# cvg/pixel-perfect-sfm

Hardware: NVIDIA B200
Metric: featuremetric BA observations/sec (higher is better)
Workload: dtype f64 (fp16 taps, fp32 horizontal, fp64 vertical/solve)

## Files before the change

pixel-perfect-sfm_b200/build.py:

```python
import os
import subprocess
import sys
from concurrent.futures import ThreadPoolExecutor

HERE = os.path.dirname(os.path.abspath(__file__))
CSRC = os.path.join(HERE, "csrc")
SOURCES = ["pxr_api.cu", "pxr_upload.cu", "pxr_ba.cu", "pxr_ba_block.cu", "pxr_inner.cu", "pxr_refs.cu", "pxr_ka.cu", "pxr_synth.cu", "pxr_extract.cu", "pxr_problem.cu"]
NVCC = os.environ.get("NVCC", "/usr/local/cuda/bin/nvcc")
FLAGS = ["-gencode", "arch=compute_100a,code=sm_100a", "-lineinfo", "-O3", "-std=c++17",
         "-Xcompiler", "-fPIC", "-ccbin", "/usr/bin/g++", "--expt-relaxed-constexpr",
         "-Xptxas", "-v"]
if os.environ.get("PXR_FM_WARPS"):
    FLAGS.append("-DPXR_FM_WARPS=" + os.environ["PXR_FM_WARPS"])


def _newer(src, obj):
    if not os.path.exists(obj):
        return True
    t = os.path.getmtime(obj)
    deps = [src] + [os.path.join(CSRC, f) for f in os.listdir(CSRC) if f.endswith((".cuh", ".h"))]
    deps.append(os.path.join(HERE, "..", "include", "pxr.h"))
    return any(os.path.getmtime(d) > t for d in deps)


def compile_one(name, verbose):
    src = os.path.join(CSRC, name)
    obj = os.path.join(CSRC, name.replace(".cu", ".o"))
    if not _newer(src, obj):
        return name, "up to date"
    cmd = [NVCC] + FLAGS + ["-c", src, "-o", obj]
    r = subprocess.run(cmd, capture_output=True, text=True)
    log = os.path.join(CSRC, name.replace(".cu", ".ptxas.log"))
    with open(log, "w") as f:
        f.write(r.stderr)
    if r.returncode != 0:
        sys.stderr.write(r.stderr[-6000:])
        raise RuntimeError("nvcc failed for " + name)
    return name, "compiled"


def build(verbose=False):
    srcs = [s for s in SOURCES if os.path.exists(os.path.join(CSRC, s))]
    with ThreadPoolExecutor(max_workers=min(8, len(srcs))) as ex:
        for name, status in ex.map(lambda n: compile_one(n, verbose), srcs):
            if verbose:
                print("  %-16s %s" % (name, status))
    objs = [os.path.join(CSRC, s.replace(".cu", ".o")) for s in srcs]
    out = os.path.join(CSRC, "libpxr.so")
    if (not os.path.exists(out)) or any(os.path.getmtime(o) > os.path.getmtime(out) for o in objs):
        cmd = [NVCC, "-shared", "-o", out] + objs + ["-gencode", "arch=compute_100a,code=sm_100a",
                                                     "-Xcompiler", "-fPIC", "-ccbin", "/usr/bin/g++", "-lcudart", "-ldl"]
        r = subprocess.run(cmd, capture_output=True, text=True)
        if r.returncode != 0:
            sys.stderr.write(r.stderr[-4000:])
            raise RuntimeError("link failed")
    return out


def build_bindings(verbose=False):
    import sysconfig
    src = os.path.join(HERE, "bindings", "pxr_pybind.cc")
    try:
        import pybind11
    except ImportError:
        sys.stderr.write("pybind11 not importable: bindings/_pxr_pybind is not built\n")
        return None
    out = os.path.join(HERE, "bindings", "_pxr_pybind" + sysconfig.get_config_var("EXT_SUFFIX"))
    deps = [src, os.path.join(HERE, "..", "include", "pxr.h"), os.path.join(CSRC, "libpxr.so")]
    if os.path.exists(out) and all(os.path.getmtime(d) <= os.path.getmtime(out) for d in deps):
        return out
    cmd = ["/usr/bin/g++", "-O2", "-std=c++17", "-shared", "-fPIC", "-I" + pybind11.get_include(),
           "-I" + sysconfig.get_paths()["include"], src, "-o", out, "-L" + CSRC, "-lpxr", "-Wl,-rpath,$ORIGIN/../csrc"]
    r = subprocess.run(cmd, capture_output=True, text=True)
    if r.returncode != 0:
        sys.stderr.write("bindings/_pxr_pybind did not build:\n" + r.stderr[-3000:])
        return None
    if verbose:
        print("  %-16s compiled" % "pxr_pybind.cc")
    return out


if __name__ == "__main__":
    print(build(verbose=True))
    print(build_bindings(verbose=True))
```

pixel-perfect-sfm_b200/csrc/pxr_ba.cu:

```cuda
#include <chrono>
#include <cmath>
#include <cstdlib>
#include <algorithm>
#include <cstring>
#include <limits>
#include <memory>

#include "pxr_ba_host.h"

#include "pxr_resident.cuh"
#include "pxr_chol2.cuh"

namespace pxr {

template <typename T, int C, int MODE, bool FS>
static int launch_fm(pxr_ctx* ctx, const FmEvalArgs& a, int* n_partials) {
  typedef FmCfg<T, C> Cfg;
  auto kern = fm_eval_kernel<T, C, MODE, FS>;
  static bool attr_set = false;
  if (!attr_set) {
    PXR_CUDA(cudaFuncSetAttribute(kern, cudaFuncAttributeMaxDynamicSharedMemorySize, Cfg::kSmem));
    attr_set = true;
  }
  const int64_t n_batches = cdiv(a.end - a.begin, 32);
  int64_t grid = cdiv(n_batches, Cfg::kWarps);
  const int64_t resident = (int64_t)ctx->sm_count * std::max(1, (int)(200 * 1024 / Cfg::kSmem));
  if (grid > resident) grid = resident;
  if (grid < 1) grid = 1;
  *n_partials = (int)(grid * Cfg::kWarps);
  PXR_LAUNCH(ctx, kern, (unsigned)grid, Cfg::kWarps * 32, Cfg::kSmem, a);
  PXR_CUDA(cudaGetLastError());
  return PXR_OK;
}

template <typename T, int C>
static int launch_fm_tc(pxr_ctx* ctx, const FmEvalArgs& a, int mode, bool fs, int* np) {
  if (mode == 1) return fs ? launch_fm<T, C, 1, true>(ctx, a, np) : launch_fm<T, C, 1, false>(ctx, a, np);
  return fs ? launch_fm<T, C, 0, true>(ctx, a, np) : launch_fm<T, C, 0, false>(ctx, a, np);
}

template <typename T, int C>
static int launch_fm_small(pxr_ctx* ctx, const FmEvalArgs& a, int mode, int* np) {
  const int64_t n = a.end - a.begin;
  *np = 0;
  if (n <= 0) return PXR_OK;
  if (mode == 1) PXR_LAUNCH(ctx, (fm_eval_small_kernel<T, C, 1>), (unsigned)cdiv(n, 128), 128, 0, a);
  else PXR_LAUNCH(ctx, (fm_eval_small_kernel<T, C, 0>), (unsigned)cdiv(n, 128), 128, 0, a);
  PXR_CUDA(cudaGetLastError());
  return PXR_OK;
}

int fm_supported(int dtype, int C) {
  if ((C == 1 || C == 3 || C == 4) && (dtype == PXR_F16 || dtype == PXR_F32 || dtype == PXR_F64)) return 1;
  if (dtype == PXR_F16) return C == 8 || C == 16 || C == 32 || C == 64 || C == 128 || C == 256;
  if (dtype == PXR_F32) return C == 16 || C == 64 || C == 128;
  if (dtype == PXR_F64) return C == 16 || C == 128;
  return 0;
}

int fm_max_partials(pxr_ctx* ctx) { return ctx->sm_count * 16 * 64; }

int launch_fm_eval(pxr_ctx* ctx, int dtype, int C, int mode, bool float_simd, const FmEvalArgs& a, int* np) {
#define PXR_SMALL(T) \
  { if (C == 3) return launch_fm_small<T, 3>(ctx, a, mode, np); if (C == 4) return launch_fm_small<T, 4>(ctx, a, mode, np); \
    if (C == 1) return launch_fm_small<T, 1>(ctx, a, mode, np); }
  if (C < 8) {
    if (dtype == PXR_F16) PXR_SMALL(__half) else if (dtype == PXR_F32) PXR_SMALL(float) else if (dtype == PXR_F64) PXR_SMALL(double)
    return fail(PXR_ERR_UNSUPPORTED, "Unsupported dimensions (CHANNELS=%d, dtype=%d, N_NODES=1).", C, dtype);
  }
#undef PXR_SMALL
#define PXR_CASE(T, CC) \
  if (C == CC) return launch_fm_tc<T, CC>(ctx, a, mode, float_simd, np);
  if (dtype == PXR_F16) {
    PXR_CASE(__half, 128) PXR_CASE(__half, 64) PXR_CASE(__half, 32) PXR_CASE(__half, 16) PXR_CASE(__half, 8)
    PXR_CASE(__half, 256)
  } else if (dtype == PXR_F32) {
    PXR_CASE(float, 128) PXR_CASE(float, 64) PXR_CASE(float, 16)
  } else if (dtype == PXR_F64) {
    PXR_CASE(double, 128) PXR_CASE(double, 16)
  }
#undef PXR_CASE
  return fail(PXR_ERR_UNSUPPORTED, "Unsupported dimensions (CHANNELS=%d, dtype=%d, N_NODES=1).", C, dtype);
}

static int check_desc(const pxr_ba_desc* d) {
  if (!d) return fail(PXR_ERR_INVALID_ARGUMENT, "desc is NULL");
  if (d->n_cameras <= 0 || d->n_images <= 0 || d->n_points < 0 || d->n_obs < 0)
    return fail(PXR_ERR_INVALID_ARGUMENT, "empty problem");
  if (!d->cam_model || !d->cam_params || !d->cam_const_mask || !d->qvec || !d->tvec || !d->img_cam ||
      !d->pose_const || !d->tvec_const_mask || (d->n_points && (!d->xyz || !d->point_const)) ||
      (d->n_obs && (!d->obs_img || !d->obs_pt)) || (!d->patches && d->n_patch_blocks <= 0) || !d->corner || !d->scale)
    return fail(PXR_ERR_INVALID_ARGUMENT, "a required array is NULL");
  if (!fm_supported(d->patch_dtype, d->channels))
    return fail(PXR_ERR_UNSUPPORTED, "Unsupported dimensions (CHANNELS=%d, dtype=%d, N_NODES=1).", d->channels, d->patch_dtype);
  if (d->ph < 1 || d->pw < 1) return fail(PXR_ERR_INVALID_ARGUMENT, "bad patch size");
  for (int c = 0; c < d->n_cameras; ++c)
    if (cam_num_params(d->cam_model[c]) == 0) return fail(PXR_ERR_UNSUPPORTED, "unsupported camera model id %d", d->cam_model[c]);
  for (int i = 0; i < d->n_images; ++i)
    if (d->img_cam[i] < 0 || d->img_cam[i] >= d->n_cameras) return fail(PXR_ERR_INVALID_ARGUMENT, "img_cam out of range");
  const int64_t np = d->obs_patch ? d->n_patches : d->n_obs;
  for (int64_t o = 0; o < d->n_obs; ++o) {
    if (d->obs_img[o] < 0 || d->obs_img[o] >= d->n_images) return fail(PXR_ERR_INVALID_ARGUMENT, "obs_img out of range");
    if (d->obs_pt[o] < 0 || d->obs_pt[o] >= d->n_points) return fail(PXR_ERR_INVALID_ARGUMENT, "obs_pt out of range");
    if (o && d->obs_pt[o] < d->obs_pt[o - 1]) return fail(PXR_ERR_INVALID_ARGUMENT, "observations must be sorted by point index");
    if (d->obs_patch && (d->obs_patch[o] < 0 || d->obs_patch[o] >= np)) return fail(PXR_ERR_INVALID_ARGUMENT, "obs_patch out of range");
  }
  if (!d->obs_patch && d->n_patches < d->n_obs) return fail(PXR_ERR_INVALID_ARGUMENT, "n_patches < n_obs with identity patch map");
  return PXR_OK;
}

int BA::create(pxr_ctx* c, const pxr_ba_desc* d, const pxr_interp_config* ic, const pxr_solver_options* so, bool for_solve) {
  ctx = c;
  PXR_TRY(check_desc(d));
  if (ic) interp = *ic; else pxr_default_interp_config(&interp);
  if (so) opt = *so; else pxr_default_ba_options(&opt);
  if (interp.check_bounds) return fail(PXR_ERR_UNSUPPORTED, "check_bounds=true is not supported on this path");
  env.pcg_sparse = getenv("PXR_PCG_SPARSE") != nullptr; env.build_atomic = getenv("PXR_BUILD_ATOMIC") != nullptr;
  env.chol_multikernel = getenv("PXR_CHOL_MULTIKERNEL") != nullptr; env.chol_test_abort = getenv("PXR_CHOL_TEST_ABORT") != nullptr;
  env.build_staged = getenv("PXR_BUILD_UNSTAGED") == nullptr;
  env.project_staged = getenv("PXR_PROJECT_UNSTAGED") == nullptr;
  env.cg_multi = getenv("PXR_CG_MULTI") != nullptr; env.no_speculation = getenv("PXR_NO_SPECULATION") != nullptr;
  if (const char* t = getenv("PXR_CHOL_TRACE")) env.chol_trace = t;
  PXR_CUDA(cudaSetDevice(ctx->device));
  cudaStream_t s = ctx->stream;
  n_cameras = d->n_cameras; n_images = d->n_images; n_points = d->n_points; n_obs = d->n_obs;
  C = d->channels; ph = d->ph; pw = d->pw; dtype = d->patch_dtype; ups = d->upsampling_factor;
  n_patches = d->obs_patch ? d->n_patches : std::max(d->n_patches, d->n_obs);
  has_refs = d->refs != nullptr;
  cudaStream_t us = nullptr;
  PXR_TRY(upload_stream(ctx, &us));
  struct JoinUpload { BA* ba; cudaStream_t us; ~JoinUpload() { if (ba->res_thread.joinable()) ba->res_thread.join(); cudaStreamSynchronize(us); } } join_upload{this, us};
  double h2d_patch = 0;
  const size_t esz = dtype == PXR_F16 ? 2 : (dtype == PXR_F32 ? 4 : 8);
  const size_t pbytes = (size_t)n_patches * ph * pw * C * esz;
  if (d->n_patch_blocks > 0) {
    if (!d->patch_block_ptrs || !d->patch_block_counts) return fail(PXR_ERR_INVALID_ARGUMENT, "patch block arrays are NULL");
    int64_t tot = 0;
    for (int b = 0; b < d->n_patch_blocks; ++b) tot += d->patch_block_counts[b];
    if (tot < n_patches) return fail(PXR_ERR_INVALID_ARGUMENT, "patch blocks hold %lld patches, %lld needed", (long long)tot, (long long)n_patches);
    PXR_TRY(patches_owned.alloc(ctx, (size_t)tot * ph * pw * C * esz));
    PXR_TRY(resident_setup(d, esz));
    if (!resident) {
      std::vector<size_t> seg_bytes((size_t)d->n_patch_blocks);
      for (int b = 0; b < d->n_patch_blocks; ++b) seg_bytes[b] = (size_t)d->patch_block_counts[b] * ph * pw * C * esz;
      PXR_TRY(upload_segments(ctx, patches_owned.p, d->patch_block_ptrs, seg_bytes.data(), d->n_patch_blocks, &h2d_patch, us));
    }
    d_patches = patches_owned.p;
  } else if (d->patches_on_device) {
    d_patches = (const uint8_t*)d->patches;
  } else {
    PXR_TRY(patches_owned.alloc(ctx, pbytes));
    PXR_TRY(resident_setup(d, esz));
    if (!resident) {
      PXR_TRY(upload_bytes(ctx, patches_owned.p, d->patches, pbytes, nullptr, us));
      h2d_patch = (double)pbytes;
// ... 27 lines not shown
  h_pt_begin.assign(n_points + 1, 0);
  for (int64_t o = 0; o < n_obs; ++o) h_pt_begin[d->obs_pt[o] + 1]++;
  for (int64_t p = 0; p < n_points; ++p) h_pt_begin[p + 1] += h_pt_begin[p];

  double h2d = h2d_patch;
  auto up = [&](auto& buf, const auto* host, size_t n) -> int { h2d += n * sizeof(*host); return buf.upload(host, n, s); };
  PXR_TRY(up(obs_img, d->obs_img, n_obs));
  PXR_TRY(up(obs_pt, d->obs_pt, n_obs));
  if (d->obs_patch) PXR_TRY(up(obs_patch, d->obs_patch, n_obs));
  PXR_TRY(up(img_cam, d->img_cam, n_images));
  PXR_TRY(up(cam_model, d->cam_model, n_cameras));
  PXR_TRY(up(cam_mask, cmask.data(), n_cameras));
  PXR_TRY(up(tmask, d->tvec_const_mask, n_images));
  PXR_TRY(up(pose_off, h_pose_off.data(), n_images));
  PXR_TRY(up(intr_off, h_intr_off.data(), n_cameras));
  PXR_TRY(up(point_off, h_point_off.data(), n_points));
  PXR_TRY(up(pt_begin, h_pt_begin.data(), n_points + 1));
  PXR_TRY(up(corner, d->corner, (size_t)n_patches * 2));
  PXR_TRY(up(scale, d->scale, (size_t)n_patches * 2));
  if (has_refs) PXR_TRY(up(refs, d->refs, (size_t)n_points * C));
  for (int k = 0; k < 2; ++k) {
    PXR_TRY(cam[k].upload(d->cam_params, (size_t)n_cameras * kMaxK, s));
    PXR_TRY(q[k].upload(d->qvec, (size_t)n_images * 4, s));
    PXR_TRY(t[k].upload(d->tvec, (size_t)n_images * 3, s));
    PXR_TRY(X[k].upload(d->xyz, (size_t)n_points * 3, s));
  }
  h2d += ((size_t)n_cameras * kMaxK + n_images * 7 + n_points * 3) * 8.0;
  cur = 0;
  PXR_TRY(uv.alloc((size_t)n_obs * 2));
  if (resident) { double wbytes = 0; PXR_TRY(resident_begin(us, &wbytes)); h2d += wbytes; }
  PXR_TRY(obs_out.alloc((size_t)n_obs * 8));
  PXR_TRY(juv.alloc((size_t)n_obs * juv_stride));
  if (for_solve) {
    PXR_TRY(uv_alt.alloc((size_t)n_obs * 2)); PXR_TRY(obs_out_alt.alloc((size_t)n_obs * 8)); PXR_TRY(juv_alt.alloc((size_t)n_obs * juv_stride));
    PXR_TRY(obs_out_alt.zero(s));
  }
  use_pcg = opt.linear_solver == PXR_SOLVER_ITERATIVE_SCHUR || (opt.linear_solver == PXR_SOLVER_AUTO && n_images > 1000);
  {
    int dc_needed = 0;
    h_img_cols.assign((size_t)n_images * 8, -1); h_img_pd.assign(n_images, 0);
    std::vector<int8_t> h_src((size_t)n_images * 8, -1);
    std::vector<int32_t> h_dc(n_images, 0);
    for (int i = 0; i < n_images; ++i) {
      std::vector<int> cols, src;
      if (h_pose_off[i] >= 0) {
        for (int k = 0; k < 3; ++k) { cols.push_back(h_pose_off[i] + k); src.push_back(k); }
        int la = 3;
        for (int k = 0; k < 3; ++k) if (!(d->tvec_const_mask[i] & (1u << k))) { cols.push_back(h_pose_off[i] + la++); src.push_back(3 + k); }
      }
      const int pd = (int)cols.size();
      const int cam_i = d->img_cam[i];
      if (h_intr_off[cam_i] >= 0) {
        const int kc = cam_num_params(d->cam_model[cam_i]);
        int la = 0;
        for (int k = 0; k < kc; ++k) if (!(cmask[cam_i] & (1u << k))) { cols.push_back(h_intr_off[cam_i] + la++); src.push_back(9 + k); }
      }
      dc_needed = std::max(dc_needed, (int)cols.size());
      h_img_pd[i] = pd;
      h_dc[i] = (int32_t)cols.size();
      for (size_t k = 0; k < cols.size() && k < 8; ++k) { h_img_cols[(size_t)i * 8 + k] = cols[k]; h_src[(size_t)i * 8 + k] = (int8_t)src[k]; }
    }
    img_dc_max = dc_needed;
    if (dc_needed <= 8) {
      PXR_TRY(img_cols8.upload(h_img_cols.data(), h_img_cols.size(), s));
      PXR_TRY(img_src8.upload(h_src.data(), h_src.size(), s));
      PXR_TRY(img_dc8.upload(h_dc.data(), h_dc.size(), s));
      PXR_CUDA(cudaStreamSynchronize(s));
    }
    h_img_cam.assign(d->img_cam, d->img_cam + n_images);
    sparse_schur = for_solve && use_pcg && dc_needed <= 8 && (n_obs > 0 || ctx->world > 1) &&
                   (env.pcg_sparse || (int64_t)nc * nc * 8 > (int64_t)4e9);
    deterministic = for_solve && opt.deterministic != 0;
    if (deterministic && dc_needed > 8)
      return fail(PXR_ERR_UNSUPPORTED, "deterministic assembly needs <= 8 camera columns per image (pose 6 + intrinsics), got %d", dc_needed);
    block_mode = for_solve && dc_needed <= 8 && (ctx->world > 1 || deterministic || getenv("PXR_BLOCK_ASSEMBLY") != nullptr);
    if (ctx->world > 1 && sparse_schur && !block_mode) sparse_schur = false;
    if (!sparse_schur && (int64_t)nc * nc * 8 > (int64_t)40e9)
      return fail(PXR_ERR_UNSUPPORTED, "reduced camera system too large for the dense path (nc=%d) and the block-sparse path needs ITERATIVE_SCHUR with <= 8 camera columns per image", nc);
  }
  if (!sparse_schur && !block_mode) PXR_TRY(Hcc.alloc((size_t)nc * nc));
  PXR_TRY(gc.alloc(nc));
  PXR_TRY(Hpp.alloc((size_t)n_points * 9)); PXR_TRY(gp.alloc((size_t)n_points * 3));
  h_obs_img.assign(d->obs_img, d->obs_img + n_obs);
  use_monolithic_inner = std::getenv("PXR_INNER_MONOLITHIC") != nullptr;
  if (for_solve) PXR_TRY(build_schur_pairs());
  if (block_mode) PXR_TRY(block_setup());
  if (for_solve && n_obs > 0 && n_obs < ((int64_t)1 << 31)) {
    int dc_needed = 0;
    std::vector<int> img_dc(n_images, 0);
    for (int i = 0; i < n_images; ++i) {
      int dc = 0;
      if (h_pose_off[i] >= 0) dc += 3 + (3 - __builtin_popcount(d->tvec_const_mask[i] & 7u));
      const int cam_i = d->img_cam[i];
      if (h_intr_off[cam_i] >= 0) dc += cam_num_params(d->cam_model[cam_i]) - __builtin_popcount(cmask[cam_i]);
      img_dc[i] = dc;
      dc_needed = std::max(dc_needed, dc);
    }
    if (dc_needed <= 8) {
      std::vector<int64_t> cnt(n_images + 1, 0);
      for (int64_t o = 0; o < n_obs; ++o) if (img_dc[d->obs_img[o]] > 0) cnt[d->obs_img[o] + 1]++;
      for (int i = 0; i < n_images; ++i) cnt[i + 1] += cnt[i];
      std::vector<int32_t> list(cnt[n_images]);
      {
        std::vector<int64_t> cur_pos(cnt.begin(), cnt.end() - 1);
        for (int64_t o = 0; o < n_obs; ++o) if (img_dc[d->obs_img[o]] > 0) list[cur_pos[d->obs_img[o]]++] = (int32_t)o;
      }
      std::vector<int64_t> cb;
      h_img_chunk_begin.assign((size_t)n_images + 1, 0);
      for (int i = 0; i < n_images; ++i) {
        h_img_chunk_begin[i] = (int64_t)cb.size();
        for (int64_t b = cnt[i]; b < cnt[i + 1]; b += 128) cb.push_back(b);
      }
      h_img_chunk_begin[n_images] = (int64_t)cb.size();
      cb.push_back(cnt[n_images]);
      io_n_chunks = (int64_t)cb.size() - 1;
      if (io_n_chunks > 0) {
        PXR_TRY(io_obs.upload(list.data(), list.size(), s));
        PXR_TRY(io_chunk_begin.upload(cb.data(), cb.size(), s));
        PXR_CUDA(cudaStreamSynchronize(s));
      }
      if (deterministic) {
        PXR_TRY(det_cam_part.alloc((size_t)std::max<int64_t>(io_n_chunks, 1) * 48));
        PXR_TRY(det_img_chunk_begin.upload(h_img_chunk_begin.data(), h_img_chunk_begin.size(), s));
        PXR_CUDA(cudaStreamSynchronize(s));
      }
    }
  }
  PXR_TRY(W.alloc((size_t)n_obs * dcmax * 3)); PXR_TRY(Wcols.alloc((size_t)n_obs * dcmax)); PXR_TRY(Wdc.alloc(n_obs));
  if (!sparse_schur) PXR_TRY(S.alloc((size_t)(nc + 1) * nc));
  PXR_TRY(rhs.alloc(nc));
  PXR_TRY(diag.alloc(nl)); PXR_TRY(jscale.alloc(nl)); PXR_TRY(D2.alloc(nl)); PXR_TRY(delta.alloc(nl));
  PXR_TRY(partials.alloc(fm_max_partials(ctx)));
  if (deterministic) {
    const int64_t big = std::max<int64_t>({n_obs, n_points * 3, (int64_t)n_images * 4, (int64_t)n_cameras * kMaxK});
    PXR_TRY(det_scal_part.alloc((size_t)(cdiv(big, 128) * 4 + 16)));
    if (io_n_chunks == 0 && n_obs > 0) return fail(PXR_ERR_UNSUPPORTED, "deterministic assembly needs the per-image chunk lists (problem too large for 32-bit observation ids)");
  }
  PXR_TRY(scalars.alloc(16));
  PXR_TRY(flags.alloc(4));
  PXR_TRY(rdiag.alloc(kNB));
  PXR_TRY(Hpp.zero(s)); PXR_TRY(gp.zero(s)); PXR_TRY(obs_out.zero(s));
  PXR_CUDA(cudaStreamSynchronize(s));
  if (res_thread.joinable()) {
    res_thread.join();
    if (res_thread_rc != PXR_OK) return fail(res_thread_rc, "%s", res_thread_err.c_str());
  }
  h2d_bytes = h2d;
  return PXR_OK;
}

int BA::build_schur_pairs() {
  if (sp_built) return PXR_OK;
  PXR_TRY(Tbuf.alloc((size_t)n_obs * dcmax * 3));
  PXR_TRY(Hinv.alloc((size_t)std::max<int64_t>(n_points, 1) * 6));
  const int64_t kChunk = 128;
  const int64_t ni = n_images;
  auto key_of = [&](int ia, int ib, bool self) -> int64_t {
    return ((int64_t)ia * (ia + 1) / 2 + ib) * 2 + (self ? 1 : 0);
  };
  const int64_t n_keys = (ni * (ni + 1) / 2) * 2;
  std::vector<int64_t> count(n_keys + 1, 0);
  int64_t total = 0;
  for (int64_t p = 0; p < n_points; ++p) {
    if (h_point_off[p] < 0) continue;
    for (int64_t i = h_pt_begin[p]; i < h_pt_begin[p + 1]; ++i)
      for (int64_t j = h_pt_begin[p]; j <= i; ++j) {
        const int a = h_obs_img[i], b = h_obs_img[j];
// ... 17 lines not shown
          pp[k] = (int32_t)p;
        }
    }
  }
  std::vector<int64_t> cb;
  std::vector<uint8_t> cself;
  std::vector<int32_t> ckey, ka, kbv;
  std::vector<uint8_t> kself;
  {
    int64_t k = 0;
    for (int64_t ia = 0; ia < ni; ++ia)
      for (int64_t ib = 0; ib <= ia; ++ib)
        for (int self = 0; self < 2; ++self, ++k) {
          if (count[k + 1] == count[k]) continue;
          if (sparse_schur || block_mode) { ka.push_back((int32_t)ia); kbv.push_back((int32_t)ib); kself.push_back((uint8_t)self); h_key_code_local.push_back(k); }
          for (int64_t s = count[k]; s < count[k + 1]; s += kChunk) {
            cb.push_back(s); cself.push_back((uint8_t)self);
            if (sparse_schur || block_mode) ckey.push_back((int32_t)ka.size() - 1);
          }
        }
  }
  cb.push_back(total);
  if (block_mode) {
    h_key_a = ka; h_key_b = kbv; h_key_self = kself;
    PXR_TRY(ss_chunk_key.upload(ckey.data(), ckey.size(), ctx->stream));
    PXR_CUDA(cudaStreamSynchronize(ctx->stream));
    h_chunk_key_local = ckey;
  } else if (sparse_schur) {
    ss_n_keys = (int)ka.size();
    PXR_TRY(ss_key_a.upload(ka.data(), ka.size(), ctx->stream)); PXR_TRY(ss_key_b.upload(kbv.data(), kbv.size(), ctx->stream));
    PXR_TRY(ss_key_self.upload(kself.data(), kself.size(), ctx->stream));
    PXR_TRY(ss_chunk_key.upload(ckey.data(), ckey.size(), ctx->stream));
    PXR_TRY(ss_Bk.alloc((size_t)std::max(ss_n_keys, 1) * 64));
    PXR_TRY(ss_Himg.alloc((size_t)n_images * 64));
    PXR_TRY(ss_img_cols.upload(h_img_cols.data(), h_img_cols.size(), ctx->stream));
    PXR_TRY(ss_img_pd.upload(h_img_pd.data(), h_img_pd.size(), ctx->stream));
    PXR_CUDA(cudaStreamSynchronize(ctx->stream));
  }
  sp_n_chunks = (int64_t)cself.size();
  cudaStream_t s = ctx->stream;
  PXR_TRY(sp_px.upload(px.data(), px.size(), s));
  PXR_TRY(sp_py.upload(py.data(), py.size(), s));
  PXR_TRY(sp_pp.upload(pp.data(), pp.size(), s));
  PXR_TRY(sp_chunk_begin.upload(cb.data(), cb.size(), s));
  PXR_TRY(sp_chunk_self.upload(cself.data(), cself.size(), s));
  PXR_CUDA(cudaStreamSynchronize(s));
  sp_built = true;
  return PXR_OK;
}

SchurPairs BA::schur_pairs() {
  SchurPairs sp;
  sp.px = sp_px.p; sp.py = sp_py.p; sp.pp = sp_pp.p; sp.chunk_begin = sp_chunk_begin.p; sp.chunk_self = sp_chunk_self.p;
  sp.n_chunks = sp_n_chunks;
  return sp;
}

int BA::project(int set, bool jac, double* xy_out) {
  ProjectArgs a;
  a.obs_img = obs_img.p; a.obs_pt = obs_pt.p; a.obs_patch = obs_patch.p;
  a.img_cam = img_cam.p; a.cam_model = cam_model.p;
  a.cam_params = cam[set].p; a.qvec = q[set].p; a.tvec = t[set].p; a.xyz = X[set].p;
  a.corner = corner.p; a.scale = scale.p; a.ups = ups;
  a.obs_begin = 0; a.obs_end = n_obs; a.item_index = nullptr;
  a.uv = uv.p; a.xy = xy_out; a.juv = jac ? juv.p : nullptr; a.juv_stride = juv_stride; a.juv_k = K;
  if (n_obs == 0) return PXR_OK;
  StageScope st(this, 2);
  const size_t staged_smem = (size_t)128 * (juv_stride | 1) * sizeof(double);
  if (jac && env.project_staged && staged_smem <= 48 * 1024)
    PXR_LAUNCH(ctx, ba_project_staged_kernel, (unsigned)cdiv(n_obs, 128), 128, staged_smem, a);
  else if (jac) PXR_LAUNCH(ctx, ba_project_kernel<true>, (unsigned)cdiv(n_obs, 128), 128, 0, a);
  else PXR_LAUNCH(ctx, ba_project_kernel<false>, (unsigned)cdiv(n_obs, 128), 128, 0, a);
  PXR_CUDA(cudaGetLastError());
  return PXR_OK;
}

int BA::resident_setup(const pxr_ba_desc* d, size_t esz) {
  resident = false;
  if (!allow_resident || n_obs == 0) return PXR_OK;
  if (const char* v = getenv("PXR_RESIDENT_WINDOW")) { const int e = std::atoi(v); if (e == 0 || !res_window_fixed) res_window = e; }
  const int W = res_window;
  if (W < 4 || C < 8 || ph > 255 || pw > 255 || ph < W + 2 || pw < W + 2) return PXR_OK;
  if ((size_t)ph * pw * C * esz > staged_chunk_bytes()) return PXR_OK;
  if (getenv("PXR_INNER_MONOLITHIC")) return PXR_OK;
  auto is_device = [](const void* ptr) -> bool {
    cudaPointerAttributes pa;
    if (cudaPointerGetAttributes(&pa, ptr) != cudaSuccess) { cudaGetLastError(); return false; }
    return pa.type == cudaMemoryTypeDevice || pa.type == cudaMemoryTypeManaged;
  };
  res_srcs.clear(); res_block_first.assign(1, 0);
  if (d->n_patch_blocks > 0) {
    for (int b = 0; b < d->n_patch_blocks; ++b) {
      if (is_device(d->patch_block_ptrs[b])) return PXR_OK;
      res_srcs.push_back(d->patch_block_ptrs[b]);
      res_block_first.push_back(res_block_first.back() + d->patch_block_counts[b]);
    }
  } else {
    if (is_device(d->patches)) return PXR_OK;
    res_srcs.push_back(d->patches);
    res_block_first.push_back(n_patches);
  }
  res_esz = esz;
  cudaStream_t s = ctx->stream;
  std::vector<uint8_t> shared((size_t)n_patches, 0);
  if (d->obs_patch) {
    h_obs_patch.assign(d->obs_patch, d->obs_patch + n_obs);
    std::vector<uint8_t> seen((size_t)n_patches, 0);
    for (int64_t o = 0; o < n_obs; ++o) { const int64_t p = d->obs_patch[o]; if (seen[p]) shared[p] = 1; seen[p] = 1; }
  }
  PXR_TRY(res_shared.upload(shared.data(), shared.size(), s));
  PXR_CUDA(cudaStreamSynchronize(s));
  PXR_TRY(res_rect.alloc((size_t)n_patches)); PXR_TRY(res_rect.zero(s));
  PXR_TRY(res_viol_count.alloc(1)); PXR_TRY(res_viol_count.zero(s));
  PXR_TRY(res_viol_list.alloc((size_t)n_obs)); PXR_TRY(res_fix_list.alloc((size_t)n_obs));
  resident = true;
  return PXR_OK;
}

int BA::resident_begin(cudaStream_t us, double* h2d_patch) {
  cudaStream_t s = ctx->stream;
  ProjectArgs pa;
  pa.obs_img = obs_img.p; pa.obs_pt = obs_pt.p; pa.obs_patch = obs_patch.p; pa.img_cam = img_cam.p; pa.cam_model = cam_model.p;
  pa.cam_params = cam[0].p; pa.qvec = q[0].p; pa.tvec = t[0].p; pa.xyz = X[0].p;
  pa.corner = corner.p; pa.scale = scale.p; pa.ups = ups; pa.obs_begin = 0; pa.obs_end = n_obs; pa.item_index = nullptr;
  pa.uv = uv.p; pa.xy = nullptr; pa.juv = nullptr; pa.juv_stride = juv_stride; pa.juv_k = K;
  PXR_LAUNCH(ctx, ba_project_kernel<false>, (unsigned)cdiv(n_obs, 128), 128, 0, pa);
  PXR_LAUNCH(ctx, resident_rect_kernel, (unsigned)cdiv(n_obs, 256), 256, 0, uv.p, obs_patch.p, res_shared.p, n_obs, ph, pw, res_window, res_rect.p);
  PXR_CUDA(cudaGetLastError());
  auto h_rect = std::make_shared<std::vector<uint32_t>>((size_t)n_patches);
  PXR_CUDA(cudaMemcpyAsync(h_rect->data(), res_rect.p, (size_t)n_patches * 4, cudaMemcpyDeviceToHost, s));
  PXR_CUDA(cudaStreamSynchronize(s));
  double bytes = 0;
  for (uint32_t rc : *h_rect) bytes += (double)((rc >> 16) & 255u) * (double)(rc >> 24) * C * (double)res_esz;
  *h2d_patch = bytes;
  res_thread_rc = PXR_OK;
  pxr_ctx* c = ctx;
  uint8_t* slab = patches_owned.p;
  const uint32_t* d_rect = res_rect.p;
  const int64_t np = n_patches; const int ph_ = ph, pw_ = pw, tap = C * (int)res_esz;
  res_thread = std::thread([this, c, slab, d_rect, np, ph_, pw_, tap, us, h_rect]() {
    cudaSetDevice(c->device);
    res_thread_rc = upload_windows(c, slab, res_srcs.data(), res_block_first.data(), (int)res_srcs.size(), h_rect->data(), d_rect,
                                   np, ph_, pw_, tap, nullptr, us);
    if (res_thread_rc != PXR_OK) res_thread_err = pxr_last_error();
  });
  return PXR_OK;
}

void BA::resident_args(FmEvalArgs& a) {
  if (!resident) return;
  a.res_rect = res_rect.p; a.viol_count = res_viol_count.p; a.viol_list = res_viol_list.p; a.viol_capacity = (long long)n_obs;
}

int BA::resident_fix(int64_t* n_fixed) {
  *n_fixed = 0;
  if (!resident) return PXR_OK;
  cudaStream_t s = ctx->stream;
  unsigned long long n = 0;
  PXR_CUDA(cudaMemcpyAsync(&n, res_viol_count.p, sizeof(n), cudaMemcpyDeviceToHost, s));
  PXR_CUDA(cudaStreamSynchronize(s));
  if (n == 0) return PXR_OK;
  n = std::min<unsigned long long>(n, (unsigned long long)n_obs);
  std::vector<int64_t> list((size_t)n);
  PXR_CUDA(cudaMemcpyAsync(list.data(), res_viol_list.p, (size_t)n * 8, cudaMemcpyDeviceToHost, s));
  PXR_CUDA(cudaMemcpyAsync(res_fix_list.p, res_viol_list.p, (size_t)n * 8, cudaMemcpyDeviceToDevice, s));
  PXR_CUDA(cudaMemsetAsync(res_viol_count.p, 0, sizeof(unsigned long long), s));
  PXR_CUDA(cudaStreamSynchronize(s));
  const size_t patch_bytes = (size_t)ph * pw * C * res_esz;
  if (res_whole.size() != (size_t)n_patches) res_whole.assign((size_t)n_patches, 0);
  int64_t fetched = 0;
  for (int64_t o : list) {
    const int64_t p = h_obs_patch.empty() ? o : h_obs_patch[(size_t)o];
    if (res_whole[(size_t)p]) continue;
    res_whole[(size_t)p] = 1; ++fetched;
    const size_t blk = (size_t)(std::upper_bound(res_block_first.begin(), res_block_first.end(), p) - res_block_first.begin()) - 1;
    const uint8_t* src = (const uint8_t*)res_srcs[blk] + (size_t)(p - res_block_first[blk]) * patch_bytes;
    PXR_CUDA(cudaMemcpyAsync(patches_owned.p + (size_t)p * patch_bytes, src, patch_bytes, cudaMemcpyHostToDevice, s));
  }
  PXR_LAUNCH(ctx, resident_mark_full_kernel, (unsigned)cdiv((int64_t)n, 256), 256, 0, res_fix_list.p, (int64_t)n, obs_patch.p, ph, pw, res_rect.p);
  PXR_CUDA(cudaGetLastError());
  res_refetched += fetched; res_passes_repeated++;
  h2d_bytes += (double)fetched * (double)patch_bytes;
  *n_fixed = (int64_t)n;
  return PXR_OK;
}

int BA::fm(int mode, double* residuals_out, double* cost_dev, double* grad_out) {
  PXR_TRY(fm_k1(mode, residuals_out, grad_out, nullptr, n_obs));
  for (;;) {
    int64_t n_fixed = 0;
    PXR_TRY(resident_fix(&n_fixed));
    if (n_fixed == 0) break;
    PXR_TRY(fm_k1(mode, residuals_out, grad_out, res_fix_list.p, n_fixed));
  }
  return fm_cost(cost_dev);
}

int BA::fm_k1(int mode, double* residuals_out, double* grad_out, const int64_t* list, int64_t n) {
  if (n <= 0 || n_obs == 0) return PXR_OK;
  FmEvalArgs a;
  a.uv = uv.p; a.item_patch = obs_patch.p; a.item_ref = obs_pt.p;
  a.patches = d_patches; a.ph = ph; a.pw = pw;
  a.refs = has_refs ? refs.p : nullptr;
  a.begin = 0; a.end = n; a.item_index = list;
  a.out = obs_out.p; a.residuals = residuals_out; a.desc = nullptr; a.grad = grad_out;
  a.loss.type = opt.loss_type; a.loss.a = opt.loss_scale;
  a.l2_normalize = interp.l2_normalize;
  resident_args(a);
  int np = 0;
  StageScope st(this, mode ? 1 : 0);
  return launch_fm_eval(ctx, dtype, C, mode, interp.use_float_simd != 0, a, &np);
}

int BA::fm_cost(double* cost_dev ) {
  if (n_obs > 0) {
    StageScope st2(this, 10);
    LossParams loss; loss.type = opt.loss_type; loss.a = opt.loss_scale;
    const int cb = std::min<int>(fm_max_partials(ctx), ctx->sm_count * 8);
    PXR_LAUNCH(ctx, cost_from_sq_norm_kernel, cb, 256, 0, obs_out.p, (int64_t)0, n_obs, loss, partials.p);
    PXR_LAUNCH(ctx, reduce_partials_kernel, 1, 1024, 0, partials.p, (int64_t)cb, cost_dev);
  } else {
    PXR_CUDA(cudaMemsetAsync(cost_dev, 0, 8, ctx->stream));
  }
  return PXR_OK;
}

int BA::evaluate(int set, bool jac, double* cost_out) {
  PXR_TRY(project(set, jac, nullptr));
  PXR_TRY(fm(jac ? 1 : 0, nullptr, scalars.p + 0));
  if (jac) PXR_TRY(build());
  if (block_mode) return global_cost_block(cost_out);
  PXR_TRY(allreduce_f64(ctx, scalars.p + 0, 1));
  double c = 0;
  PXR_CUDA(cudaMemcpyAsync(&c, scalars.p + 0, 8, cudaMemcpyDeviceToHost, ctx->stream));
  PXR_CUDA(cudaStreamSynchronize(ctx->stream));
  *cost_out = c;
  return PXR_OK;
}

BADev BA::dev() {
  BADev d;
  d.n_cameras = n_cameras; d.n_images = n_images; d.K = K; d.n_points = n_points; d.n_obs = n_obs;
  d.nc = nc; d.nl = (int)nl; d.dcmax = dcmax; d.juv_stride = juv_stride;
  d.obs_img = obs_img.p; d.obs_pt = obs_pt.p; d.img_cam = img_cam.p; d.cam_model = cam_model.p;
  d.cam_mask = cam_mask.p; d.tmask = tmask.p; d.pose_off = pose_off.p; d.intr_off = intr_off.p;
  d.point_off = point_off.p; d.pt_begin = pt_begin.p; d.obs_out = obs_out.p; d.juv = juv.p;
  d.img_cols8 = img_cols8.p; d.img_src8 = img_src8.p; d.img_dc8 = img_dc8.p;
  d.Hcc = Hcc.p; d.Hpp = Hpp.p; d.gp = gp.p; d.W = W.p; d.Wcols = Wcols.p; d.Wdc = Wdc.p;
  d.gc = block_mode ? pack_local.p + pk_off_gc : gc.p;
  d.loss.type = opt.loss_type; d.loss.a = opt.loss_scale;
  return d;
}

int BA::build() {
  if (block_mode) return build_block();
  StageScope st(this, 3);
  if (!sparse_schur) PXR_TRY(Hcc.zero(ctx->stream));
  PXR_TRY(gc.zero(ctx->stream));
  PXR_TRY(Hpp.zero(ctx->stream));
  PXR_TRY(gp.zero(ctx->stream));
  const bool chunked = io_n_chunks > 0 && (sparse_schur || !env.build_atomic);
  if (sparse_schur && !chunked && n_obs > 0) return fail(PXR_ERR_INTERNAL, "block-sparse path without per-image chunks");
  if (sparse_schur) PXR_TRY(ss_Himg.zero(ctx->stream));
  if (n_obs > 0) {
    const BADev dv = dev();
    const size_t staged_smem = (size_t)128 * ((std::max(dv.juv_stride, dv.dcmax * 3) | 1) + 9) * sizeof(double);
    if (img_src8.p && chunked && env.build_staged && staged_smem <= 48 * 1024)
      PXR_LAUNCH(ctx, ba_build_staged_kernel, (unsigned)cdiv(n_obs, 128), 128, staged_smem, dv);
    else if (img_src8.p) PXR_LAUNCH(ctx, ba_build_kernel<true>, (unsigned)cdiv(n_obs, 128), 128, 0, dv, chunked ? 0 : 1);
    else PXR_LAUNCH(ctx, ba_build_kernel<false>, (unsigned)cdiv(n_obs, 128), 128, 0, dv, chunked ? 0 : 1);
  }
  if (n_obs > 0 && chunked)
    PXR_LAUNCH(ctx, ba_build_cam_kernel, (unsigned)cdiv(io_n_chunks * 32, 256), 256, 0, dev(), io_obs.p, io_chunk_begin.p, io_n_chunks,
               sparse_schur ? ss_Himg.p : nullptr);
  const int64_t n = std::max<int64_t>(nc, n_points);
  if (sparse_schur && nc > 0) PXR_CUDA(cudaMemsetAsync(diag.p, 0, (size_t)nc * 8, ctx->stream));
  if (n > 0) PXR_LAUNCH(ctx, ba_diag_kernel, (unsigned)cdiv(n, 256), 256, 0, dev(), diag.p);
  if (sparse_schur && nc > 0) PXR_LAUNCH(ctx, sp_diag_kernel, (unsigned)cdiv((int64_t)n_images * 8, 256), 256, 0, sparse(), diag.p);
  if (ctx->world > 1 && nc > 0) {
    if (!gc_local.p) { PXR_TRY(gc_local.alloc(nc)); PXR_TRY(ar_buf.alloc((size_t)2 * nc)); }
    PXR_CUDA(cudaMemcpyAsync(gc_local.p, gc.p, (size_t)nc * 8, cudaMemcpyDeviceToDevice, ctx->stream));
    PXR_CUDA(cudaMemcpyAsync(ar_buf.p, diag.p, (size_t)nc * 8, cudaMemcpyDeviceToDevice, ctx->stream));
    PXR_CUDA(cudaMemcpyAsync(ar_buf.p + nc, gc.p, (size_t)nc * 8, cudaMemcpyDeviceToDevice, ctx->stream));
    PXR_TRY(allreduce_f64(ctx, ar_buf.p, (size_t)2 * nc));
    PXR_CUDA(cudaMemcpyAsync(diag.p, ar_buf.p, (size_t)nc * 8, cudaMemcpyDeviceToDevice, ctx->stream));
    PXR_CUDA(cudaMemcpyAsync(gc.p, ar_buf.p + nc, (size_t)nc * 8, cudaMemcpyDeviceToDevice, ctx->stream));
  }
  PXR_CUDA(cudaGetLastError());
  return PXR_OK;
}

SparseSchur BA::sparse() {
  SparseSchur q;
  q.n_images = n_images; q.n_keys = ss_n_keys; q.nc = nc;
  q.img_cols = ss_img_cols.p; q.img_pd = ss_img_pd.p; q.img_pose_blk = ss_img_pose_blk.p; q.img_cam_blk = ss_img_cam_blk.p;
  q.key_a = ss_key_a.p; q.key_b = ss_key_b.p; q.key_self = ss_key_self.p;
  q.Himg = ss_Himg.p; q.Bk = ss_Bk.p;
  return q;
}

int BA::chol_launch() {
  cudaStream_t s = ctx->stream;
    if (!chol_graph_exec) {
      chol_multikernel = chol_force_multikernel || env.chol_multikernel;
      if (!chol_multikernel) {
        int per_sm = 0, sms = 0, dev = 0;
        PXR_CUDA(cudaGetDevice(&dev));
        PXR_CUDA(cudaDeviceGetAttribute(&sms, cudaDevAttrMultiProcessorCount, dev));
        chol_band = getenv("PXR_CHOL_BAND") != nullptr;
        if (chol_band) {
          PXR_CUDA(cudaFuncSetAttribute(pxr_chol2::chol_band_kernel, cudaFuncAttributeMaxDynamicSharedMemorySize, (int)pxr_chol2::smem_bytes()));
          PXR_CUDA(cudaOccupancyMaxActiveBlocksPerMultiprocessor(&per_sm, pxr_chol2::chol_band_kernel, pxr_chol::kThreads, pxr_chol2::smem_bytes()));
        } else {
// ... 126 lines not shown
    PXR_TRY(launch_schur_pairs(d));
  }
  if (nc > 0) PXR_CUDA(cudaMemcpyAsync(S.p + (size_t)nc * nc, rhs.p, (size_t)nc * 8, cudaMemcpyDeviceToDevice, s));
  if (ctx->world > 1 && nc > 0) {
    PXR_TRY(allreduce_f64(ctx, S.p, (size_t)(nc + 1) * nc));
    PXR_CUDA(cudaMemcpyAsync(rhs.p, S.p + (size_t)nc * nc, (size_t)nc * 8, cudaMemcpyDeviceToDevice, s));
  }
  }
  st.reset(); st.reset(new StageScope(this, 5));
  last_linear_iterations = 1;
  if (nc > 0 && sparse_schur) {
    PXR_TRY(pcg_solve_sparse());
  } else if (nc > 0 && use_pcg) {
    PXR_TRY(pcg_solve());
  } else if (nc > 0) {
    PXR_TRY(chol_launch());
  }
  st.reset(); st.reset(new StageScope(this, 7));
  PXR_CUDA(cudaMemsetAsync(scalars.p + 4, 0, 4 * 8, s));
  if (n_points > 0) PXR_LAUNCH(ctx, ba_backsub_kernel, (unsigned)cdiv(n_points * 32, 256), 256, 0, d, D2.p, delta.p);
  if (n_obs > 0) {
    if (img_src8.p) PXR_LAUNCH(ctx, ba_model_cost_kernel<true>, (unsigned)cdiv(n_obs, 256), 256, 0, d, delta.p, scalars.p + 4);
    else PXR_LAUNCH(ctx, ba_model_cost_kernel<false>, (unsigned)cdiv(n_obs, 256), 256, 0, d, delta.p, scalars.p + 4);
  }
  PXR_CUDA(cudaGetLastError());
  st.reset();
  double acc = 0, fld = 0;
  if (chol_graph_exec && !chol_multikernel && !use_pcg && env.chol_test_abort) {
    const int one = 1;
    PXR_CUDA(cudaMemcpyAsync(chol_sync.p + (pxr_chol::sync_ints((int)cdiv(nc, kNB)) - 1), &one, sizeof(int), cudaMemcpyHostToDevice, s));
    PXR_CUDA(cudaMemcpyAsync(flags.p + 1, &one, sizeof(int), cudaMemcpyHostToDevice, s));
    PXR_CUDA(cudaStreamSynchronize(s));
  }
  PXR_LAUNCH(ctx, flags_to_double_kernel, 1, 1, 0, flags.p, scalars.p + 5);
  PXR_TRY(allreduce_f64(ctx, scalars.p + 4, 2));
  double two[2] = {0, 0};
  PXR_CUDA(cudaMemcpyAsync(two, scalars.p + 4, 16, cudaMemcpyDeviceToHost, s));
  PXR_CUDA(cudaStreamSynchronize(s));
  acc = two[0]; fld = two[1];
  if (fld != 0.0 && chol_graph_exec && !chol_multikernel && !use_pcg && ctx->world <= 1) {
    int aborted = 0;
    const int nbt = (int)cdiv(nc, kNB);
    PXR_CUDA(cudaMemcpyAsync(&aborted, chol_sync.p + (pxr_chol::sync_ints(nbt) - 1), sizeof(int), cudaMemcpyDeviceToHost, s));
    PXR_CUDA(cudaStreamSynchronize(s));
    if (aborted) {
      cudaGraphExecDestroy(chol_graph_exec); chol_graph_exec = nullptr;
      chol_force_multikernel = true;
      return compute_step(radius, valid, model_cost_change);
    }
  }
  const bool solved = fld == 0.0 && std::isfinite(acc);
  *model_cost_change = -acc;
  *valid = solved && (*model_cost_change > 0.0);
  return PXR_OK;
}

int BA::apply_step(double* step_norm, double* x_norm) {
  PlusArgs a;
  a.n_cameras = n_cameras; a.n_images = n_images; a.n_points = n_points;
  a.cam_model = cam_model.p; a.cam_mask = cam_mask.p; a.tmask = tmask.p;
  a.pose_off = pose_off.p; a.intr_off = intr_off.p; a.point_off = point_off.p;
  a.cam = cam[cur].p; a.q = q[cur].p; a.t = t[cur].p; a.X = X[cur].p;
  a.cam_o = cam[1 - cur].p; a.q_o = q[1 - cur].p; a.t_o = t[1 - cur].p; a.X_o = X[1 - cur].p;
  a.delta = delta.p; a.acc = scalars.p + 4;
  StageScope st(this, 8);
  PXR_CUDA(cudaMemsetAsync(scalars.p + 5, 0, 4 * 8, ctx->stream));
  const int64_t n = std::max<int64_t>(std::max<int64_t>(n_points, n_images), n_cameras);
  if (deterministic) a.part = det_scal_part.p;
  PXR_LAUNCH(ctx, ba_plus_kernel, (unsigned)cdiv(n, 128), 128, 0, a);
  if (deterministic)
    for (int k = 0; k < 4; ++k) PXR_LAUNCH(ctx, det_reduce_add_kernel, 1, 1024, 0, det_scal_part.p, cdiv(n, 128), 4, k, a.acc + 1 + k);
  PXR_CUDA(cudaGetLastError());
  if (!block_mode) PXR_TRY(allreduce_f64(ctx, scalars.p + 5, 2));
  if (step_norm || x_norm) {
    double v[4];
    PXR_CUDA(cudaMemcpyAsync(v, scalars.p + 5, 32, cudaMemcpyDeviceToHost, ctx->stream));
    PXR_CUDA(cudaStreamSynchronize(ctx->stream));
    if (step_norm) *step_norm = std::sqrt(v[0] + v[2]);
    if (x_norm) *x_norm = std::sqrt(v[1] + v[3]);
  }
  return PXR_OK;
}

int BA::eval_list(int set, const int64_t* list, int64_t n, const unsigned long long* n_dev, bool settle) {
  if (n <= 0) return PXR_OK;
  ProjectArgs pa;
  pa.obs_img = obs_img.p; pa.obs_pt = obs_pt.p; pa.obs_patch = obs_patch.p;
  pa.img_cam = img_cam.p; pa.cam_model = cam_model.p;
  pa.cam_params = cam[set].p; pa.qvec = q[set].p; pa.tvec = t[set].p; pa.xyz = X[set].p;
  pa.corner = corner.p; pa.scale = scale.p; pa.ups = ups;
  pa.obs_begin = 0; pa.obs_end = n; pa.item_index = list; pa.n_dev = n_dev;
  pa.uv = uv.p; pa.xy = nullptr; pa.juv = juv.p; pa.juv_stride = juv_stride; pa.juv_k = K;
  PXR_LAUNCH(ctx, ba_project_kernel<true>, (unsigned)cdiv(n, 128), 128, 0, pa);
  FmEvalArgs a;
  a.uv = uv.p; a.item_patch = obs_patch.p; a.item_ref = obs_pt.p;
  a.patches = d_patches; a.ph = ph; a.pw = pw;
  a.refs = has_refs ? refs.p : nullptr;
  a.begin = 0; a.end = n; a.item_index = list; a.end_dev = n_dev;
  a.out = obs_out.p; a.residuals = nullptr; a.desc = nullptr;
  a.loss.type = opt.loss_type; a.loss.a = opt.loss_scale;
  a.l2_normalize = interp.l2_normalize;
  resident_args(a);
  int np = 0;
  PXR_TRY(launch_fm_eval(ctx, dtype, C, 1, interp.use_float_simd != 0, a, &np));
  if (!settle) return PXR_OK;
  for (;;) {
    int64_t n_fixed = 0;
    PXR_TRY(resident_fix(&n_fixed));
    if (n_fixed == 0) break;
    a.item_index = res_fix_list.p; a.begin = 0; a.end = n_fixed; a.end_dev = nullptr;
    PXR_TRY(launch_fm_eval(ctx, dtype, C, 1, interp.use_float_simd != 0, a, &np));
  }
  return PXR_OK;
}

constexpr int kInnerRounds = 53;
int BA::inner_rounds(int set) {
  cudaStream_t s = ctx->stream;
  InnerStepArgs a;
  a.n_points = n_points; a.point_off = point_off.p; a.pt_begin = pt_begin.p;
  a.obs_out = obs_out.p; a.juv = juv.p; a.juv_stride = juv_stride; a.juv_w = 9 + K;
  a.xyz = X[set].p; a.st = inner_state.p;
  a.loss.type = opt.loss_type; a.loss.a = opt.loss_scale;
  a.list = inner_list.p; a.counters = inner_counters.p;
  const unsigned pgrid = (unsigned)cdiv(n_points, 128);
  for (int round = 0; round < kInnerRounds; ++round) {
    if (round >= 2) {
      const cudaError_t q = cudaEventQuery(inner_events[round - 2]);
      if (q == cudaSuccess) { if (inner_cnt_host[2 * (round - 2)] == 0) break; }
      else if (q != cudaErrorNotReady) PXR_CUDA(q);
      else if ((void)cudaGetLastError(), round >= 8 && (round & 3) == 0) {
        PXR_CUDA(cudaEventSynchronize(inner_events[round - 2]));
        if (inner_cnt_host[2 * (round - 2)] == 0) break;
      }
    }
    PXR_CUDA(cudaMemsetAsync(inner_counters.p, 0, 2 * sizeof(unsigned long long), s));
    PXR_LAUNCH(ctx, inner_list_kernel, pgrid, 128, 0, a, round == 0 ? 1 : 0);
    PXR_CUDA(cudaMemcpyAsync(inner_cnt_host + 2 * round, inner_counters.p, 2 * sizeof(unsigned long long), cudaMemcpyDeviceToHost, s));
    PXR_CUDA(cudaEventRecord(inner_events[round], s));
    PXR_TRY(eval_list(set, inner_list.p, n_obs, inner_counters.p, false));
    PXR_LAUNCH(ctx, inner_step_kernel, pgrid, 128, 0, a, round == 0 ? 0 : 1);
  }
  PXR_CUDA(cudaGetLastError());
  return PXR_OK;
}

int BA::inner_iterations_batched(int set) {
  if (n_points == 0 || n_obs == 0) return PXR_OK;
  StageScope stg(this, 9);
  cudaStream_t s = ctx->stream;
  if (!inner_state.p) {
    PXR_TRY(inner_state.alloc(n_points));
    PXR_TRY(inner_list.alloc(n_obs));
    PXR_TRY(inner_counters.alloc(2));
    PXR_CUDA(cudaHostAlloc((void**)&inner_cnt_host, (size_t)kInnerRounds * 2 * sizeof(unsigned long long), cudaHostAllocDefault));
    inner_events.resize(kInnerRounds, nullptr);
    for (auto& e : inner_events) PXR_CUDA(cudaEventCreateWithFlags(&e, cudaEventDisableTiming));
  }
  if (!resident) return inner_rounds(set);
  if (!inner_snapshot.p) PXR_TRY(inner_snapshot.alloc((size_t)n_points * 3));
  PXR_CUDA(cudaMemcpyAsync(inner_snapshot.p, X[set].p, (size_t)n_points * 24, cudaMemcpyDeviceToDevice, s));
  for (;;) {
    PXR_TRY(inner_rounds(set));
    int64_t n_fixed = 0;
    PXR_TRY(resident_fix(&n_fixed));
    if (n_fixed == 0) break;
    PXR_CUDA(cudaMemcpyAsync(X[set].p, inner_snapshot.p, (size_t)n_points * 24, cudaMemcpyDeviceToDevice, s));
  }
  return PXR_OK;
}

int BA::inner_iterations(int set) {
  if (!use_monolithic_inner) return inner_iterations_batched(set);
  InnerArgs a;
  a.n_points = n_points; a.point_off = point_off.p; a.pt_begin = pt_begin.p;
  a.obs_img = obs_img.p; a.obs_patch = obs_patch.p; a.img_cam = img_cam.p; a.cam_model = cam_model.p;
  a.cam_params = cam[set].p; a.qvec = q[set].p; a.tvec = t[set].p; a.xyz = X[set].p;
  a.corner = corner.p; a.scale = scale.p; a.ups = ups;
  a.patches = d_patches; a.ph = ph; a.pw = pw;
  a.refs = has_refs ? refs.p : nullptr;
  a.loss.type = opt.loss_type; a.loss.a = opt.loss_scale;
  a.l2_normalize = interp.l2_normalize;
  if (n_points == 0) return PXR_OK;
  StageScope st(this, 9);
  return launch_inner(ctx, dtype, C, interp.use_float_simd != 0, a);
}

int BA::step_norm_between_sets(double* out) {
  cudaStream_t s = ctx->stream;
  PXR_CUDA(cudaMemsetAsync(scalars.p + 11, 0, 16, s));
  auto run = [&](const double* a, const double* b, int64_t n, double* acc) {
    if (n > 0) PXR_LAUNCH(ctx, diff_norm_kernel, (unsigned)cdiv(n, 256), 256, 0, a, b, n, acc);
  };
  run(cam[0].p, cam[1].p, (int64_t)n_cameras * kMaxK, scalars.p + 12);
  run(q[0].p, q[1].p, (int64_t)n_images * 4, scalars.p + 12);
  run(t[0].p, t[1].p, (int64_t)n_images * 3, scalars.p + 12);
  run(X[0].p, X[1].p, n_points * 3, scalars.p + 11);
  PXR_TRY(allreduce_f64(ctx, scalars.p + 11, 1));
  double v[2] = {0, 0};
  PXR_CUDA(cudaMemcpyAsync(v, scalars.p + 11, 16, cudaMemcpyDeviceToHost, s));
  PXR_CUDA(cudaStreamSynchronize(s));
  *out = std::sqrt(v[0] + v[1]);
  return PXR_OK;
}

int BA::pcg_setup_blocks() {
  if (cg_state.p) return PXR_OK;
  cudaStream_t s = ctx->stream;
  std::vector<int32_t> off;
  for (int i = 0; i < n_images; ++i) if (h_pose_off[i] >= 0) off.push_back(h_pose_off[i]);
  for (int c = 0; c < n_cameras; ++c) if (h_intr_off[c] >= 0) off.push_back(h_intr_off[c]);
  std::sort(off.begin(), off.end());
  std::vector<int32_t> sd(off.size());
  for (size_t k = 0; k < off.size(); ++k) sd[k] = (k + 1 < off.size() ? off[k + 1] : nc) - off[k];
  cg_nblk = (int)off.size();
  PXR_TRY(cg_blk_off.upload(off.data(), off.size(), s)); PXR_TRY(cg_blk_dim.upload(sd.data(), sd.size(), s));
  PXR_TRY(cg_Minv.alloc((size_t)nc * 12)); PXR_TRY(cg_row_off.alloc(nc)); PXR_TRY(cg_row_dim.alloc(nc));
  PXR_TRY(cg_z.alloc(nc)); PXR_TRY(cg_p.alloc(nc)); PXR_TRY(cg_q.alloc(nc)); PXR_TRY(cg_r.alloc(nc)); PXR_TRY(cg_x.alloc(nc)); PXR_TRY(cg_tmp.alloc(nc));
  PXR_TRY(cg_state.alloc(1));
  if (sparse_schur) {
    auto blk_of = [&](int offset) -> int32_t { return (int32_t)(std::lower_bound(off.begin(), off.end(), offset) - off.begin()); };
    h_img_pose_blk.assign(n_images, -1); h_img_cam_blk.assign(n_images, -1);
    for (int i = 0; i < n_images; ++i) {
      if (h_pose_off[i] >= 0) h_img_pose_blk[i] = blk_of(h_pose_off[i]);
      const int io = h_intr_off[h_img_cam[i]];
      if (io >= 0) h_img_cam_blk[i] = blk_of(io);
    }
    PXR_TRY(ss_img_pose_blk.upload(h_img_pose_blk.data(), h_img_pose_blk.size(), s));
    PXR_TRY(ss_img_cam_blk.upload(h_img_cam_blk.data(), h_img_cam_blk.size(), s));
    PXR_TRY(ss_Dblk.alloc((size_t)std::max(cg_nblk, 1) * 144));
  }
  PXR_CUDA(cudaStreamSynchronize(s));
  return PXR_OK;
}

int BA::pcg_solve_sparse() {
  cudaStream_t s = ctx->stream;
  PXR_TRY(pcg_setup_blocks());
  const int n = nc;
  const SparseSchur sp = sparse();
  const int64_t nthreads = std::max<int64_t>(((int64_t)n_images + ss_n_keys) * 8, n);
  const unsigned gs = (unsigned)cdiv(nthreads, 256);
  const int add_d2 = (ctx->world <= 1 || ctx->rank == 0) ? 1 : 0;
  auto spmv = [&](const double* x, double* y) -> int {
    PXR_CUDA(cudaMemsetAsync(y, 0, (size_t)n * 8, s));
    PXR_LAUNCH(ctx, sp_spmv_kernel, gs, 256, 0, sp, D2.p, x, y, add_d2, cg_state.p);
    if (ctx->world > 1) PXR_TRY(allreduce_f64(ctx, y, n));
    return PXR_OK;
  };
  PXR_TRY(ss_Dblk.zero(s));
  PXR_LAUNCH(ctx, sp_blockdiag_kernel, (unsigned)cdiv(((int64_t)n_images + ss_n_keys) * 8, 256), 256, 0, sp, ss_Dblk.p);
  if (ctx->world > 1) PXR_TRY(allreduce_f64(ctx, ss_Dblk.p, (size_t)cg_nblk * 144));
  PXR_LAUNCH(ctx, sp_block_inverse_kernel, (unsigned)cdiv(cg_nblk, 64), 64, 0, ss_Dblk.p, D2.p, 1, cg_blk_off.p, cg_blk_dim.p, cg_nblk,
             cg_Minv.p, cg_row_off.p, cg_row_dim.p, flags.p + 1);
  return run_cg(spmv);
}

int BA::pcg_solve() {
  cudaStream_t s = ctx->stream;
  PXR_TRY(pcg_setup_blocks());
  const int n = nc;
  const unsigned gv = (unsigned)cdiv((int64_t)n * 32, 256);
  PXR_LAUNCH(ctx, cg_mirror_kernel, (unsigned)cdiv((int64_t)n * n, 256), 256, 0, S.p, n);
  PXR_LAUNCH(ctx, cg_block_inverse_kernel, (unsigned)cdiv(cg_nblk, 64), 64, 0, S.p, n, cg_blk_off.p, cg_blk_dim.p, cg_nblk, cg_Minv.p,
             cg_row_off.p, cg_row_dim.p, flags.p + 1);
  auto spmv = [&](const double* x, double* y) -> int {
    PXR_LAUNCH(ctx, cg_gemv_kernel, gv, 256, 0, S.p, x, y, n, cg_state.p);
    return PXR_OK;
// ... 89 lines not shown

bool BA::lm_finalize(int max_iteration) {
  pxr_iteration_summary& it = lm.it;
  if (lm.pending_finalize) {
    if (it.step_is_successful) {
      ++lm.n_succ;
      if (lm.x_cost < lm.minimum_cost) lm.minimum_cost = lm.x_cost;
    } else if (it.iteration > 0) ++lm.n_unsucc;
    it.trust_region_radius = lm.radius;
    it.iteration_time_s = std::chrono::duration<double>(std::chrono::steady_clock::now() - lm.it_start).count();
    lm.its.push_back(it);
    lm.pending_finalize = false;
  }
  if (it.iteration >= max_iteration) { lm.term = 1; lm.message = "Maximum number of iterations reached."; return false; }
  if (it.gradient_max_norm <= opt.gradient_tolerance) { lm.term = 0; lm.message = "Gradient tolerance reached."; lm.finished = true; return false; }
  if (lm.radius < opt.min_trust_region_radius) { lm.term = 0; lm.message = "Minimum trust region radius reached."; lm.finished = true; return false; }
  return true;
}

int BA::lm_iterate(int max_iteration) {
  if (block_mode) return lm_iterate_block(max_iteration);
  using clk = std::chrono::steady_clock;
  if (!lm.started) PXR_TRY(lm_begin());
  lm.it_start = clk::now();
  while (!lm.finished && lm_finalize(max_iteration)) {
    if (interrupt_pending()) {
      lm.finished = true; lm.term = 3;
      lm.message = "interrupted by the host";
      return fail(PXR_ERR_INTERRUPTED, "interrupted by the host after LM iteration %d", lm.it.iteration);
    }
    lm.it_start = clk::now();
    pxr_iteration_summary& it = lm.it;
    const double prev_gmax = it.gradient_max_norm;
    const int iteration = it.iteration + 1;
    std::memset(&it, 0, sizeof(it));
    it.iteration = iteration;
    lm.pending_finalize = true;

    bool valid = false;
    double model_cost_change = 0;
    PXR_TRY(compute_step(lm.radius, &valid, &model_cost_change));
    it.linear_solver_iterations = last_linear_iterations;
    it.step_is_valid = valid;
    if (!valid) {
      if (++lm.num_invalid >= opt.max_num_consecutive_invalid_steps) {
        lm.term = 2; lm.finished = true;
        lm.message = "Number of consecutive invalid steps more than Solver::Options::max_num_consecutive_invalid_steps";
        break;
      }
      lm.radius /= lm.decrease_factor; lm.decrease_factor *= 2.0;
      it.cost = lm.x_cost; it.gradient_max_norm = prev_gmax;
      continue;
    }
    lm.num_invalid = 0;

    double step_norm = 0, x_norm = 0, candidate_cost = 0;
    const bool speculate = !lm.inner_enabled && !env.no_speculation;
    if (speculate) PXR_TRY(apply_step(nullptr, nullptr)); else PXR_TRY(apply_step(&step_norm, &x_norm));
    swap_sets();
    int rc = PXR_OK;
    if (speculate) {
      rc = project(1 - cur, true, nullptr);
      if (rc == PXR_OK) rc = fm(1, nullptr, scalars.p + 0);
      if (rc == PXR_OK) rc = allreduce_f64(ctx, scalars.p + 0, 1);
      if (rc == PXR_OK) {
        double nv[4] = {0, 0, 0, 0};
        cudaError_t e = cudaMemcpyAsync(&candidate_cost, scalars.p + 0, 8, cudaMemcpyDeviceToHost, ctx->stream);
        if (e == cudaSuccess) e = cudaMemcpyAsync(nv, scalars.p + 5, 32, cudaMemcpyDeviceToHost, ctx->stream);
        if (e == cudaSuccess) e = cudaStreamSynchronize(ctx->stream);
        if (e != cudaSuccess) rc = fail(PXR_ERR_CUDA, "trial evaluation failed: %s", cudaGetErrorString(e));
        step_norm = std::sqrt(nv[0] + nv[2]); x_norm = std::sqrt(nv[1] + nv[3]);
      }
    } else {
      rc = evaluate(1 - cur, false, &candidate_cost);
    }
    if (rc != PXR_OK) { swap_sets(); return rc; }
    if (!std::isfinite(candidate_cost)) candidate_cost = std::numeric_limits<double>::max();

    bool inner_useful = false;
    if (lm.inner_enabled && candidate_cost < std::numeric_limits<double>::max()) {
      ++lm.n_inner;
      rc = inner_iterations(1 - cur);
      double inner_cost = 0;
      if (rc == PXR_OK) rc = evaluate(1 - cur, false, &inner_cost);
      if (rc != PXR_OK) { swap_sets(); return rc; }
      if (std::isfinite(inner_cost)) {
        model_cost_change += candidate_cost - inner_cost;
        inner_useful = inner_cost < lm.x_cost;
        const double rel = 1.0 - inner_cost / candidate_cost;
        lm.inner_enabled = rel > opt.inner_iteration_tolerance;
        candidate_cost = inner_cost;
        rc = step_norm_between_sets(&step_norm);
        if (rc != PXR_OK) { swap_sets(); return rc; }
      }
    }
    swap_sets();
    it.step_norm = step_norm;
    if (step_norm <= opt.parameter_tolerance * (x_norm + opt.parameter_tolerance)) {
      lm.term = 0; lm.message = "Parameter tolerance reached."; lm.finished = true; break;
    }
    it.cost_change = lm.x_cost - candidate_cost;
    if (std::fabs(it.cost_change) <= opt.function_tolerance * lm.x_cost) {
      lm.term = 0; lm.message = "Function tolerance reached."; lm.finished = true; break;
    }
    it.relative_decrease = lm.ev.quality(candidate_cost, model_cost_change);
    const bool ok = inner_useful || it.relative_decrease > opt.min_relative_decrease;
    if (ok) {
      cur = 1 - cur;
      if (speculate && candidate_cost < std::numeric_limits<double>::max()) {
        swap_sets();
        PXR_TRY(build());
        lm.x_cost = candidate_cost;
      } else {
        PXR_TRY(evaluate(cur, true, &lm.x_cost));
      }
      it.cost = lm.x_cost;
      PXR_TRY(gradient_max_norm(&it.gradient_max_norm));
      it.step_is_successful = 1;
      lm.radius = lm.radius / std::max(1.0 / 3.0, 1.0 - std::pow(2.0 * it.relative_decrease - 1.0, 3));
      lm.radius = std::min(opt.max_trust_region_radius, lm.radius);
      lm.decrease_factor = 2.0;
      lm.ev.accepted(candidate_cost, model_cost_change);
      if (opt.use_nonmonotonic_steps) {
        if (lm.x_cost < lm.minimum_cost) lm.best_is_current = true;
        else if (lm.best_is_current) { PXR_TRY(save_best(1 - cur)); lm.best_is_current = false; }
      }
    } else {
      it.step_is_successful = 0;
      it.cost = candidate_cost;
      it.gradient_max_norm = prev_gmax;
      lm.radius /= lm.decrease_factor; lm.decrease_factor *= 2.0;
    }
  }
  if (lm.x_cost < lm.minimum_cost) lm.minimum_cost = lm.x_cost;
  PXR_CUDA(cudaStreamSynchronize(ctx->stream));
  return PXR_OK;
}

void BA::fill_summary(pxr_summary* sum, double seconds, int64_t launches) {
  if (!sum) return;
  sum->initial_cost = lm.initial_cost; sum->final_cost = lm.minimum_cost;
  sum->num_residual_blocks = (int32_t)n_obs; sum->num_residuals = n_obs * C;
  sum->num_successful_steps = lm.n_succ; sum->num_unsuccessful_steps = lm.n_unsucc;
  sum->num_inner_iteration_steps = lm.n_inner; sum->termination_type = lm.term;
  sum->solve_time_s = seconds; sum->total_time_s = seconds;
  sum->h2d_bytes = h2d_bytes; sum->d2h_bytes = 0;
  sum->num_iterations = (int32_t)lm.its.size();
  const int m = std::min<int>((int)lm.its.size(), sum->iterations ? sum->iterations_capacity : 0);
  for (int i = 0; i < m; ++i) sum->iterations[i] = lm.its[i];
  sum->kernel_launches = launches;
  std::snprintf(sum->message, sizeof(sum->message), "%s", lm.message.c_str());
  sum->resident_window = resident ? res_window : 0;
  sum->resident_passes_repeated = (int32_t)res_passes_repeated; sum->resident_refetched = res_refetched;
}

int BA::solve(pxr_summary* sum) {
  const auto t0 = std::chrono::steady_clock::now();
  const int64_t l0 = ctx->launches;
  PXR_TRY(lm_begin());
  PXR_TRY(lm_iterate(opt.max_num_iterations));
  if (block_mode) PXR_TRY(finish_gmax_block());
  fill_summary(sum, std::chrono::duration<double>(std::chrono::steady_clock::now() - t0).count(), ctx->launches - l0);
  return PXR_OK;
}

int BA::save_best(int set) {
  cudaStream_t s = ctx->stream;
// ... 258 lines not shown
```

pixel-perfect-sfm_b200/csrc/pxr_ba_block.cu:

```cuda
#include <algorithm>
#include <cmath>
#include <cstring>
#include <limits>
#include <memory>
#include <numeric>

#include "pxr_ba_host.h"

namespace pxr {

namespace {

struct Contribution { int64_t dest; int32_t src; };

struct HostGatherMap { std::vector<int64_t> dest, ptr; std::vector<int32_t> src; };

HostGatherMap make_gather_map(std::vector<Contribution>& c, int64_t n_dest_rows, int64_t row_len, bool all_rows) {
  HostGatherMap m;
  std::vector<int64_t> cnt((size_t)n_dest_rows + 1, 0);
  for (const auto& e : c) cnt[(size_t)(e.dest / row_len) + 1]++;
  for (int64_t r = 0; r < n_dest_rows; ++r) cnt[r + 1] += cnt[r];
  std::vector<Contribution> sorted(c.size());
  {
    std::vector<int64_t> cur(cnt.begin(), cnt.end() - 1);
// ... 413 lines not shown
  return run_cg(spmv);
}

int BA::lm_begin_block() {
  PXR_CUDA(cudaSetDevice(ctx->device));
  cudaStream_t s = ctx->stream;
  lm = LMState();
  lm.radius = opt.initial_trust_region_radius;
  lm.inner_enabled = opt.use_inner_iterations != 0;
  PXR_TRY(project(cur, true, nullptr));
  PXR_TRY(fm(1, nullptr, scalars.p + 0));
  PXR_TRY(build_block());
  PXR_TRY(global_cost_block(&lm.x_cost));
  if (!std::isfinite(lm.x_cost)) return fail(PXR_ERR_NUMERIC, "initial cost is not finite");
  if (nl - nc > 0) PXR_LAUNCH(ctx, ba_scale_kernel, (unsigned)cdiv(nl - nc, 256), 256, 0, diag.p + nc, jscale.p + nc, nl - nc, opt.jacobi_scaling);
  jscale_c_pending = true;
  std::memset(&lm.it, 0, sizeof(lm.it));
  lm.it.cost = lm.x_cost;
  if (blk_lag_gmax) { lm.it.gradient_max_norm = std::numeric_limits<double>::quiet_NaN(); lm.gmax_pending = true; }
  else { PXR_TRY(gradient_max_norm(&lm.it.gradient_max_norm)); lm.gmax_pending = false; }
  lm.initial_cost = lm.minimum_cost = lm.x_cost;
  lm.ev.init(lm.x_cost, opt.use_nonmonotonic_steps ? opt.max_consecutive_nonmonotonic_steps : 0);
  lm.best_is_current = true;
  lm.started = true;
  lm.pending_finalize = true;
  lm.term = 1;
  lm.message = "Maximum number of iterations reached.";
  return PXR_OK;
}

int BA::finish_gmax_block() {
  if (!lm.gmax_pending) return PXR_OK;
  cudaStream_t s = ctx->stream;
  PXR_CUDA(cudaMemsetAsync(scalars.p + 10, 0, 8, s));
  if (nc > 0) {
    PXR_TRY(allreduce_f64_oop(ctx, pack_local.p + pk_off_gc, pk(true) + pk_off_gc, (size_t)nc));
    const int64_t n = std::max<int64_t>(n_images, n_cameras);
    PXR_LAUNCH(ctx, ba_gradmax_kernel, (unsigned)cdiv(n, 256), 256, 0, dev(), pk(true) + pk_off_gc, q[cur].p, 0, scalars.p + 10);
  }
  PXR_CUDA(cudaMemsetAsync(flags.p + 3, 0, sizeof(int), s));
  PXR_LAUNCH(ctx, blk_pack_scalars_kernel, 1, 1, 0, scalars.p, flags.p, mb_in.p, 3, ctx->rank == 0 ? 1 : 0, 0);
  PXR_TRY(exchange_scalars(1));
  double gcm = 0, gpm = 0;
  PXR_CUDA(cudaMemcpyAsync(&gcm, scalars.p + 10, 8, cudaMemcpyDeviceToHost, s));
  PXR_CUDA(cudaMemcpyAsync(&gpm, mb_out.p + 11, 8, cudaMemcpyDeviceToHost, s));
  PXR_CUDA(cudaStreamSynchronize(s));
  const double g = std::max(gcm, gpm);
  lm.it.gradient_max_norm = g;
  if (!lm.its.empty() && !(lm.its.back().gradient_max_norm == lm.its.back().gradient_max_norm)) lm.its.back().gradient_max_norm = g;
  lm.gmax_pending = false;
  return PXR_OK;
}

int BA::lm_iterate_block(int max_iteration) {
  using clk = std::chrono::steady_clock;
  cudaStream_t s = ctx->stream;
  if (!lm.started) PXR_TRY(lm_begin_block());
  lm.it_start = clk::now();
  const double kMax = std::numeric_limits<double>::max();
  while (!lm.finished && lm_finalize(max_iteration)) {
    const int interrupted = interrupt_pending() ? 1 : 0;
    lm.it_start = clk::now();
    pxr_iteration_summary& it = lm.it;
    const pxr_iteration_summary prev_it = it;
    const double prev_gmax = it.gradient_max_norm;
    const int iteration = it.iteration + 1;
    std::memset(&it, 0, sizeof(it));
    it.iteration = iteration;
    lm.pending_finalize = true;

    PXR_TRY(compute_step_block(lm.radius));
    it.linear_solver_iterations = last_linear_iterations;
    PXR_LAUNCH(ctx, blk_pack_scalars_kernel, 1, 1, 0, scalars.p, flags.p, mb_in.p, 0, ctx->rank == 0 ? 1 : 0, interrupted);
    PXR_TRY(apply_step(nullptr, nullptr));
    swap_sets();
    const bool speculate = !lm.inner_enabled && !env.no_speculation;
    const bool ran_inner = lm.inner_enabled;
    int rc = project(1 - cur, speculate, nullptr);
    if (rc == PXR_OK) rc = fm(speculate ? 1 : 0, nullptr, scalars.p + 0);
    if (rc != PXR_OK) { swap_sets(); return rc; }
    PXR_LAUNCH(ctx, blk_pack_scalars_kernel, 1, 1, 0, scalars.p, flags.p, mb_in.p, 1, ctx->rank == 0 ? 1 : 0, 0);
    if (ran_inner) {
      rc = inner_iterations(1 - cur);
      if (rc == PXR_OK) rc = project(1 - cur, false, nullptr);
      if (rc == PXR_OK) rc = fm(0, nullptr, scalars.p + 0);
      if (rc != PXR_OK) { swap_sets(); return rc; }
      PXR_CUDA(cudaMemsetAsync(scalars.p + 11, 0, 16, s));
      auto run = [&](const double* a, const double* b, int64_t n, double* acc) {
        if (n <= 0) return;
        PXR_LAUNCH(ctx, diff_norm_kernel, (unsigned)cdiv(n, 256), 256, 0, a, b, n, acc, deterministic ? det_scal_part.p : nullptr);
        if (deterministic) PXR_LAUNCH(ctx, det_reduce_add_kernel, 1, 1024, 0, det_scal_part.p, cdiv(n, 256), 1, 0, acc);
      };
      run(cam[0].p, cam[1].p, (int64_t)n_cameras * kMaxK, scalars.p + 12);
      run(q[0].p, q[1].p, (int64_t)n_images * 4, scalars.p + 12);
      run(t[0].p, t[1].p, (int64_t)n_images * 3, scalars.p + 12);
      run(X[0].p, X[1].p, n_points * 3, scalars.p + 11);
      PXR_LAUNCH(ctx, blk_pack_scalars_kernel, 1, 1, 0, scalars.p, flags.p, mb_in.p, 2, ctx->rank == 0 ? 1 : 0, 0);
    }
    PXR_TRY(exchange_scalars(11));
    double o[12]; double gmax_here = 0; int mfail = 0;
    PXR_CUDA(cudaMemcpyAsync(o, mb_out.p, sizeof(o), cudaMemcpyDeviceToHost, s));
    PXR_CUDA(cudaMemcpyAsync(&gmax_here, scalars.p + 10, 8, cudaMemcpyDeviceToHost, s));
    PXR_CUDA(cudaMemcpyAsync(&mfail, flags.p + 3, sizeof(int), cudaMemcpyDeviceToHost, s));
    PXR_CUDA(cudaStreamSynchronize(s));
    swap_sets();
    if (mfail) { lm.finished = true; lm.term = 2; return fail(PXR_ERR_NCCL, "a peer rank did not deliver its scalars (mailbox time-out)"); }
    gmax_here = std::max(gmax_here, o[11]);

    if (lm.gmax_pending) {
      lm.gmax_pending = false;
      if (!lm.its.empty()) lm.its.back().gradient_max_norm = gmax_here;
      if (gmax_here <= opt.gradient_tolerance) {
        it = prev_it; it.gradient_max_norm = gmax_here;
        lm.pending_finalize = false;
        lm.term = 0; lm.message = "Gradient tolerance reached."; lm.finished = true;
        break;
      }
    }
    const double known_gmax = blk_lag_gmax ? gmax_here : prev_gmax;
    if (o[10] > 0.0) {
      it = prev_it; lm.pending_finalize = false;
      lm.finished = true; lm.term = 3; lm.message = "interrupted by the host";
      return fail(PXR_ERR_INTERRUPTED, "interrupted by the host after LM iteration %d", it.iteration);
    }
    double model_cost_change = -o[0];
    const bool valid = o[1] == 0.0 && std::isfinite(o[0]) && model_cost_change > 0.0;
    it.step_is_valid = valid;
    if (!valid) {
      if (++lm.num_invalid >= opt.max_num_consecutive_invalid_steps) {
        lm.term = 2; lm.finished = true;
        lm.message = "Number of consecutive invalid steps more than Solver::Options::max_num_consecutive_invalid_steps";
        break;
      }
      lm.radius /= lm.decrease_factor; lm.decrease_factor *= 2.0;
      it.cost = lm.x_cost; it.gradient_max_norm = known_gmax;
      continue;
    }
    lm.num_invalid = 0;
    double candidate_cost = o[2];
    if (!std::isfinite(candidate_cost)) candidate_cost = kMax;
    double step_norm = std::sqrt(o[3] + o[5]);
    const double x_norm = std::sqrt(o[4] + o[6]);
    bool inner_useful = false;
    if (ran_inner && candidate_cost < kMax) {
      ++lm.n_inner;
      const double inner_cost = o[7];
      if (std::isfinite(inner_cost)) {
        model_cost_change += candidate_cost - inner_cost;
        inner_useful = inner_cost < lm.x_cost;
        const double rel = 1.0 - inner_cost / candidate_cost;
        lm.inner_enabled = rel > opt.inner_iteration_tolerance;
        candidate_cost = inner_cost;
        step_norm = std::sqrt(o[8] + o[9]);
      }
    }
    it.step_norm = step_norm;
    if (step_norm <= opt.parameter_tolerance * (x_norm + opt.parameter_tolerance)) {
      lm.term = 0; lm.message = "Parameter tolerance reached."; lm.finished = true; break;
    }
    it.cost_change = lm.x_cost - candidate_cost;
    if (std::fabs(it.cost_change) <= opt.function_tolerance * lm.x_cost) {
      lm.term = 0; lm.message = "Function tolerance reached."; lm.finished = true; break;
    }
    it.relative_decrease = lm.ev.quality(candidate_cost, model_cost_change);
    const bool ok = inner_useful || it.relative_decrease > opt.min_relative_decrease;
    if (ok) {
      cur = 1 - cur;
      if (speculate && candidate_cost < kMax) {
// ... 35 lines not shown
```

pixel-perfect-sfm_b200/csrc/pxr_ba_host.h:

```cpp
#pragma once
#include <cstdlib>
#include <chrono>
#include <string>
#include <functional>
#include <thread>
#include <limits>
#include <algorithm>
#include <utility>
#include <vector>

#include "pxr_ba_kernels.cuh"
#include "pxr_chol.cuh"
#include "pxr_fm_eval.cuh"
#include "pxr_fm_small.cuh"
#include "pxr_inner.cuh"
#include "pxr_internal.h"
#include "pxr_pcg.cuh"
#include "pxr_sparse_schur.cuh"
#include "pxr_block.cuh"

namespace pxr {

int fm_supported(int dtype, int C);
int fm_max_partials(pxr_ctx* ctx);
int launch_fm_eval(pxr_ctx* ctx, int dtype, int C, int mode, bool float_simd, const FmEvalArgs& a, int* n_partials);
int launch_inner(pxr_ctx* ctx, int dtype, int C, bool float_simd, const InnerArgs& a);

struct StepEvaluator {
  int max_nonmonotonic = 0, num_consecutive_nonmonotonic_steps = 0;
  double minimum_cost = 0, current_cost = 0, reference_cost = 0, candidate_cost = 0;
  double acc_reference = 0, acc_candidate = 0;
  void init(double c, int max_nm) { *this = StepEvaluator(); max_nonmonotonic = max_nm; minimum_cost = current_cost = reference_cost = candidate_cost = c; }
  double quality(double cost, double mcc) const {
    if (cost >= std::numeric_limits<double>::max()) return std::numeric_limits<double>::lowest();
    return std::max((current_cost - cost) / mcc, (reference_cost - cost) / (acc_reference + mcc));
  }
  void accepted(double cost, double mcc) {
    current_cost = cost; acc_candidate += mcc; acc_reference += mcc;
    if (current_cost < minimum_cost) { minimum_cost = current_cost; num_consecutive_nonmonotonic_steps = 0; candidate_cost = current_cost; acc_candidate = 0; }
    else { ++num_consecutive_nonmonotonic_steps; if (current_cost > candidate_cost) { candidate_cost = current_cost; acc_candidate = 0; } }
    if (num_consecutive_nonmonotonic_steps == max_nonmonotonic) { reference_cost = candidate_cost; acc_reference = acc_candidate; }
  }
};

struct LMState {
  bool started = false, finished = false, pending_finalize = false, inner_enabled = false;
  StepEvaluator ev;
  bool gmax_pending = false;
  bool best_is_current = true;
  double x_cost = 0, radius = 1e4, decrease_factor = 2.0, initial_cost = 0, minimum_cost = 0;
  int num_invalid = 0, n_succ = 0, n_unsucc = 0, n_inner = 0, term = 1;
  pxr_iteration_summary it;
  std::vector<pxr_iteration_summary> its;
  std::string message;
  std::chrono::steady_clock::time_point it_start;
};

struct BA {
  pxr_ctx* ctx = nullptr;
  LMState lm;
  static constexpr int kNumStages = 12;
  bool time_kernels = false;
  std::vector<std::pair<cudaEvent_t, cudaEvent_t>> timed[kNumStages];
  struct StageScope {
    BA* b; int id; cudaEvent_t e0 = nullptr, e1 = nullptr;
    StageScope(BA* b_, int id_) : b(b_), id(id_) {
      if (b->time_kernels && cudaEventCreate(&e0) == cudaSuccess && cudaEventCreate(&e1) == cudaSuccess) cudaEventRecord(e0, b->ctx->stream);
    }
    ~StageScope() { if (e0 && e1) { cudaEventRecord(e1, b->ctx->stream); b->timed[id].push_back({e0, e1}); } }
  };
  pxr_interp_config interp;
  pxr_solver_options opt;
  int n_cameras = 0, n_images = 0, K = 0, C = 0, ph = 0, pw = 0, dtype = 0;
  int64_t n_points = 0, n_obs = 0, n_patches = 0, nl = 0;
  int nc = 0, dcmax = 0, juv_stride = 0, img_dc_max = 0;
  double ups = 1.0;
  bool has_refs = false;
  double h2d_bytes = 0;
  std::vector<int32_t> h_pose_off, h_intr_off;
  std::vector<int64_t> h_point_off, h_pt_begin;
  DevBuf<int32_t> obs_img, img_cam, cam_model, pose_off, intr_off, corner, Wcols, Wdc;
  DevBuf<int64_t> obs_pt, obs_patch, point_off, pt_begin;
  DevBuf<uint32_t> cam_mask;
  DevBuf<uint8_t> tmask;
  PatchSlab patches_owned;
  DevBuf<double> scale, refs;
  const uint8_t* d_patches = nullptr;
  DevBuf<double> cam[2], q[2], t[2], X[2];
  DevBuf<double> best_cam, best_q, best_t, best_X;
  int save_best(int set);
  int cur = 0;
  DevBuf<double> uv_alt, obs_out_alt, juv_alt;
  void swap_sets() { std::swap(uv.p, uv_alt.p); std::swap(uv.n, uv_alt.n); std::swap(obs_out.p, obs_out_alt.p); std::swap(obs_out.n, obs_out_alt.n); std::swap(juv.p, juv_alt.p); std::swap(juv.n, juv_alt.n); }
  DevBuf<double> ar_buf;
  DevBuf<double> gc_local;
  DevBuf<double> uv, obs_out, juv, Hcc, gc, Hpp, gp, W, S, rhs, diag, jscale, D2, delta, partials, scalars;
  DevBuf<int> flags;
  DevBuf<double> rdiag;
  bool use_pcg = false;
  DevBuf<double> cg_Minv, cg_z, cg_p, cg_q, cg_r, cg_x, cg_tmp, cg_part;
  DevBuf<int32_t> cg_blk_off, cg_blk_dim, cg_row_off, cg_row_dim;
  DevBuf<CGState> cg_state;
  int cg_nblk = 0, last_linear_iterations = 1;
  int pcg_solve();
  int run_cg(const std::function<int(const double*, double*)>& spmv);
  struct EnvFlags { bool pcg_sparse = false, build_atomic = false, chol_multikernel = false, chol_test_abort = false,
                         cg_multi = false, no_speculation = false, build_staged = true, project_staged = true; std::string chol_trace; } env;
  bool sparse_schur = false;
  int ss_n_keys = 0;
  std::vector<int32_t> h_img_cols, h_img_pd, h_img_pose_blk, h_img_cam_blk, h_img_cam;
  DevBuf<int32_t> ss_img_cols, ss_img_pd, ss_img_pose_blk, ss_img_cam_blk, ss_key_a, ss_key_b, ss_chunk_key;
  DevBuf<uint8_t> ss_key_self;
  DevBuf<double> ss_Himg, ss_Bk, ss_Dblk;
  SparseSchur sparse();
  int pcg_solve_sparse();
  bool block_mode = false;
  DevBuf<double> pack_local, pack_global;
  size_t pk_off_B = 0, pk_off_rhs = 0, pk_off_gc = 0, pk_off_slots = 0, pk_n = 0;
  double* pk(bool global) { return (global && pack_global.p) ? pack_global.p : pack_local.p; }
  SparseSchur sparse_blk(bool global);
  std::vector<int32_t> h_key_a, h_key_b; std::vector<uint8_t> h_key_self;
  DevBuf<int64_t> gmS_dest, gmS_ptr, dg_ptr, gmD_dest, gmD_ptr, br_chunk_begin, br_cols_ptr;
  DevBuf<int32_t> gmS_src, dg_src, gmD_src, br_chunk_img, br_ent_key, br_cols_src;
  DevBuf<uint8_t> br_chunk_first;
  DevBuf<double> br_ypart, mb_in, mb_out;
  int64_t gmS_rows = 0, gmD_rows = 0, br_n_chunks = 0;
  bool deterministic = false;
  std::vector<int64_t> h_img_chunk_begin;
  DevBuf<int64_t> det_img_chunk_begin, det_key_chunk_begin;
  DevBuf<double> det_cam_part, det_pair_part, det_gimg, det_rimg, det_scal_part;
  bool jscale_c_pending = false;
  bool blk_lag_gmax = false;
  int block_setup();
  int build_block();
  int compute_step_block(double radius);
  int compute_step_block_sync(double radius, bool* valid, double* model_cost_change);
  int global_cost_block(double* cost_out);
  int pcg_solve_block();
  int lm_begin_block();
  int lm_iterate_block(int max_iteration);
  int finish_gmax_block();
  int exchange_scalars(int n_sum);
  std::vector<int32_t> h_chunk_key_local;
  std::vector<int64_t> h_key_code_local;
  int pcg_setup_blocks();
  int launch_schur_pairs(const BADev& d);
  int launch_sp_schur_pairs(const BADev& d, double* Bk, double* rhs_out, double* part);
  cudaGraphExec_t chol_graph_exec = nullptr;
  int64_t chol_graph_kernels = 0;
  bool chol_multikernel = false, chol_force_multikernel = false, chol_band = false; int chol_grid = 0;
  int schur_kernel = [] { const char* e = getenv("PXR_SCHUR_KERNEL"); return !e ? 0 : (e[0] == 'm' ? 3 : (e[0] == 's' ? 1 : (e[0] == 'd' ? 2 : 0))); }();
  int schur_ctas = getenv("PXR_SCHUR_CTAS") ? atoi(getenv("PXR_SCHUR_CTAS")) : 0;
  DevBuf<int32_t> img_cols8, img_dc8; DevBuf<int8_t> img_src8;
  DevBuf<int32_t> io_obs;
  DevBuf<int64_t> io_chunk_begin; int64_t io_n_chunks = 0;
  DevBuf<long long> chol_trace;
  DevBuf<int> chol_sync;
  ~BA() { if (inner_cnt_host) cudaFreeHost(inner_cnt_host); for (auto e : inner_events) cudaEventDestroy(e); if (res_thread.joinable()) res_thread.join(); if (chol_graph_exec) cudaGraphExecDestroy(chol_graph_exec); for (int k = 0; k < kNumStages; ++k) for (auto& pr : timed[k]) { cudaEventDestroy(pr.first); cudaEventDestroy(pr.second); } }
  DevBuf<int32_t> sp_px, sp_py, sp_pp;
  DevBuf<int64_t> sp_chunk_begin;
  DevBuf<uint8_t> sp_chunk_self;
  DevBuf<double> Tbuf, Hinv;
  int64_t sp_n_chunks = 0;
  bool sp_built = false;
  std::vector<int32_t> h_obs_img;
  int build_schur_pairs();
  SchurPairs schur_pairs();

  int create(pxr_ctx* c, const pxr_ba_desc* d, const pxr_interp_config* ic, const pxr_solver_options* so, bool for_solve);
  bool allow_resident = false, resident = false;
  int res_window = 8;
  bool res_window_fixed = false;
  DevBuf<uint32_t> res_rect;
  DevBuf<unsigned long long> res_viol_count;
  DevBuf<int64_t> res_viol_list, res_fix_list;
  DevBuf<uint8_t> res_shared;
  std::vector<const void*> res_srcs;
  std::vector<int64_t> res_block_first;
  std::vector<int64_t> h_obs_patch;
  std::vector<uint8_t> res_whole;
  int64_t res_refetched = 0, res_passes_repeated = 0;
  size_t res_esz = 2;
  std::thread res_thread;
  int res_thread_rc = 0; std::string res_thread_err;
  int resident_setup(const pxr_ba_desc* d, size_t esz);
  int resident_begin(cudaStream_t us, double* h2d_patch);
  int resident_fix(int64_t* n_fixed);
  void resident_args(FmEvalArgs& a);
  BADev dev();
  int project(int set, bool jac, double* xy_out);
  int fm(int mode, double* residuals_out, double* cost_dev, double* grad_out = nullptr);
  int fm_k1(int mode, double* residuals_out, double* grad_out, const int64_t* list, int64_t n);
  int fm_cost(double* cost_dev);
  int build();
  int evaluate(int set, bool jac, double* cost_out);
  int compute_step(double radius, bool* valid, double* model_cost_change);
  int chol_launch();
  int apply_step(double* step_norm, double* x_norm);
  int gradient_max_norm(double* out);
  int inner_iterations(int set);
  int inner_iterations_batched(int set);
  int eval_list(int set, const int64_t* list, int64_t n, const unsigned long long* n_dev = nullptr, bool settle = true);
  int inner_rounds(int set);
  unsigned long long* inner_cnt_host = nullptr;
  std::vector<cudaEvent_t> inner_events;
  DevBuf<double> inner_snapshot;
  DevBuf<InnerState> inner_state;
  DevBuf<int64_t> inner_list;
  DevBuf<unsigned long long> inner_counters;
  bool use_monolithic_inner = false;
  int step_norm_between_sets(double* out);
  int lm_begin();
  bool lm_finalize(int max_iteration);
  int lm_iterate(int max_iteration);
  void fill_summary(pxr_summary* sum, double seconds, int64_t launches);
  int solve(pxr_summary* sum);
  int read_params(double* cam_o, double* q_o, double* t_o, double* X_o);
};

}
```

pixel-perfect-sfm_b200/csrc/pxr_fm_eval.cuh:

```cuda
#pragma once
#include "pxr_device.cuh"

namespace pxr {

struct ProjectArgs {
  const int32_t* obs_img; const int64_t* obs_pt; const int64_t* obs_patch;
  const int32_t* img_cam; const int32_t* cam_model;
  const double* cam_params; const double* qvec; const double* tvec; const double* xyz;
  const int32_t* corner; const double* scale; double ups;
  int64_t obs_begin, obs_end;
  const int64_t* item_index;
  const unsigned long long* n_dev = nullptr;
  double* uv;
  double* xy;
  double* juv;
  int juv_stride;
  int juv_k;
};

template <bool JAC>
__device__ __forceinline__ void project_observation(const ProjectArgs& a, int64_t o, double* out) {
  const int img = a.obs_img[o];
  const int64_t pt = a.obs_pt[o];
  const int64_t pi = a.obs_patch ? a.obs_patch[o] : o;
  const int cam = a.img_cam[img];
  const int model = a.cam_model[cam];
  double q[4], t[3], X[3], cp[kMaxK];
#pragma unroll
  for (int i = 0; i < 4; ++i) q[i] = a.qvec[4 * (int64_t)img + i];
#pragma unroll
  for (int i = 0; i < 3; ++i) { t[i] = a.tvec[3 * (int64_t)img + i]; X[i] = a.xyz[3 * pt + i]; }
#pragma unroll
  for (int i = 0; i < kMaxK; ++i) cp[i] = a.cam_params[(int64_t)cam * kMaxK + i];
  double xy[2], Jpose[2][6], Jpt[2][3], Jk[2][kMaxK];
  world_to_pixel<JAC>(model, cp, q, t, X, xy, Jpose, Jpt, Jk);
  const double sx = a.scale[2 * pi], sy = a.scale[2 * pi + 1];
  const double cx = (double)a.corner[2 * pi], cy = (double)a.corner[2 * pi + 1];
  a.uv[2 * o] = (xy[0] * sx - 0.5 - cx) * a.ups;
  a.uv[2 * o + 1] = (xy[1] * sy - 0.5 - cy) * a.ups;
  if (a.xy) { a.xy[2 * o] = xy[0]; a.xy[2 * o + 1] = xy[1]; }
  if (JAC && out) {
    const int W = 9 + a.juv_k;
    const double s[2] = {sx * a.ups, sy * a.ups};
#pragma unroll
    for (int r = 0; r < 2; ++r) {
#pragma unroll
      for (int k = 0; k < 6; ++k) out[r * W + k] = s[r] * Jpose[r][k];
#pragma unroll
      for (int k = 0; k < 3; ++k) out[r * W + 6 + k] = s[r] * Jpt[r][k];
      for (int k = 0; k < a.juv_k; ++k) out[r * W + 9 + k] = s[r] * Jk[r][k];
    }
  }
}

template <bool JAC>
__global__ void __launch_bounds__(128) ba_project_kernel(ProjectArgs a) {
  const int64_t k = a.obs_begin + (int64_t)blockIdx.x * blockDim.x + threadIdx.x;
  const int64_t end = a.n_dev ? a.obs_begin + (int64_t)*a.n_dev : a.obs_end;
  if (k >= end) return;
  const int64_t o = a.item_index ? a.item_index[k] : k;
  project_observation<JAC>(a, o, (JAC && a.juv) ? a.juv + o * (int64_t)a.juv_stride : nullptr);
}

static __global__ void __launch_bounds__(128) ba_project_staged_kernel(ProjectArgs a) {
  extern __shared__ double sm_proj[];
  const int tid = threadIdx.x;
  const int64_t o0 = a.obs_begin + (int64_t)blockIdx.x * 128;
  const int n = (int)min((int64_t)128, a.obs_end - o0);
  const int js = a.juv_stride, SP = js | 1;
  if (tid < n) project_observation<true>(a, o0 + tid, sm_proj + tid * SP);
  __syncthreads();
  double* dst = a.juv + o0 * (int64_t)js;
  int r = tid / js, c = tid - r * js;
  const int dr = 128 / js, dcol = 128 - dr * js;
  for (int i = tid; i < n * js; i += 128) {
    dst[i] = sm_proj[r * SP + c];
    r += dr; c += dcol;
    if (c >= js) { c -= js; ++r; }
  }
}

struct FmEvalArgs {
  const double* uv;
  const int64_t* item_patch;
  const int64_t* item_ref;
  const uint8_t* patches; int ph, pw;
  const double* refs;
  int64_t begin, end;
  const int64_t* item_index;
  double* out;
  double* residuals;
  double* desc;
  double* grad = nullptr;
  const uint32_t* res_rect = nullptr;
  unsigned long long* viol_count = nullptr;
  int64_t* viol_list = nullptr;
  long long viol_capacity = 0;
  const unsigned long long* end_dev = nullptr;
  LossParams loss;
  int l2_normalize;
};

__device__ __forceinline__ bool window_resident(uint32_t rect, int row, int col, int ph, int pw) {
  const int r0 = (int)(rect & 255u), c0 = (int)((rect >> 8) & 255u), nr = (int)((rect >> 16) & 255u), ncol = (int)(rect >> 24);
  const int rlo = min(max(row - 1, 0), ph - 1), rhi = min(max(row + 2, 0), ph - 1);
  const int clo = min(max(col - 1, 0), pw - 1), chi = min(max(col + 2, 0), pw - 1);
  return rlo >= r0 && rhi < r0 + nr && clo >= c0 && chi < c0 + ncol;
}

#ifndef PXR_FM_WARPS
#define PXR_FM_WARPS 16
#endif
constexpr int kFmStages = 2;
struct FmAux {
  double xc, xr;
  int64_t item;
  const uint8_t* src;
  int col, row;
};
template <typename T, int C> struct FmCfg {
  static constexpr int kSlot = 16 * C * (int)sizeof(T);
  static constexpr int kWarps = kSlot <= 4096 ? PXR_FM_WARPS : (kSlot <= 8192 ? 8 : (kSlot <= 16384 ? 4 : 2));
  static constexpr int kSmem = kWarps * kFmStages * kSlot + kWarps * kFmStages * 8 + kWarps * 32 * (int)sizeof(FmAux);
};

template <typename T> struct HorizT { typedef float type; };
template <> struct HorizT<double> { typedef double type; };

template <typename T, int CPL>
__device__ __forceinline__ void load_tap(const uint8_t* p, typename HorizT<T>::type v[CPL]);
template <> __device__ __forceinline__ void load_tap<__half, 4>(const uint8_t* p, float v[4]) {
  const uint2 w = *reinterpret_cast<const uint2*>(p);
  const float2 a = __half22float2(*reinterpret_cast<const __half2*>(&w.x));
  const float2 b = __half22float2(*reinterpret_cast<const __half2*>(&w.y));
  v[0] = a.x; v[1] = a.y; v[2] = b.x; v[3] = b.y;
}
template <> __device__ __forceinline__ void load_tap<__half, 2>(const uint8_t* p, float v[2]) {
  const float2 a = __half22float2(*reinterpret_cast<const __half2*>(p));
  v[0] = a.x; v[1] = a.y;
}
template <> __device__ __forceinline__ void load_tap<__half, 1>(const uint8_t* p, float v[1]) {
  v[0] = __half2float(*reinterpret_cast<const __half*>(p));
}
template <> __device__ __forceinline__ void load_tap<__half, 8>(const uint8_t* p, float v[8]) {
  const uint4 w = *reinterpret_cast<const uint4*>(p);
  const uint32_t ws[4] = {w.x, w.y, w.z, w.w};
#pragma unroll
  for (int i = 0; i < 4; ++i) { const float2 a = __half22float2(*reinterpret_cast<const __half2*>(&ws[i])); v[2 * i] = a.x; v[2 * i + 1] = a.y; }
}
template <> __device__ __forceinline__ void load_tap<float, 4>(const uint8_t* p, float v[4]) {
  const float4 w = *reinterpret_cast<const float4*>(p); v[0] = w.x; v[1] = w.y; v[2] = w.z; v[3] = w.w;
}
template <> __device__ __forceinline__ void load_tap<float, 2>(const uint8_t* p, float v[2]) {
  const float2 w = *reinterpret_cast<const float2*>(p); v[0] = w.x; v[1] = w.y;
}
template <> __device__ __forceinline__ void load_tap<float, 1>(const uint8_t* p, float v[1]) { v[0] = *reinterpret_cast<const float*>(p); }
template <> __device__ __forceinline__ void load_tap<float, 8>(const uint8_t* p, float v[8]) {
  load_tap<float, 4>(p, v); load_tap<float, 4>(p + 16, v + 4);
}
template <> __device__ __forceinline__ void load_tap<double, 4>(const uint8_t* p, double v[4]) {
  const double2 a = *reinterpret_cast<const double2*>(p); const double2 b = *reinterpret_cast<const double2*>(p + 16);
  v[0] = a.x; v[1] = a.y; v[2] = b.x; v[3] = b.y;
}
template <> __device__ __forceinline__ void load_tap<double, 2>(const uint8_t* p, double v[2]) {
  const double2 a = *reinterpret_cast<const double2*>(p); v[0] = a.x; v[1] = a.y;
}
template <> __device__ __forceinline__ void load_tap<double, 1>(const uint8_t* p, double v[1]) { v[0] = *reinterpret_cast<const double*>(p); }
template <> __device__ __forceinline__ void load_tap<double, 8>(const uint8_t* p, double v[8]) {
  load_tap<double, 4>(p, v); load_tap<double, 4>(p + 32, v + 4);
}

template <int TAP_BYTES>
struct SmemWindow {
  const uint8_t* win;
  __device__ __forceinline__ const uint8_t* operator()(int i, int j) const { return win + (4 * i + j) * TAP_BYTES; }
};
struct GlobalWindow {
  const uint8_t* rowp[4];
  int coff[4];
  __device__ __forceinline__ const uint8_t* operator()(int i, int j) const { return rowp[i] + coff[j]; }
};

template <typename T, int C, int CPL, bool DERIV, bool FLOAT_SIMD, typename Addr>
__device__ __forceinline__ void bicubic_window(const Addr& addr, int lane, double xc, double xr,
                                               double f[CPL], double fr[CPL], double fc[CPL]) {
  typedef typename HorizT<T>::type H;
  const size_t loff = (size_t)lane * CPL * sizeof(T);
  if (C >= 8) {
    H hf[4][CPL], hd[4][CPL];
#pragma unroll
    for (int i = 0; i < 4; ++i) {
      H p0[CPL], p1[CPL], p2[CPL], p3[CPL];
      load_tap<T, CPL>(addr(i, 0) + loff, p0);
      load_tap<T, CPL>(addr(i, 1) + loff, p1);
      load_tap<T, CPL>(addr(i, 2) + loff, p2);
      load_tap<T, CPL>(addr(i, 3) + loff, p3);
      if (sizeof(H) == 4) {
        const SplineCoefF32 cc(xc);
        if (CPL % 2 == 0) {
#pragma unroll
          for (int k = 0; k < CPL; k += 2) {
            float2 ff, dd = make_float2(0.f, 0.f);
            spline_f32x2<DERIV>(make_float2((float)p0[k], (float)p0[k + 1]), make_float2((float)p1[k], (float)p1[k + 1]),
                                make_float2((float)p2[k], (float)p2[k + 1]), make_float2((float)p3[k], (float)p3[k + 1]), cc, ff, dd);
            hf[i][k] = (H)ff.x; hf[i][k + 1] = (H)ff.y; hd[i][k] = (H)dd.x; hd[i][k + 1] = (H)dd.y;
          }
        } else {
// ... 51 lines not shown
      load_tap<T, CPL>(addr(i, 2) + loff, p2);
      load_tap<T, CPL>(addr(i, 3) + loff, p3);
#pragma unroll
      for (int k = 0; k < CPL; ++k) {
        hd[i][k] = 0.0;
        spline_ceres<DERIV>((double)p0[k], (double)p1[k], (double)p2[k], (double)p3[k], xc, hf[i][k], hd[i][k]);
      }
    }
#pragma unroll
    for (int k = 0; k < CPL; ++k) {
      double dd = 0.0, unused = 0.0;
      spline_ceres<DERIV>(hf[0][k], hf[1][k], hf[2][k], hf[3][k], xr, f[k], dd);
      if (DERIV) { fr[k] = dd; spline_ceres<false>(hd[0][k], hd[1][k], hd[2][k], hd[3][k], xr, fc[k], unused); }
    }
  }
}

template <int CPL, bool DERIV, bool ALLRED>
__device__ __forceinline__ double normalize_and_reduce(bool active, bool l2, const double* refp ,
                                                       double f[CPL], double fr[CPL], double fc[CPL],
                                                       double r[CPL], double red[6], int lane) {
  if (l2) {
    double n2 = 0.0;
    if (active) {
#pragma unroll
      for (int k = 0; k < CPL; ++k) n2 += f[k] * f[k];
    }
    n2 = warp_sum(n2);
    const double ninv = 1.0 / sqrt(n2);
    double dc = 0.0, dr = 0.0;
#pragma unroll
    for (int k = 0; k < CPL; ++k) {
      f[k] *= ninv;
      if (DERIV) { fc[k] *= ninv; fr[k] *= ninv; if (active) { dc += f[k] * fc[k]; dr += f[k] * fr[k]; } }
    }
    if (DERIV) {
      dc = warp_sum(dc); dr = warp_sum(dr);
#pragma unroll
      for (int k = 0; k < CPL; ++k) { fc[k] -= dc * f[k]; fr[k] -= dr * f[k]; }
    }
  }
  double v[8] = {0, 0, 0, 0, 0, 0, 0, 0};
  if (active) {
#pragma unroll
    for (int k = 0; k < CPL; ++k) {
      r[k] = refp ? f[k] - refp[k] : f[k];
      v[0] += r[k] * r[k];
      if (DERIV) {
        v[1] += fc[k] * r[k]; v[2] += fr[k] * r[k];
        v[3] += fc[k] * fc[k]; v[4] += fc[k] * fr[k]; v[5] += fr[k] * fr[k];
      }
    }
  }
  if (!DERIV) { red[0] = warp_sum(v[0]); return red[0]; }
  if (ALLRED) {
#pragma unroll
    for (int k = 0; k < 6; ++k) red[k] = warp_sum(v[k]);
    return red[0];
  }
  return warp_reduce8_transposed(v, lane);
}

template <typename T, int C, int MODE, bool FLOAT_SIMD>
__global__ void __launch_bounds__(FmCfg<T, C>::kWarps * 32, 1) fm_eval_kernel(FmEvalArgs a) {
  constexpr int kFmWarps = FmCfg<T, C>::kWarps;
  constexpr bool DERIV = MODE == 1;
  constexpr int CPL = C >= 32 ? C / 32 : 1;
  constexpr int ACTIVE = C / CPL;
  constexpr int TAP_BYTES = C * (int)sizeof(T);
  constexpr int SLOT_BYTES = 16 * TAP_BYTES;
  static_assert(TAP_BYTES % 16 == 0, "bulk copies need 16-byte multiples");
  extern __shared__ __align__(128) uint8_t smem[];
  const int warp = threadIdx.x >> 5, lane = threadIdx.x & 31;
  uint8_t* wbase = smem + (size_t)warp * kFmStages * SLOT_BYTES;
  uint64_t* bars = reinterpret_cast<uint64_t*>(smem + (size_t)kFmWarps * kFmStages * SLOT_BYTES) + warp * kFmStages;
  FmAux* aux = reinterpret_cast<FmAux*>(smem + (size_t)kFmWarps * kFmStages * SLOT_BYTES + kFmWarps * kFmStages * 8) + warp * 32;
  if (lane == 0) {
#pragma unroll
    for (int s = 0; s < kFmStages; ++s) mbar_init(&bars[s], 1);
    mbar_fence_init();
  }
  __syncwarp();
  const bool active = lane < ACTIVE;
  const int64_t item_end = a.end_dev ? a.begin + (int64_t)*a.end_dev : a.end;
  const int64_t n_items = item_end - a.begin;
  const int64_t n_batches = (n_items + 31) / 32;
  const int64_t warp_global = (int64_t)blockIdx.x * kFmWarps + warp;
  const int64_t warps_total = (int64_t)gridDim.x * kFmWarps;
  uint32_t phase_bits = 0;
  const int64_t patch_bytes = (int64_t)a.ph * a.pw * TAP_BYTES;
  const bool has_ref = a.refs != nullptr;

  for (int64_t batch = warp_global; batch < n_batches; batch += warps_total) {
    const int nvalid = (int)min((int64_t)32, item_end - (a.begin + batch * 32));
    int64_t o = a.begin + batch * 32 + lane;
    if (a.item_index && lane < nvalid) o = a.item_index[o];
    __syncwarp();
    int64_t ref_idx = 0;
    {
      double u = 0.0, v = 0.0;
      int64_t pidx = 0, ridx = 0;
      if (lane < nvalid) {
        u = a.uv[2 * o]; v = a.uv[2 * o + 1];
        pidx = a.item_patch ? a.item_patch[o] : o;
        ridx = a.item_ref ? a.item_ref[o] : o;
      }
      const double fu = floor(u), fv = floor(v);
      FmAux x;
      x.item = o;
      x.col = (int)fmin(fmax(fu, -4.0), (double)a.pw + 4.0);
      x.row = (int)fmin(fmax(fv, -4.0), (double)a.ph + 4.0);
      x.xc = u - fu; x.xr = v - fv;
      x.src = a.patches + pidx * patch_bytes;
      aux[lane] = x;
      ref_idx = ridx;
      if (a.res_rect && lane < nvalid && !window_resident(a.res_rect[pidx], x.row, x.col, a.ph, a.pw)) {
        const unsigned long long slot = atomicAdd(a.viol_count, 1ull);
        if ((long long)slot < a.viol_capacity) a.viol_list[slot] = o;
      }
    }
    __syncwarp();

    auto issue = [&](int j, int slot) {
      const int jc = aux[j].col, jr = aux[j].row;
      const uint8_t* src = aux[j].src;
      uint8_t* dst = wbase + (size_t)slot * SLOT_BYTES;
      if (lane == 0) mbar_expect_tx(&bars[slot], SLOT_BYTES);
      __syncwarp();
      const bool contiguous = (jc - 1 >= 0) && (jc + 2 <= a.pw - 1);
      if (contiguous) {
        if (lane < 4) {
          const int rr = min(max(jr - 1 + lane, 0), a.ph - 1);
          bulk_g2s(dst + lane * 4 * TAP_BYTES, src + ((int64_t)rr * a.pw + (jc - 1)) * TAP_BYTES, 4 * TAP_BYTES, &bars[slot]);
        }
      } else if (lane < 16) {
        const int rr = min(max(jr - 1 + (lane >> 2), 0), a.ph - 1);
        const int cc = min(max(jc - 1 + (lane & 3), 0), a.pw - 1);
        bulk_g2s(dst + lane * TAP_BYTES, src + ((int64_t)rr * a.pw + cc) * TAP_BYTES, TAP_BYTES, &bars[slot]);
      }
    };

#pragma unroll
    for (int s = 0; s < kFmStages; ++s)
      if (s < nvalid) issue(s, s);
    for (int j = 0; j < nvalid; ++j) {
      const int slot = j % kFmStages;
      const double jxc = aux[j].xc, jxr = aux[j].xr;
      double refv[CPL];
      if (has_ref) {
        const int64_t jref = __shfl_sync(0xffffffffu, (long long)ref_idx, j);
        const double* rp = a.refs + jref * C + (active ? lane * CPL : 0);
#pragma unroll
        for (int k = 0; k < CPL; ++k) refv[k] = __ldg(rp + k);
      }
      mbar_wait(&bars[slot], (phase_bits >> slot) & 1u);
      phase_bits ^= (1u << slot);
      double f[CPL], fr[CPL], fc[CPL], r[CPL], red[6];
#pragma unroll
      for (int k = 0; k < CPL; ++k) { f[k] = 0; fr[k] = 0; fc[k] = 0; r[k] = 0; }
      if (active) {
        const SmemWindow<TAP_BYTES> win{wbase + (size_t)slot * SLOT_BYTES};
        bicubic_window<T, C, CPL, DERIV, FLOAT_SIMD>(win, lane, jxc, jxr, f, fr, fc);
      }
      __syncwarp();
      if (j + kFmStages < nvalid) issue(j + kFmStages, slot);
      const double tot = normalize_and_reduce<CPL, DERIV, false>(active, a.l2_normalize != 0, has_ref ? refv : nullptr, f, fr, fc, r, red, lane);
      const int64_t oj = aux[j].item;
      if (a.residuals && active) {
#pragma unroll
        for (int k = 0; k < CPL; ++k) a.residuals[oj * C + lane * CPL + k] = r[k];
      }
      if (a.desc && active) {
#pragma unroll
        for (int k = 0; k < CPL; ++k) a.desc[oj * C + lane * CPL + k] = f[k];
      }
      if (DERIV && a.grad && active) {
#pragma unroll
        for (int k = 0; k < CPL; ++k) {
          a.grad[(oj * 2) * C + lane * CPL + k] = fc[k];
          a.grad[(oj * 2 + 1) * C + lane * CPL + k] = fr[k];
        }
      }
      if (a.out) {
        if (DERIV) {
          const int idx = ((lane >> 4) & 1) * 4 + ((lane >> 3) & 1) * 2 + ((lane >> 2) & 1);
          if ((lane & 3) == 0 && idx < 6) a.out[oj * 8 + idx] = tot;
        } else if (lane == 0) {
          a.out[oj * 8] = tot;
        }
      }
    }
  }
}

static __global__ void __launch_bounds__(256) cost_from_sq_norm_kernel(const double* __restrict__ out, int64_t begin, int64_t end,
                                                                       LossParams loss, double* __restrict__ partials) {
  double acc = 0.0;
  for (int64_t i = begin + (int64_t)blockIdx.x * blockDim.x + threadIdx.x; i < end; i += (int64_t)gridDim.x * blockDim.x) {
    double rho[3];
    loss_eval(loss, 1.0, out[i * 8], rho);
    acc += 0.5 * rho[0];
  }
  __shared__ double sh[8];
  acc = warp_sum(acc);
  if ((threadIdx.x & 31) == 0) sh[threadIdx.x >> 5] = acc;
  __syncthreads();
  if (threadIdx.x == 0) { double t = 0; for (int k = 0; k < 8; ++k) t += sh[k]; partials[blockIdx.x] = t; }
}

}
```

pixel-perfect-sfm_b200/csrc/pxr_fm_small.cuh:

```cuda
#pragma once
#include "pxr_fm_eval.cuh"

namespace pxr {

template <typename T> __device__ __forceinline__ double small_tap(const T* p);
template <> __device__ __forceinline__ double small_tap<__half>(const __half* p) { return (double)__half2float(*p); }
template <> __device__ __forceinline__ double small_tap<float>(const float* p) { return (double)*p; }
template <> __device__ __forceinline__ double small_tap<double>(const double* p) { return *p; }

template <typename T, int C, int MODE>
static __global__ void __launch_bounds__(128) fm_eval_small_kernel(FmEvalArgs a) {
  constexpr bool DERIV = MODE == 1;
  const int64_t k = a.begin + (int64_t)blockIdx.x * blockDim.x + threadIdx.x;
  if (k >= (a.end_dev ? a.begin + (int64_t)*a.end_dev : a.end)) return;
  const int64_t o = a.item_index ? a.item_index[k] : k;
  const double u = a.uv[2 * o], v = a.uv[2 * o + 1];
  const int64_t pidx = a.item_patch ? a.item_patch[o] : o;
  const double fu = floor(u), fv = floor(v);
  const int col = (int)fmin(fmax(fu, -4.0), (double)a.pw + 4.0);
  const int row = (int)fmin(fmax(fv, -4.0), (double)a.ph + 4.0);
  const double xc = u - fu, xr = v - fv;
  const T* src = reinterpret_cast<const T*>(a.patches) + pidx * (int64_t)a.ph * a.pw * C;
  int cc[4], rr[4];
#pragma unroll
  for (int i = 0; i < 4; ++i) {
    cc[i] = min(max(col - 1 + i, 0), a.pw - 1);
    rr[i] = min(max(row - 1 + i, 0), a.ph - 1);
  }
  double f[C], fr[C], fc[C];
#pragma unroll
  for (int ch = 0; ch < C; ++ch) {
    double fi[4], di[4];
#pragma unroll
    for (int i = 0; i < 4; ++i) {
      const T* rowp = src + (int64_t)rr[i] * a.pw * C + ch;
      const double p0 = small_tap<T>(rowp + cc[0] * C), p1 = small_tap<T>(rowp + cc[1] * C);
      const double p2 = small_tap<T>(rowp + cc[2] * C), p3 = small_tap<T>(rowp + cc[3] * C);
      double dd = 0.0;
      spline_ceres<DERIV>(p0, p1, p2, p3, xc, fi[i], dd);
      di[i] = dd;
    }
    double d0 = 0.0, d1 = 0.0;
    spline_ceres<DERIV>(fi[0], fi[1], fi[2], fi[3], xr, f[ch], d0);
    fr[ch] = d0;
    if (DERIV) { double g; spline_ceres<false>(di[0], di[1], di[2], di[3], xr, g, d1); fc[ch] = g; } else fc[ch] = 0.0;
  }
  if (a.l2_normalize) {
    double n2 = 0.0;
#pragma unroll
    for (int ch = 0; ch < C; ++ch) n2 += f[ch] * f[ch];
    const double ninv = 1.0 / sqrt(n2);
    double dc = 0.0, dr = 0.0;
#pragma unroll
    for (int ch = 0; ch < C; ++ch) { f[ch] *= ninv; if (DERIV) { fc[ch] *= ninv; fr[ch] *= ninv; } }
    if (DERIV) {
#pragma unroll
      for (int ch = 0; ch < C; ++ch) { dc += f[ch] * fc[ch]; dr += f[ch] * fr[ch]; }
#pragma unroll
      for (int ch = 0; ch < C; ++ch) { fc[ch] -= dc * f[ch]; fr[ch] -= dr * f[ch]; }
    }
  }
  const int64_t ridx = a.item_ref ? a.item_ref[o] : o;
  double s = 0, bu = 0, bv = 0, auu = 0, auv = 0, avv = 0;
#pragma unroll
  for (int ch = 0; ch < C; ++ch) {
    const double r = a.refs ? f[ch] - a.refs[ridx * C + ch] : f[ch];
    if (a.residuals) a.residuals[o * C + ch] = r;
    if (a.desc) a.desc[o * C + ch] = f[ch];
    if (DERIV && a.grad) { a.grad[(o * 2) * C + ch] = fc[ch]; a.grad[(o * 2 + 1) * C + ch] = fr[ch]; }
    s += r * r;
    if (DERIV) { bu += fc[ch] * r; bv += fr[ch] * r; auu += fc[ch] * fc[ch]; auv += fc[ch] * fr[ch]; avv += fr[ch] * fr[ch]; }
  }
  if (a.out) {
    double* op = a.out + o * 8;
    op[0] = s;
    if (DERIV) { op[1] = bu; op[2] = bv; op[3] = auu; op[4] = auv; op[5] = avv; }
  }
}

template <typename T> struct DiffT;
template <> struct DiffT<__half> {
  static __device__ __forceinline__ double diff(__half a, __half b) { return (double)__half2float(__float2half_rn(__half2float(a) - __half2float(b))); }
  static __device__ __forceinline__ double val(__half a) { return (double)__half2float(a); }
};
template <> struct DiffT<float> {
  static __device__ __forceinline__ double diff(float a, float b) { return (double)__fsub_rn(a, b); }
  static __device__ __forceinline__ double val(float a) { return (double)a; }
};
template <> struct DiffT<double> {
  static __device__ __forceinline__ double diff(double a, double b) { return __dsub_rn(a, b); }
  static __device__ __forceinline__ double val(double a) { return a; }
};
template <typename TO> __device__ __forceinline__ TO costmap_cast(double v);
template <> __device__ __forceinline__ __half costmap_cast<__half>(double v) { return __float2half_rn(__double2float_rn(v)); }
template <> __device__ __forceinline__ float costmap_cast<float>(double v) { return (float)v; }
template <> __device__ __forceinline__ double costmap_cast<double>(double v) { return v; }

struct CostmapArgs {
  const uint8_t* patches; int ph, pw, C;
  const double* refs;
  const int64_t* item_patch;
  const int64_t* item_ref;
  int64_t n_items;
  uint8_t* out; int OC;
  LossParams loss;
  int as_gradientfield, apply_sqrt;
};

template <typename T, typename TO>
static __global__ void __launch_bounds__(256) costmap_extract_kernel(CostmapArgs a) {
  const int lane = threadIdx.x & 31;
  const int64_t wid = ((int64_t)blockIdx.x * blockDim.x + threadIdx.x) >> 5;
  const int64_t px_per = (int64_t)a.ph * a.pw;
  if (wid >= a.n_items * px_per) return;
  const int64_t item = wid / px_per;
  const int pix = (int)(wid % px_per);
  const int y = pix / a.pw, x = pix % a.pw;
  const int64_t pidx = a.item_patch ? a.item_patch[item] : item;
  const int C = a.C;
  const T* src = reinterpret_cast<const T*>(a.patches) + pidx * px_per * C;
  const double* ref = a.refs + a.item_ref[item] * C;
  const int top = min(a.ph - 1, y + 1), bottom = max(0, y - 1);
  const int right = min(a.pw - 1, x + 1), left = max(0, x - 1);
  const T* pc = src + ((int64_t)y * a.pw + x) * C;
  const T* pt = src + ((int64_t)top * a.pw + x) * C;
  const T* pb = src + ((int64_t)bottom * a.pw + x) * C;
  const T* pr = src + ((int64_t)y * a.pw + right) * C;
  const T* pl = src + ((int64_t)y * a.pw + left) * C;
  double s = 0.0, dr = 0.0, dc = 0.0;
  for (int ch = lane; ch < C; ch += 32) {
    const double r = DiffT<T>::val(pc[ch]) - ref[ch];
    s += r * r;
    if (a.as_gradientfield) {
      dr += r * (DiffT<T>::diff(pt[ch], pb[ch]) * 0.5);
      dc += r * (DiffT<T>::diff(pr[ch], pl[ch]) * 0.5);
    }
  }
  s = warp_sum(s); dr = warp_sum(dr); dc = warp_sum(dc);
  if (lane != 0) return;
  double rho[3];
  loss_eval(a.loss, 1.0, s, rho);
  double cost = rho[0] * 0.5;
  double dcostdr = 0.0, dcostdc = 0.0;
  TO* op = reinterpret_cast<TO*>(a.out) + (pidx * px_per + pix) * a.OC;
  if (a.as_gradientfield) {
    if (cost > 1.0e-8) {
      dcostdr = rho[1] * dr;
      dcostdc = rho[1] * dc;
      if (a.apply_sqrt) {
        cost = sqrt(cost);
        dcostdr *= 0.5 / cost;
        dcostdc *= 0.5 / cost;
      }
    }
    op[0] = costmap_cast<TO>(cost); op[1] = costmap_cast<TO>(dcostdr); op[2] = costmap_cast<TO>(dcostdc);
  } else {
    if (a.apply_sqrt) cost = sqrt(cost);
    op[0] = costmap_cast<TO>(cost);
  }
// ... 4 lines not shown
```

pixel-perfect-sfm_b200/csrc/pxr_inner.cu:

```cuda
#include "pxr_ba_host.h"

namespace pxr {

template <typename T, int C>
static int launch_inner_tc(pxr_ctx* ctx, bool fs, const InnerArgs& a) {
  const unsigned grid = (unsigned)cdiv(a.n_points * 32, 128);
  if (fs) PXR_LAUNCH(ctx, (ba_inner_kernel<T, C, true>), grid, 128, 0, a);
  else PXR_LAUNCH(ctx, (ba_inner_kernel<T, C, false>), grid, 128, 0, a);
  PXR_CUDA(cudaGetLastError());
  return PXR_OK;
}

int launch_inner(pxr_ctx* ctx, int dtype, int C, bool float_simd, const InnerArgs& a) {
#define PXR_CASE(T, CC) \
  if (C == CC) return launch_inner_tc<T, CC>(ctx, float_simd, a);
  if (dtype == PXR_F16) {
    PXR_CASE(__half, 128) PXR_CASE(__half, 64) PXR_CASE(__half, 32) PXR_CASE(__half, 16) PXR_CASE(__half, 8)
    PXR_CASE(__half, 256)
  } else if (dtype == PXR_F32) {
    PXR_CASE(float, 128) PXR_CASE(float, 64) PXR_CASE(float, 16)
  } else if (dtype == PXR_F64) {
    PXR_CASE(double, 128) PXR_CASE(double, 16)
  }
#undef PXR_CASE
  return fail(PXR_ERR_UNSUPPORTED, "Unsupported dimensions (CHANNELS=%d, dtype=%d, N_NODES=1).", C, dtype);
}

}
```

pixel-perfect-sfm_b200/csrc/pxr_inner.cuh:

```cuda
#pragma once
#include "pxr_ba_kernels.cuh"
#include "pxr_fm_eval.cuh"

namespace pxr {

struct InnerArgs {
  int64_t n_points;
  const int64_t* point_off; const int64_t* pt_begin;
  const int32_t* obs_img; const int64_t* obs_patch;
  const int32_t* img_cam; const int32_t* cam_model;
  const double* cam_params; const double* qvec; const double* tvec;
  double* xyz;
  const int32_t* corner; const double* scale; double ups;
  const uint8_t* patches; int ph, pw;
  const double* refs;
  LossParams loss;
  int l2_normalize;
};

struct PointEval { double cost, H[6], g[3]; };

template <typename T, int C, bool FS>
__device__ __forceinline__ void inner_eval(const InnerArgs& a, int64_t p, int lane, const double X[3], PointEval& e) {
  constexpr int CPL = C >= 32 ? C / 32 : 1;
  constexpr int ACTIVE = C / CPL;
  constexpr int TAP_BYTES = C * (int)sizeof(T);
  const bool active = lane < ACTIVE;
  const int64_t ob = a.pt_begin[p], oe = a.pt_begin[p + 1];
  double cost = 0, H0 = 0, H1 = 0, H2 = 0, H3 = 0, H4 = 0, H5 = 0, g0 = 0, g1 = 0, g2 = 0;
  double refv[CPL];
  if (a.refs && active) {
#pragma unroll
    for (int k = 0; k < CPL; ++k) refv[k] = __ldg(a.refs + p * C + lane * CPL + k);
  }
  for (int64_t base = ob; base < oe; base += 32) {
    const int cnt = (int)min((int64_t)32, oe - base);
    double u = 0, v = 0, Jp[2][3] = {{0, 0, 0}, {0, 0, 0}};
    const uint8_t* pbase = a.patches;
    if (lane < cnt) {
      const int64_t o = base + lane;
      const int img = a.obs_img[o];
      const int64_t pi = a.obs_patch ? a.obs_patch[o] : o;
      const int cam = a.img_cam[img];
      double q[4], t[3], cp[kMaxK], xy[2], Jpose[2][6], Jk[2][kMaxK];
#pragma unroll
      for (int i = 0; i < 4; ++i) q[i] = a.qvec[4 * (int64_t)img + i];
#pragma unroll
      for (int i = 0; i < 3; ++i) t[i] = a.tvec[3 * (int64_t)img + i];
#pragma unroll
      for (int i = 0; i < kMaxK; ++i) cp[i] = a.cam_params[(int64_t)cam * kMaxK + i];
      world_to_pixel<true>(a.cam_model[cam], cp, q, t, X, xy, Jpose, Jp, Jk);
      const double sx = a.scale[2 * pi] * a.ups, sy = a.scale[2 * pi + 1] * a.ups;
      u = (xy[0] * a.scale[2 * pi] - 0.5 - (double)a.corner[2 * pi]) * a.ups;
      v = (xy[1] * a.scale[2 * pi + 1] - 0.5 - (double)a.corner[2 * pi + 1]) * a.ups;
#pragma unroll
      for (int k = 0; k < 3; ++k) { Jp[0][k] *= sx; Jp[1][k] *= sy; }
      pbase = a.patches + pi * (int64_t)a.ph * a.pw * TAP_BYTES;
    }
    const double fu = floor(u), fv = floor(v);
    const int col = (int)fmin(fmax(fu, -4.0), (double)a.pw + 4.0);
    const int row = (int)fmin(fmax(fv, -4.0), (double)a.ph + 4.0);
    const double xc = u - fu, xr = v - fv;
    double my_red[6] = {0, 0, 0, 0, 0, 0};
    for (int j = 0; j < cnt; ++j) {
      const int jc = __shfl_sync(0xffffffffu, col, j);
      const int jr = __shfl_sync(0xffffffffu, row, j);
      const double jxc = __shfl_sync(0xffffffffu, xc, j);
      const double jxr = __shfl_sync(0xffffffffu, xr, j);
      const uint8_t* src = reinterpret_cast<const uint8_t*>((uintptr_t)__shfl_sync(0xffffffffu, (unsigned long long)(uintptr_t)pbase, j));
      GlobalWindow win;
#pragma unroll
      for (int i = 0; i < 4; ++i) {
        const int rr = min(max(jr - 1 + i, 0), a.ph - 1);
        win.rowp[i] = src + (int64_t)rr * a.pw * TAP_BYTES;
        win.coff[i] = min(max(jc - 1 + i, 0), a.pw - 1) * TAP_BYTES;
      }
      double f[CPL], fr[CPL], fc[CPL], r[CPL], red[6];
#pragma unroll
      for (int k = 0; k < CPL; ++k) { f[k] = 0; fr[k] = 0; fc[k] = 0; r[k] = 0; }
      if (active) bicubic_window<T, C, CPL, true, FS>(win, lane, jxc, jxr, f, fr, fc);
      normalize_and_reduce<CPL, true, true>(active, a.l2_normalize != 0, a.refs ? refv : nullptr, f, fr, fc, r, red, lane);
      if (lane == j) {
#pragma unroll
        for (int k = 0; k < 6; ++k) my_red[k] = red[k];
      }
    }
    if (lane < cnt) {
      double rho[3];
      loss_eval(a.loss, 1.0, my_red[0], rho);
      cost += 0.5 * rho[0];
      const double bu = rho[1] * my_red[1], bv = rho[1] * my_red[2];
      const double auu = rho[1] * my_red[3], auv = rho[1] * my_red[4], avv = rho[1] * my_red[5];
      double apu[3], apv[3];
#pragma unroll
      for (int k = 0; k < 3; ++k) { apu[k] = auu * Jp[0][k] + auv * Jp[1][k]; apv[k] = auv * Jp[0][k] + avv * Jp[1][k]; }
      H0 += Jp[0][0] * apu[0] + Jp[1][0] * apv[0];
      H1 += Jp[0][0] * apu[1] + Jp[1][0] * apv[1];
      H2 += Jp[0][0] * apu[2] + Jp[1][0] * apv[2];
      H3 += Jp[0][1] * apu[1] + Jp[1][1] * apv[1];
      H4 += Jp[0][1] * apu[2] + Jp[1][1] * apv[2];
      H5 += Jp[0][2] * apu[2] + Jp[1][2] * apv[2];
      g0 += Jp[0][0] * bu + Jp[1][0] * bv;
      g1 += Jp[0][1] * bu + Jp[1][1] * bv;
      g2 += Jp[0][2] * bu + Jp[1][2] * bv;
    }
  }
  e.cost = warp_sum(cost);
  e.H[0] = warp_sum(H0); e.H[1] = warp_sum(H1); e.H[2] = warp_sum(H2);
  e.H[3] = warp_sum(H3); e.H[4] = warp_sum(H4); e.H[5] = warp_sum(H5);
  e.g[0] = warp_sum(g0); e.g[1] = warp_sum(g1); e.g[2] = warp_sum(g2);
}

template <typename T, int C, bool FS>
__global__ void __launch_bounds__(128) ba_inner_kernel(InnerArgs a) {
  const int64_t p = ((int64_t)blockIdx.x * blockDim.x + threadIdx.x) >> 5;
  const int lane = threadIdx.x & 31;
  if (p >= a.n_points || a.point_off[p] < 0) return;
  if (a.pt_begin[p + 1] == a.pt_begin[p]) return;
  const int max_iter = 50, max_invalid = 5;
  const double ftol = 1e-6, gtol = 1e-10, ptol = 1e-8, min_rel_dec = 1e-3;
  const double max_radius = 1e16, min_radius = 1e-32, min_diag = 1e-6, max_diag = 1e32;
  double x[3] = {a.xyz[3 * p], a.xyz[3 * p + 1], a.xyz[3 * p + 2]};
  PointEval cur;
  inner_eval<T, C, FS>(a, p, lane, x, cur);
  if (!isfinite(cur.cost)) return;
  double sc[3];
  sc[0] = 1.0 / (1.0 + sqrt(cur.H[0])); sc[1] = 1.0 / (1.0 + sqrt(cur.H[3])); sc[2] = 1.0 / (1.0 + sqrt(cur.H[5]));
  double radius = 1e4, decrease_factor = 2.0;
  double x_cost = cur.cost, current_cost = cur.cost;
  double x_norm = sqrt(x[0] * x[0] + x[1] * x[1] + x[2] * x[2]);
  double gmax = fmax(fabs(cur.g[0]), fmax(fabs(cur.g[1]), fabs(cur.g[2])));
  int num_invalid = 0;
  for (int iter = 1;; ++iter) {
    if (iter - 1 >= max_iter) break;
    if (gmax <= gtol) break;
    if (radius < min_radius) break;
    const double diag[3] = {cur.H[0], cur.H[3], cur.H[5]};
    double D2[3];
#pragma unroll
    for (int k = 0; k < 3; ++k) {
      const double s2 = sc[k] * sc[k];
      D2[k] = fmin(fmax(diag[k] * s2, min_diag), max_diag) / (radius * s2);
    }
    const double Hf[9] = {cur.H[0], cur.H[1], cur.H[2], cur.H[1], cur.H[3], cur.H[4], cur.H[2], cur.H[4], cur.H[5]};
    double inv[9];
    bool valid = inv3_sym(Hf, D2, inv);
    double d[3] = {0, 0, 0}, mcc = 0;
    if (valid) {
#pragma unroll
      for (int k = 0; k < 3; ++k) d[k] = -(inv[k * 3] * cur.g[0] + inv[k * 3 + 1] * cur.g[1] + inv[k * 3 + 2] * cur.g[2]);
      double gd = 0, dHd = 0;
#pragma unroll
      for (int k = 0; k < 3; ++k) {
        gd += cur.g[k] * d[k];
        dHd += d[k] * (Hf[k * 3] * d[0] + Hf[k * 3 + 1] * d[1] + Hf[k * 3 + 2] * d[2]);
      }
      mcc = -gd - 0.5 * dHd;
      valid = isfinite(d[0]) && isfinite(d[1]) && isfinite(d[2]) && mcc > 0.0;
    }
    if (!valid) {
      if (++num_invalid >= max_invalid) break;
      radius /= decrease_factor; decrease_factor *= 2.0;
      continue;
    }
    num_invalid = 0;
    const double xc_[3] = {x[0] + d[0], x[1] + d[1], x[2] + d[2]};
    PointEval cand;
    inner_eval<T, C, FS>(a, p, lane, xc_, cand);
    const double candidate_cost = isfinite(cand.cost) ? cand.cost : 1.7976931348623157e308;
    const double step_norm = sqrt((xc_[0] - x[0]) * (xc_[0] - x[0]) + (xc_[1] - x[1]) * (xc_[1] - x[1]) + (xc_[2] - x[2]) * (xc_[2] - x[2]));
    if (step_norm <= ptol * (x_norm + ptol)) break;
    const double cost_change = x_cost - candidate_cost;
    if (fabs(cost_change) <= ftol * x_cost) break;
    const double rel = (current_cost - candidate_cost) / mcc;
    if (rel > min_rel_dec) {
      x[0] = xc_[0]; x[1] = xc_[1]; x[2] = xc_[2];
      x_norm = sqrt(x[0] * x[0] + x[1] * x[1] + x[2] * x[2]);
      cur = cand; x_cost = cand.cost; current_cost = candidate_cost;
      gmax = fmax(fabs(cur.g[0]), fmax(fabs(cur.g[1]), fabs(cur.g[2])));
      radius = radius / fmax(1.0 / 3.0, 1.0 - pow(2.0 * rel - 1.0, 3.0));
      radius = fmin(max_radius, radius);
      decrease_factor = 2.0;
    } else {
      radius /= decrease_factor; decrease_factor *= 2.0;
    }
  }
  if (lane == 0) { a.xyz[3 * p] = x[0]; a.xyz[3 * p + 1] = x[1]; a.xyz[3 * p + 2] = x[2]; }
}

struct InnerState {
  double x[3];
  double cand[3];
  double cost, current_cost, H[6], g[3], sc[3];
  double radius, decf, xnorm, gmax, mcc;
  int iter, invalid, active;
};

struct InnerStepArgs {
  int64_t n_points;
  const int64_t* point_off; const int64_t* pt_begin;
  const double* obs_out; const double* juv; int juv_stride; int juv_w;
  double* xyz;
  InnerState* st;
  LossParams loss;
  int64_t* list;
  unsigned long long* counters;
};

__device__ __forceinline__ bool inner_propose(InnerState& s) {
  const int max_iter = 50, max_invalid = 5;
  const double gtol = 1e-10, min_radius = 1e-32, min_diag = 1e-6, max_diag = 1e32;
  for (;;) {
    s.iter += 1;
    if (s.iter - 1 >= max_iter) return false;
    if (s.gmax <= gtol) return false;
    if (s.radius < min_radius) return false;
    const double diag[3] = {s.H[0], s.H[3], s.H[5]};
    double D2[3];
#pragma unroll
    for (int k = 0; k < 3; ++k) {
      const double s2 = s.sc[k] * s.sc[k];
      D2[k] = fmin(fmax(diag[k] * s2, min_diag), max_diag) / (s.radius * s2);
    }
    const double Hf[9] = {s.H[0], s.H[1], s.H[2], s.H[1], s.H[3], s.H[4], s.H[2], s.H[4], s.H[5]};
    double inv[9];
    bool valid = inv3_sym(Hf, D2, inv);
    double d[3] = {0, 0, 0}, mcc = 0;
    if (valid) {
#pragma unroll
      for (int k = 0; k < 3; ++k) d[k] = -(inv[k * 3] * s.g[0] + inv[k * 3 + 1] * s.g[1] + inv[k * 3 + 2] * s.g[2]);
      double gd = 0, dHd = 0;
#pragma unroll
      for (int k = 0; k < 3; ++k) {
        gd += s.g[k] * d[k];
        dHd += d[k] * (Hf[k * 3] * d[0] + Hf[k * 3 + 1] * d[1] + Hf[k * 3 + 2] * d[2]);
      }
      mcc = -gd - 0.5 * dHd;
      valid = isfinite(d[0]) && isfinite(d[1]) && isfinite(d[2]) && mcc > 0.0;
    }
    if (!valid) {
      if (++s.invalid >= max_invalid) return false;
      s.radius /= s.decf; s.decf *= 2.0;
      continue;
    }
    s.invalid = 0;
    s.mcc = mcc;
#pragma unroll
    for (int k = 0; k < 3; ++k) s.cand[k] = s.x[k] + d[k];
    return true;
  }
}

static __global__ void __launch_bounds__(128) inner_step_kernel(InnerStepArgs a, int phase) {
  const int64_t p = (int64_t)blockIdx.x * blockDim.x + threadIdx.x;
  if (p >= a.n_points) return;
  InnerState s = a.st[p];
  if (phase == 0) {
    s.active = (a.point_off[p] >= 0 && a.pt_begin[p + 1] > a.pt_begin[p]) ? 1 : 0;
    s.iter = 0; s.invalid = 0;
    if (!s.active) { a.st[p] = s; return; }
#pragma unroll
    for (int k = 0; k < 3; ++k) s.x[k] = a.xyz[3 * p + k];
  } else if (!s.active) return;
  double cost = 0, H[6] = {0, 0, 0, 0, 0, 0}, g[3] = {0, 0, 0};
  for (int64_t o = a.pt_begin[p]; o < a.pt_begin[p + 1]; ++o) {
    const double* oo = a.obs_out + o * 8;
    double rho[3];
    loss_eval(a.loss, 1.0, oo[0], rho);
    cost += 0.5 * rho[0];
    const double bu = rho[1] * oo[1], bv = rho[1] * oo[2];
    const double auu = rho[1] * oo[3], auv = rho[1] * oo[4], avv = rho[1] * oo[5];
    const double* J = a.juv + o * (int64_t)a.juv_stride;
    const double pu[3] = {J[6], J[7], J[8]}, pv[3] = {J[a.juv_w + 6], J[a.juv_w + 7], J[a.juv_w + 8]};
    double apu[3], apv[3];
#pragma unroll
    for (int k = 0; k < 3; ++k) { apu[k] = auu * pu[k] + auv * pv[k]; apv[k] = auv * pu[k] + avv * pv[k]; }
    H[0] += pu[0] * apu[0] + pv[0] * apv[0];
    H[1] += pu[0] * apu[1] + pv[0] * apv[1];
    H[2] += pu[0] * apu[2] + pv[0] * apv[2];
    H[3] += pu[1] * apu[1] + pv[1] * apv[1];
    H[4] += pu[1] * apu[2] + pv[1] * apv[2];
    H[5] += pu[2] * apu[2] + pv[2] * apv[2];
#pragma unroll
    for (int k = 0; k < 3; ++k) g[k] += pu[k] * bu + pv[k] * bv;
  }
  const double ftol = 1e-6, ptol = 1e-8, min_rel_dec = 1e-3, max_radius = 1e16;
  bool go = true;
  if (phase == 0) {
    if (!isfinite(cost)) go = false;
    s.cost = s.current_cost = cost;
#pragma unroll
    for (int k = 0; k < 6; ++k) s.H[k] = H[k];
#pragma unroll
    for (int k = 0; k < 3; ++k) s.g[k] = g[k];
    s.sc[0] = 1.0 / (1.0 + sqrt(H[0])); s.sc[1] = 1.0 / (1.0 + sqrt(H[3])); s.sc[2] = 1.0 / (1.0 + sqrt(H[5]));
    s.radius = 1e4; s.decf = 2.0;
    s.xnorm = sqrt(s.x[0] * s.x[0] + s.x[1] * s.x[1] + s.x[2] * s.x[2]);
    s.gmax = fmax(fabs(g[0]), fmax(fabs(g[1]), fabs(g[2])));
  } else {
    const double candidate_cost = isfinite(cost) ? cost : 1.7976931348623157e308;
    const double dx = s.cand[0] - s.x[0], dy = s.cand[1] - s.x[1], dz = s.cand[2] - s.x[2];
    const double step_norm = sqrt(dx * dx + dy * dy + dz * dz);
    if (step_norm <= ptol * (s.xnorm + ptol)) go = false;
    else if (fabs(s.cost - candidate_cost) <= ftol * s.cost) go = false;
    else {
      const double rel = (s.current_cost - candidate_cost) / s.mcc;
      if (rel > min_rel_dec) {
#pragma unroll
        for (int k = 0; k < 3; ++k) { s.x[k] = s.cand[k]; s.g[k] = g[k]; }
#pragma unroll
        for (int k = 0; k < 6; ++k) s.H[k] = H[k];
        s.xnorm = sqrt(s.x[0] * s.x[0] + s.x[1] * s.x[1] + s.x[2] * s.x[2]);
        s.cost = cost; s.current_cost = candidate_cost;
        s.gmax = fmax(fabs(g[0]), fmax(fabs(g[1]), fabs(g[2])));
        s.radius = s.radius / fmax(1.0 / 3.0, 1.0 - pow(2.0 * rel - 1.0, 3.0));
        s.radius = fmin(max_radius, s.radius);
        s.decf = 2.0;
      } else {
        s.radius /= s.decf; s.decf *= 2.0;
      }
    }
  }
  if (go) go = inner_propose(s);
  if (go) {
#pragma unroll
    for (int k = 0; k < 3; ++k) a.xyz[3 * p + k] = s.cand[k];
  } else {
    s.active = 0;
#pragma unroll
    for (int k = 0; k < 3; ++k) a.xyz[3 * p + k] = s.x[k];
  }
  a.st[p] = s;
}

static __global__ void __launch_bounds__(128) inner_list_kernel(InnerStepArgs a, int all_variable) {
  const int64_t p = (int64_t)blockIdx.x * blockDim.x + threadIdx.x;
  if (p >= a.n_points) return;
  const bool act = all_variable ? (a.point_off[p] >= 0 && a.pt_begin[p + 1] > a.pt_begin[p]) : (a.st[p].active != 0);
  if (!act) return;
  const int64_t ob = a.pt_begin[p], n = a.pt_begin[p + 1] - ob;
  const unsigned long long base = atomicAdd(&a.counters[0], (unsigned long long)n);
  atomicAdd(&a.counters[1], 1ull);
  for (int64_t i = 0; i < n; ++i) a.list[base + i] = ob + i;
}

static __global__ void __launch_bounds__(256) diff_norm_kernel(const double* a, const double* b, int64_t n, double* acc, double* part = nullptr) {
  const int64_t i = (int64_t)blockIdx.x * blockDim.x + threadIdx.x;
  double v = 0.0;
  if (i < n) { const double d = a[i] - b[i]; v = d * d; }
  __shared__ double sh[8];
  v = warp_sum(v);
  if ((threadIdx.x & 31) == 0) sh[threadIdx.x >> 5] = v;
  __syncthreads();
  if (threadIdx.x == 0) {
    double s = 0; for (int k = 0; k < 8; ++k) s += sh[k];
    if (part) part[blockIdx.x] = s;
    else atomicAdd(acc, s);
  }
}

static __global__ void ba_add_reduced_kernel(const double* Hcc, const double* gc, const double* D2, double* S,
                                      double* rhs, int nc) {
  const int64_t i = (int64_t)blockIdx.x * blockDim.x + threadIdx.x;
  const int64_t n2 = (int64_t)nc * nc;
  if (i < n2) {
    const int r = (int)(i / nc), c = (int)(i % nc);
    double v = c <= r ? Hcc[i] : 0.0;
    if (r == c) v += D2[r];
    S[i] += v;
  }
  if (i < nc) rhs[i] -= gc[i];
}

}
```

Baseline: 144.4 million.

## Replace host-driven batched inner point iterations with a persistent fused device kernel

Replaces the host-loop of up to 53 rounds (list build, projection, feature-metric eval, step kernel, event polling) with one persistent kernel. Blocks claim points via an atomic counter and run projection, bicubic evaluation and the per-point LM step in shared-memory slots. This removes per-round launches, memsets and host polling, and drops the redundant re-projection before the cost evaluation after inner iterations. In exchange there are per-observation record buffers and __syncthreads barriers each iteration, so load imbalance between slots can leave warps idle.

Measured after the change: 158.4 million (median of 6 runs). 1.1x the previous value.

```diff
diff --git a/pixel-perfect-sfm_b200/build.py b/pixel-perfect-sfm_b200/build.py
--- a/pixel-perfect-sfm_b200/build.py
+++ b/pixel-perfect-sfm_b200/build.py
@@ -5,7 +5,7 @@
 
 HERE = os.path.dirname(os.path.abspath(__file__))
 CSRC = os.path.join(HERE, "csrc")
-SOURCES = ["pxr_api.cu", "pxr_upload.cu", "pxr_ba.cu", "pxr_ba_block.cu", "pxr_inner.cu", "pxr_refs.cu", "pxr_ka.cu", "pxr_synth.cu", "pxr_extract.cu", "pxr_problem.cu"]
+SOURCES = ["pxr_api.cu", "pxr_upload.cu", "pxr_ba.cu", "pxr_ba_block.cu", "pxr_refs.cu", "pxr_ka.cu", "pxr_synth.cu", "pxr_extract.cu", "pxr_problem.cu"]
 NVCC = os.environ.get("NVCC", "/usr/local/cuda/bin/nvcc")
 FLAGS = ["-gencode", "arch=compute_100a,code=sm_100a", "-lineinfo", "-O3", "-std=c++17",
          "-Xcompiler", "-fPIC", "-ccbin", "/usr/bin/g++", "--expt-relaxed-constexpr",
diff --git a/pixel-perfect-sfm_b200/csrc/pxr_ba.cu b/pixel-perfect-sfm_b200/csrc/pxr_ba.cu
--- a/pixel-perfect-sfm_b200/csrc/pxr_ba.cu
+++ b/pixel-perfect-sfm_b200/csrc/pxr_ba.cu
@@ -71,6 +71,44 @@
 #undef PXR_SMALL
 #define PXR_CASE(T, CC) \
   if (C == CC) return launch_fm_tc<T, CC>(ctx, a, mode, float_simd, np);
+  if (dtype == PXR_F16) {
+    PXR_CASE(__half, 128) PXR_CASE(__half, 64) PXR_CASE(__half, 32) PXR_CASE(__half, 16) PXR_CASE(__half, 8)
+    PXR_CASE(__half, 256)
+  } else if (dtype == PXR_F32) {
+    PXR_CASE(float, 128) PXR_CASE(float, 64) PXR_CASE(float, 16)
+  } else if (dtype == PXR_F64) {
+    PXR_CASE(double, 128) PXR_CASE(double, 16)
+  }
+#undef PXR_CASE
+  return fail(PXR_ERR_UNSUPPORTED, "Unsupported dimensions (CHANNELS=%d, dtype=%d, N_NODES=1).", C, dtype);
+}
+
+template <typename T, int C, bool FS>
+static int launch_inner_k(pxr_ctx* ctx, const InnerArgs& a) {
+  typedef InnerCfg<T, C> Cfg;
+  auto kern = inner_fused_kernel<T, C, FS>;
+  static bool attr_set = false;
+  if (!attr_set) {
+    PXR_CUDA(cudaFuncSetAttribute(kern, cudaFuncAttributeMaxDynamicSharedMemorySize, Cfg::kSmem));
+    attr_set = true;
+  }
+  const int64_t grid = std::max<int64_t>(1, std::min<int64_t>((int64_t)ctx->sm_count * 2, cdiv(a.n_points, kInnerSlots)));
+  PXR_LAUNCH(ctx, kern, (unsigned)grid, Cfg::kWarps * 32, Cfg::kSmem, a);
+  PXR_CUDA(cudaGetLastError());
+  return PXR_OK;
+}
+
+int launch_inner_fused(pxr_ctx* ctx, int dtype, int C, bool float_simd, const InnerArgs& a) {
+#define PXR_SMALL(T) \
+  { if (C == 3) return launch_inner_k<T, 3, false>(ctx, a); if (C == 4) return launch_inner_k<T, 4, false>(ctx, a); \
+    if (C == 1) return launch_inner_k<T, 1, false>(ctx, a); }
+  if (C < 8) {
+    if (dtype == PXR_F16) PXR_SMALL(__half) else if (dtype == PXR_F32) PXR_SMALL(float) else if (dtype == PXR_F64) PXR_SMALL(double)
+    return fail(PXR_ERR_UNSUPPORTED, "Unsupported dimensions (CHANNELS=%d, dtype=%d, N_NODES=1).", C, dtype);
+  }
+#undef PXR_SMALL
+#define PXR_CASE(T, CC) \
+  if (C == CC) return float_simd ? launch_inner_k<T, CC, true>(ctx, a) : launch_inner_k<T, CC, false>(ctx, a);
   if (dtype == PXR_F16) {
     PXR_CASE(__half, 128) PXR_CASE(__half, 64) PXR_CASE(__half, 32) PXR_CASE(__half, 16) PXR_CASE(__half, 8)
     PXR_CASE(__half, 256)
@@ -264,7 +302,6 @@
   PXR_TRY(gc.alloc(nc));
   PXR_TRY(Hpp.alloc((size_t)n_points * 9)); PXR_TRY(gp.alloc((size_t)n_points * 3));
   h_obs_img.assign(d->obs_img, d->obs_img + n_obs);
-  use_monolithic_inner = std::getenv("PXR_INNER_MONOLITHIC") != nullptr;
   if (for_solve) PXR_TRY(build_schur_pairs());
   if (block_mode) PXR_TRY(block_setup());
   if (for_solve && n_obs > 0 && n_obs < ((int64_t)1 << 31)) {
@@ -448,7 +485,6 @@
   const int W = res_window;
   if (W < 4 || C < 8 || ph > 255 || pw > 255 || ph < W + 2 || pw < W + 2) return PXR_OK;
   if ((size_t)ph * pw * C * esz > staged_chunk_bytes()) return PXR_OK;
-  if (getenv("PXR_INNER_MONOLITHIC")) return PXR_OK;
   auto is_device = [](const void* ptr) -> bool {
     cudaPointerAttributes pa;
     if (cudaPointerGetAttributes(&pa, ptr) != cudaSuccess) { cudaGetLastError(); return false; }
@@ -595,6 +631,10 @@
   PXR_TRY(project(set, jac, nullptr));
   PXR_TRY(fm(jac ? 1 : 0, nullptr, scalars.p + 0));
   if (jac) PXR_TRY(build());
+  return read_cost(cost_out);
+}
+
+int BA::read_cost(double* cost_out) {
   if (block_mode) return global_cost_block(cost_out);
   PXR_TRY(allreduce_f64(ctx, scalars.p + 0, 1));
   double c = 0;
@@ -887,108 +927,41 @@
   return PXR_OK;
 }
 
-int BA::eval_list(int set, const int64_t* list, int64_t n, const unsigned long long* n_dev, bool settle) {
-  if (n <= 0) return PXR_OK;
-  ProjectArgs pa;
-  pa.obs_img = obs_img.p; pa.obs_pt = obs_pt.p; pa.obs_patch = obs_patch.p;
-  pa.img_cam = img_cam.p; pa.cam_model = cam_model.p;
-  pa.cam_params = cam[set].p; pa.qvec = q[set].p; pa.tvec = t[set].p; pa.xyz = X[set].p;
-  pa.corner = corner.p; pa.scale = scale.p; pa.ups = ups;
-  pa.obs_begin = 0; pa.obs_end = n; pa.item_index = list; pa.n_dev = n_dev;
-  pa.uv = uv.p; pa.xy = nullptr; pa.juv = juv.p; pa.juv_stride = juv_stride; pa.juv_k = K;
-  PXR_LAUNCH(ctx, ba_project_kernel<true>, (unsigned)cdiv(n, 128), 128, 0, pa);
-  FmEvalArgs a;
-  a.uv = uv.p; a.item_patch = obs_patch.p; a.item_ref = obs_pt.p;
-  a.patches = d_patches; a.ph = ph; a.pw = pw;
-  a.refs = has_refs ? refs.p : nullptr;
-  a.begin = 0; a.end = n; a.item_index = list; a.end_dev = n_dev;
-  a.out = obs_out.p; a.residuals = nullptr; a.desc = nullptr;
-  a.loss.type = opt.loss_type; a.loss.a = opt.loss_scale;
-  a.l2_normalize = interp.l2_normalize;
-  resident_args(a);
-  int np = 0;
-  PXR_TRY(launch_fm_eval(ctx, dtype, C, 1, interp.use_float_simd != 0, a, &np));
-  if (!settle) return PXR_OK;
-  for (;;) {
-    int64_t n_fixed = 0;
-    PXR_TRY(resident_fix(&n_fixed));
-    if (n_fixed == 0) break;
-    a.item_index = res_fix_list.p; a.begin = 0; a.end = n_fixed; a.end_dev = nullptr;
-    PXR_TRY(launch_fm_eval(ctx, dtype, C, 1, interp.use_float_simd != 0, a, &np));
-  }
-  return PXR_OK;
-}
-
-constexpr int kInnerRounds = 53;
-int BA::inner_rounds(int set) {
-  cudaStream_t s = ctx->stream;
-  InnerStepArgs a;
-  a.n_points = n_points; a.point_off = point_off.p; a.pt_begin = pt_begin.p;
-  a.obs_out = obs_out.p; a.juv = juv.p; a.juv_stride = juv_stride; a.juv_w = 9 + K;
-  a.xyz = X[set].p; a.st = inner_state.p;
-  a.loss.type = opt.loss_type; a.loss.a = opt.loss_scale;
-  a.list = inner_list.p; a.counters = inner_counters.p;
-  const unsigned pgrid = (unsigned)cdiv(n_points, 128);
-  for (int round = 0; round < kInnerRounds; ++round) {
-    if (round >= 2) {
-      const cudaError_t q = cudaEventQuery(inner_events[round - 2]);
-      if (q == cudaSuccess) { if (inner_cnt_host[2 * (round - 2)] == 0) break; }
-      else if (q != cudaErrorNotReady) PXR_CUDA(q);
-      else if ((void)cudaGetLastError(), round >= 8 && (round & 3) == 0) {
-        PXR_CUDA(cudaEventSynchronize(inner_events[round - 2]));
-        if (inner_cnt_host[2 * (round - 2)] == 0) break;
-      }
-    }
-    PXR_CUDA(cudaMemsetAsync(inner_counters.p, 0, 2 * sizeof(unsigned long long), s));
-    PXR_LAUNCH(ctx, inner_list_kernel, pgrid, 128, 0, a, round == 0 ? 1 : 0);
-    PXR_CUDA(cudaMemcpyAsync(inner_cnt_host + 2 * round, inner_counters.p, 2 * sizeof(unsigned long long), cudaMemcpyDeviceToHost, s));
-    PXR_CUDA(cudaEventRecord(inner_events[round], s));
-    PXR_TRY(eval_list(set, inner_list.p, n_obs, inner_counters.p, false));
-    PXR_LAUNCH(ctx, inner_step_kernel, pgrid, 128, 0, a, round == 0 ? 0 : 1);
-  }
-  PXR_CUDA(cudaGetLastError());
-  return PXR_OK;
-}
-
-int BA::inner_iterations_batched(int set) {
+int BA::inner_iterations(int set) {
   if (n_points == 0 || n_obs == 0) return PXR_OK;
   StageScope stg(this, 9);
   cudaStream_t s = ctx->stream;
-  if (!inner_state.p) {
-    PXR_TRY(inner_state.alloc(n_points));
-    PXR_TRY(inner_list.alloc(n_obs));
-    PXR_TRY(inner_counters.alloc(2));
-    PXR_CUDA(cudaHostAlloc((void**)&inner_cnt_host, (size_t)kInnerRounds * 2 * sizeof(unsigned long long), cudaHostAllocDefault));
-    inner_events.resize(kInnerRounds, nullptr);
-    for (auto& e : inner_events) PXR_CUDA(cudaEventCreateWithFlags(&e, cudaEventDisableTiming));
-  }
-  if (!resident) return inner_rounds(set);
-  if (!inner_snapshot.p) PXR_TRY(inner_snapshot.alloc((size_t)n_points * 3));
-  PXR_CUDA(cudaMemcpyAsync(inner_snapshot.p, X[set].p, (size_t)n_points * 24, cudaMemcpyDeviceToDevice, s));
+  if (!inner_rec.p) { PXR_TRY(inner_rec.alloc((size_t)n_obs * kInnerRec)); PXR_TRY(inner_next.alloc(1)); }
+  InnerArgs a;
+  a.n_points = n_points; a.point_off = point_off.p; a.pt_begin = pt_begin.p;
+  a.geo.obs_img = obs_img.p; a.geo.obs_pt = obs_pt.p; a.geo.obs_patch = obs_patch.p;
+  a.geo.img_cam = img_cam.p; a.geo.cam_model = cam_model.p;
+  a.geo.cam_params = cam[set].p; a.geo.qvec = q[set].p; a.geo.tvec = t[set].p; a.geo.xyz = X[set].p;
+  a.geo.corner = corner.p; a.geo.scale = scale.p; a.geo.ups = ups;
+  a.geo.obs_begin = 0; a.geo.obs_end = n_obs; a.geo.item_index = nullptr;
+  a.geo.uv = nullptr; a.geo.xy = nullptr; a.geo.juv = nullptr; a.geo.juv_stride = juv_stride; a.geo.juv_k = K;
+  a.fm.uv = nullptr; a.fm.item_patch = obs_patch.p; a.fm.item_ref = obs_pt.p;
+  a.fm.patches = d_patches; a.fm.ph = ph; a.fm.pw = pw;
+  a.fm.refs = has_refs ? refs.p : nullptr;
+  a.fm.begin = 0; a.fm.end = n_obs; a.fm.item_index = nullptr;
+  a.fm.out = obs_out.p; a.fm.residuals = nullptr; a.fm.desc = nullptr;
+  a.fm.loss.type = opt.loss_type; a.fm.loss.a = opt.loss_scale;
+  a.fm.l2_normalize = interp.l2_normalize;
+  resident_args(a.fm);
+  a.xyz = X[set].p; a.rec = inner_rec.p; a.next_point = inner_next.p;
+  if (resident) {
+    if (!inner_snapshot.p) PXR_TRY(inner_snapshot.alloc((size_t)n_points * 3));
+    PXR_CUDA(cudaMemcpyAsync(inner_snapshot.p, X[set].p, (size_t)n_points * 24, cudaMemcpyDeviceToDevice, s));
+  }
   for (;;) {
-    PXR_TRY(inner_rounds(set));
+    PXR_CUDA(cudaMemsetAsync(inner_next.p, 0, sizeof(unsigned long long), s));
+    PXR_TRY(launch_inner_fused(ctx, dtype, C, interp.use_float_simd != 0, a));
     int64_t n_fixed = 0;
     PXR_TRY(resident_fix(&n_fixed));
     if (n_fixed == 0) break;
     PXR_CUDA(cudaMemcpyAsync(X[set].p, inner_snapshot.p, (size_t)n_points * 24, cudaMemcpyDeviceToDevice, s));
   }
   return PXR_OK;
-}
-
-int BA::inner_iterations(int set) {
-  if (!use_monolithic_inner) return inner_iterations_batched(set);
-  InnerArgs a;
-  a.n_points = n_points; a.point_off = point_off.p; a.pt_begin = pt_begin.p;
-  a.obs_img = obs_img.p; a.obs_patch = obs_patch.p; a.img_cam = img_cam.p; a.cam_model = cam_model.p;
-  a.cam_params = cam[set].p; a.qvec = q[set].p; a.tvec = t[set].p; a.xyz = X[set].p;
-  a.corner = corner.p; a.scale = scale.p; a.ups = ups;
-  a.patches = d_patches; a.ph = ph; a.pw = pw;
-  a.refs = has_refs ? refs.p : nullptr;
-  a.loss.type = opt.loss_type; a.loss.a = opt.loss_scale;
-  a.l2_normalize = interp.l2_normalize;
-  if (n_points == 0) return PXR_OK;
-  StageScope st(this, 9);
-  return launch_inner(ctx, dtype, C, interp.use_float_simd != 0, a);
 }
 
 int BA::step_norm_between_sets(double* out) {
@@ -1244,7 +1217,8 @@
       ++lm.n_inner;
       rc = inner_iterations(1 - cur);
       double inner_cost = 0;
-      if (rc == PXR_OK) rc = evaluate(1 - cur, false, &inner_cost);
+      if (rc == PXR_OK) rc = fm_cost(scalars.p + 0);
+      if (rc == PXR_OK) rc = read_cost(&inner_cost);
       if (rc != PXR_OK) { swap_sets(); return rc; }
       if (std::isfinite(inner_cost)) {
         model_cost_change += candidate_cost - inner_cost;
diff --git a/pixel-perfect-sfm_b200/csrc/pxr_ba_block.cu b/pixel-perfect-sfm_b200/csrc/pxr_ba_block.cu
--- a/pixel-perfect-sfm_b200/csrc/pxr_ba_block.cu
+++ b/pixel-perfect-sfm_b200/csrc/pxr_ba_block.cu
@@ -519,8 +519,7 @@
     PXR_LAUNCH(ctx, blk_pack_scalars_kernel, 1, 1, 0, scalars.p, flags.p, mb_in.p, 1, ctx->rank == 0 ? 1 : 0, 0);
     if (ran_inner) {
       rc = inner_iterations(1 - cur);
-      if (rc == PXR_OK) rc = project(1 - cur, false, nullptr);
-      if (rc == PXR_OK) rc = fm(0, nullptr, scalars.p + 0);
+      if (rc == PXR_OK) rc = fm_cost(scalars.p + 0);
       if (rc != PXR_OK) { swap_sets(); return rc; }
       PXR_CUDA(cudaMemsetAsync(scalars.p + 11, 0, 16, s));
       auto run = [&](const double* a, const double* b, int64_t n, double* acc) {
diff --git a/pixel-perfect-sfm_b200/csrc/pxr_ba_host.h b/pixel-perfect-sfm_b200/csrc/pxr_ba_host.h
--- a/pixel-perfect-sfm_b200/csrc/pxr_ba_host.h
+++ b/pixel-perfect-sfm_b200/csrc/pxr_ba_host.h
@@ -24,7 +24,7 @@
 int fm_supported(int dtype, int C);
 int fm_max_partials(pxr_ctx* ctx);
 int launch_fm_eval(pxr_ctx* ctx, int dtype, int C, int mode, bool float_simd, const FmEvalArgs& a, int* n_partials);
-int launch_inner(pxr_ctx* ctx, int dtype, int C, bool float_simd, const InnerArgs& a);
+int launch_inner_fused(pxr_ctx* ctx, int dtype, int C, bool float_simd, const InnerArgs& a);
 
 struct StepEvaluator {
   int max_nonmonotonic = 0, num_consecutive_nonmonotonic_steps = 0;
@@ -156,7 +156,7 @@
   DevBuf<int64_t> io_chunk_begin; int64_t io_n_chunks = 0;
   DevBuf<long long> chol_trace;
   DevBuf<int> chol_sync;
-  ~BA() { if (inner_cnt_host) cudaFreeHost(inner_cnt_host); for (auto e : inner_events) cudaEventDestroy(e); if (res_thread.joinable()) res_thread.join(); if (chol_graph_exec) cudaGraphExecDestroy(chol_graph_exec); for (int k = 0; k < kNumStages; ++k) for (auto& pr : timed[k]) { cudaEventDestroy(pr.first); cudaEventDestroy(pr.second); } }
+  ~BA() { if (res_thread.joinable()) res_thread.join(); if (chol_graph_exec) cudaGraphExecDestroy(chol_graph_exec); for (int k = 0; k < kNumStages; ++k) for (auto& pr : timed[k]) { cudaEventDestroy(pr.first); cudaEventDestroy(pr.second); } }
   DevBuf<int32_t> sp_px, sp_py, sp_pp;
   DevBuf<int64_t> sp_chunk_begin;
   DevBuf<uint8_t> sp_chunk_self;
@@ -194,21 +194,15 @@
   int fm_cost(double* cost_dev);
   int build();
   int evaluate(int set, bool jac, double* cost_out);
+  int read_cost(double* cost_out);
   int compute_step(double radius, bool* valid, double* model_cost_change);
   int chol_launch();
   int apply_step(double* step_norm, double* x_norm);
   int gradient_max_norm(double* out);
   int inner_iterations(int set);
-  int inner_iterations_batched(int set);
-  int eval_list(int set, const int64_t* list, int64_t n, const unsigned long long* n_dev = nullptr, bool settle = true);
-  int inner_rounds(int set);
-  unsigned long long* inner_cnt_host = nullptr;
-  std::vector<cudaEvent_t> inner_events;
+  DevBuf<double> inner_rec;
+  DevBuf<unsigned long long> inner_next;
   DevBuf<double> inner_snapshot;
-  DevBuf<InnerState> inner_state;
-  DevBuf<int64_t> inner_list;
-  DevBuf<unsigned long long> inner_counters;
-  bool use_monolithic_inner = false;
   int step_norm_between_sets(double* out);
   int lm_begin();
   bool lm_finalize(int max_iteration);
diff --git a/pixel-perfect-sfm_b200/csrc/pxr_fm_eval.cuh b/pixel-perfect-sfm_b200/csrc/pxr_fm_eval.cuh
--- a/pixel-perfect-sfm_b200/csrc/pxr_fm_eval.cuh
+++ b/pixel-perfect-sfm_b200/csrc/pxr_fm_eval.cuh
@@ -10,7 +10,6 @@
   const int32_t* corner; const double* scale; double ups;
   int64_t obs_begin, obs_end;
   const int64_t* item_index;
-  const unsigned long long* n_dev = nullptr;
   double* uv;
   double* xy;
   double* juv;
@@ -19,29 +18,39 @@
 };
 
 template <bool JAC>
-__device__ __forceinline__ void project_observation(const ProjectArgs& a, int64_t o, double* out) {
+__device__ __forceinline__ void observe(const ProjectArgs& a, int64_t o, const double X[3], double uv[2], double xy[2],
+                                        double sc[2], double Jpose[2][6], double Jpt[2][3], double Jk[2][kMaxK]) {
   const int img = a.obs_img[o];
-  const int64_t pt = a.obs_pt[o];
   const int64_t pi = a.obs_patch ? a.obs_patch[o] : o;
   const int cam = a.img_cam[img];
   const int model = a.cam_model[cam];
-  double q[4], t[3], X[3], cp[kMaxK];
+  double q[4], t[3], cp[kMaxK];
 #pragma unroll
   for (int i = 0; i < 4; ++i) q[i] = a.qvec[4 * (int64_t)img + i];
 #pragma unroll
-  for (int i = 0; i < 3; ++i) { t[i] = a.tvec[3 * (int64_t)img + i]; X[i] = a.xyz[3 * pt + i]; }
+  for (int i = 0; i < 3; ++i) t[i] = a.tvec[3 * (int64_t)img + i];
 #pragma unroll
   for (int i = 0; i < kMaxK; ++i) cp[i] = a.cam_params[(int64_t)cam * kMaxK + i];
-  double xy[2], Jpose[2][6], Jpt[2][3], Jk[2][kMaxK];
   world_to_pixel<JAC>(model, cp, q, t, X, xy, Jpose, Jpt, Jk);
   const double sx = a.scale[2 * pi], sy = a.scale[2 * pi + 1];
   const double cx = (double)a.corner[2 * pi], cy = (double)a.corner[2 * pi + 1];
-  a.uv[2 * o] = (xy[0] * sx - 0.5 - cx) * a.ups;
-  a.uv[2 * o + 1] = (xy[1] * sy - 0.5 - cy) * a.ups;
+  uv[0] = (xy[0] * sx - 0.5 - cx) * a.ups;
+  uv[1] = (xy[1] * sy - 0.5 - cy) * a.ups;
+  sc[0] = sx * a.ups; sc[1] = sy * a.ups;
+}
+
+template <bool JAC>
+__device__ __forceinline__ void project_observation(const ProjectArgs& a, int64_t o, double* out) {
+  const int64_t pt = a.obs_pt[o];
+  double X[3], uv[2], xy[2], s[2], Jpose[2][6], Jpt[2][3], Jk[2][kMaxK];
+#pragma unroll
+  for (int i = 0; i < 3; ++i) X[i] = a.xyz[3 * pt + i];
+  observe<JAC>(a, o, X, uv, xy, s, Jpose, Jpt, Jk);
+  a.uv[2 * o] = uv[0];
+  a.uv[2 * o + 1] = uv[1];
   if (a.xy) { a.xy[2 * o] = xy[0]; a.xy[2 * o + 1] = xy[1]; }
   if (JAC && out) {
     const int W = 9 + a.juv_k;
-    const double s[2] = {sx * a.ups, sy * a.ups};
 #pragma unroll
     for (int r = 0; r < 2; ++r) {
 #pragma unroll
@@ -56,8 +65,7 @@
 template <bool JAC>
 __global__ void __launch_bounds__(128) ba_project_kernel(ProjectArgs a) {
   const int64_t k = a.obs_begin + (int64_t)blockIdx.x * blockDim.x + threadIdx.x;
-  const int64_t end = a.n_dev ? a.obs_begin + (int64_t)*a.n_dev : a.obs_end;
-  if (k >= end) return;
+  if (k >= a.obs_end) return;
   const int64_t o = a.item_index ? a.item_index[k] : k;
   project_observation<JAC>(a, o, (JAC && a.juv) ? a.juv + o * (int64_t)a.juv_stride : nullptr);
 }
@@ -96,7 +104,6 @@
   unsigned long long* viol_count = nullptr;
   int64_t* viol_list = nullptr;
   long long viol_capacity = 0;
-  const unsigned long long* end_dev = nullptr;
   LossParams loss;
   int l2_normalize;
 };
@@ -123,6 +130,35 @@
   static constexpr int kWarps = kSlot <= 4096 ? PXR_FM_WARPS : (kSlot <= 8192 ? 8 : (kSlot <= 16384 ? 4 : 2));
   static constexpr int kSmem = kWarps * kFmStages * kSlot + kWarps * kFmStages * 8 + kWarps * 32 * (int)sizeof(FmAux);
 };
+
+template <int TAP_BYTES>
+__device__ __forceinline__ void issue_window(const FmAux& x, uint8_t* dst, uint64_t* bar, int ph, int pw, int lane) {
+  const int jc = x.col, jr = x.row;
+  if (lane == 0) mbar_expect_tx(bar, 16 * TAP_BYTES);
+  __syncwarp();
+  const bool contiguous = (jc - 1 >= 0) && (jc + 2 <= pw - 1);
+  if (contiguous) {
+    if (lane < 4) {
+      const int rr = min(max(jr - 1 + lane, 0), ph - 1);
+      bulk_g2s(dst + lane * 4 * TAP_BYTES, x.src + ((int64_t)rr * pw + (jc - 1)) * TAP_BYTES, 4 * TAP_BYTES, bar);
+    }
+  } else if (lane < 16) {
+    const int rr = min(max(jr - 1 + (lane >> 2), 0), ph - 1);
+    const int cc = min(max(jc - 1 + (lane & 3), 0), pw - 1);
+    bulk_g2s(dst + lane * TAP_BYTES, x.src + ((int64_t)rr * pw + cc) * TAP_BYTES, TAP_BYTES, bar);
+  }
+}
+
+__device__ __forceinline__ FmAux window_geometry(double u, double v, const uint8_t* src, int64_t item, int ph, int pw) {
+  const double fu = floor(u), fv = floor(v);
+  FmAux x;
+  x.item = item;
+  x.col = (int)fmin(fmax(fu, -4.0), (double)pw + 4.0);
+  x.row = (int)fmin(fmax(fv, -4.0), (double)ph + 4.0);
+  x.xc = u - fu; x.xr = v - fv;
+  x.src = src;
+  return x;
+}
 
 template <typename T> struct HorizT { typedef float type; };
 template <> struct HorizT<double> { typedef double type; };
@@ -340,7 +376,7 @@
   }
   __syncwarp();
   const bool active = lane < ACTIVE;
-  const int64_t item_end = a.end_dev ? a.begin + (int64_t)*a.end_dev : a.end;
+  const int64_t item_end = a.end;
   const int64_t n_items = item_end - a.begin;
   const int64_t n_batches = (n_items + 31) / 32;
   const int64_t warp_global = (int64_t)blockIdx.x * kFmWarps + warp;
@@ -363,13 +399,7 @@
         pidx = a.item_patch ? a.item_patch[o] : o;
         ridx = a.item_ref ? a.item_ref[o] : o;
       }
-      const double fu = floor(u), fv = floor(v);
-      FmAux x;
-      x.item = o;
-      x.col = (int)fmin(fmax(fu, -4.0), (double)a.pw + 4.0);
-      x.row = (int)fmin(fmax(fv, -4.0), (double)a.ph + 4.0);
-      x.xc = u - fu; x.xr = v - fv;
-      x.src = a.patches + pidx * patch_bytes;
+      const FmAux x = window_geometry(u, v, a.patches + pidx * patch_bytes, o, a.ph, a.pw);
       aux[lane] = x;
       ref_idx = ridx;
       if (a.res_rect && lane < nvalid && !window_resident(a.res_rect[pidx], x.row, x.col, a.ph, a.pw)) {
@@ -380,22 +410,7 @@
     __syncwarp();
 
     auto issue = [&](int j, int slot) {
-      const int jc = aux[j].col, jr = aux[j].row;
-      const uint8_t* src = aux[j].src;
-      uint8_t* dst = wbase + (size_t)slot * SLOT_BYTES;
-      if (lane == 0) mbar_expect_tx(&bars[slot], SLOT_BYTES);
-      __syncwarp();
-      const bool contiguous = (jc - 1 >= 0) && (jc + 2 <= a.pw - 1);
-      if (contiguous) {
-        if (lane < 4) {
-          const int rr = min(max(jr - 1 + lane, 0), a.ph - 1);
-          bulk_g2s(dst + lane * 4 * TAP_BYTES, src + ((int64_t)rr * a.pw + (jc - 1)) * TAP_BYTES, 4 * TAP_BYTES, &bars[slot]);
-        }
-      } else if (lane < 16) {
-        const int rr = min(max(jr - 1 + (lane >> 2), 0), a.ph - 1);
-        const int cc = min(max(jc - 1 + (lane & 3), 0), a.pw - 1);
-        bulk_g2s(dst + lane * TAP_BYTES, src + ((int64_t)rr * a.pw + cc) * TAP_BYTES, TAP_BYTES, &bars[slot]);
-      }
+      issue_window<TAP_BYTES>(aux[j], wbase + (size_t)slot * SLOT_BYTES, &bars[slot], a.ph, a.pw, lane);
     };
 
 #pragma unroll
diff --git a/pixel-perfect-sfm_b200/csrc/pxr_fm_small.cuh b/pixel-perfect-sfm_b200/csrc/pxr_fm_small.cuh
--- a/pixel-perfect-sfm_b200/csrc/pxr_fm_small.cuh
+++ b/pixel-perfect-sfm_b200/csrc/pxr_fm_small.cuh
@@ -8,13 +8,8 @@
 template <> __device__ __forceinline__ double small_tap<float>(const float* p) { return (double)*p; }
 template <> __device__ __forceinline__ double small_tap<double>(const double* p) { return *p; }
 
-template <typename T, int C, int MODE>
-static __global__ void __launch_bounds__(128) fm_eval_small_kernel(FmEvalArgs a) {
-  constexpr bool DERIV = MODE == 1;
-  const int64_t k = a.begin + (int64_t)blockIdx.x * blockDim.x + threadIdx.x;
-  if (k >= (a.end_dev ? a.begin + (int64_t)*a.end_dev : a.end)) return;
-  const int64_t o = a.item_index ? a.item_index[k] : k;
-  const double u = a.uv[2 * o], v = a.uv[2 * o + 1];
+template <typename T, int C, bool DERIV>
+__device__ __forceinline__ void fm_small_item(const FmEvalArgs& a, int64_t o, double u, double v, double red[6]) {
   const int64_t pidx = a.item_patch ? a.item_patch[o] : o;
   const double fu = floor(u), fv = floor(v);
   const int col = (int)fmin(fmax(fu, -4.0), (double)a.pw + 4.0);
@@ -71,10 +66,22 @@
     s += r * r;
     if (DERIV) { bu += fc[ch] * r; bv += fr[ch] * r; auu += fc[ch] * fc[ch]; auv += fc[ch] * fr[ch]; avv += fr[ch] * fr[ch]; }
   }
+  red[0] = s;
+  if (DERIV) { red[1] = bu; red[2] = bv; red[3] = auu; red[4] = auv; red[5] = avv; }
+}
+
+template <typename T, int C, int MODE>
+static __global__ void __launch_bounds__(128) fm_eval_small_kernel(FmEvalArgs a) {
+  constexpr bool DERIV = MODE == 1;
+  const int64_t k = a.begin + (int64_t)blockIdx.x * blockDim.x + threadIdx.x;
+  if (k >= a.end) return;
+  const int64_t o = a.item_index ? a.item_index[k] : k;
+  double red[6];
+  fm_small_item<T, C, DERIV>(a, o, a.uv[2 * o], a.uv[2 * o + 1], red);
   if (a.out) {
     double* op = a.out + o * 8;
-    op[0] = s;
-    if (DERIV) { op[1] = bu; op[2] = bv; op[3] = auu; op[4] = auv; op[5] = avv; }
+    op[0] = red[0];
+    if (DERIV) { op[1] = red[1]; op[2] = red[2]; op[3] = red[3]; op[4] = red[4]; op[5] = red[5]; }
   }
 }
 
diff --git a/pixel-perfect-sfm_b200/csrc/pxr_inner.cu b/pixel-perfect-sfm_b200/csrc/pxr_inner.cu
--- a/pixel-perfect-sfm_b200/csrc/pxr_inner.cu
+++ /dev/null
@@ -1,29 +0,0 @@
-#include "pxr_ba_host.h"
-
-namespace pxr {
-
-template <typename T, int C>
-static int launch_inner_tc(pxr_ctx* ctx, bool fs, const InnerArgs& a) {
-  const unsigned grid = (unsigned)cdiv(a.n_points * 32, 128);
-  if (fs) PXR_LAUNCH(ctx, (ba_inner_kernel<T, C, true>), grid, 128, 0, a);
-  else PXR_LAUNCH(ctx, (ba_inner_kernel<T, C, false>), grid, 128, 0, a);
-  PXR_CUDA(cudaGetLastError());
-  return PXR_OK;
-}
-
-int launch_inner(pxr_ctx* ctx, int dtype, int C, bool float_simd, const InnerArgs& a) {
-#define PXR_CASE(T, CC) \
-  if (C == CC) return launch_inner_tc<T, CC>(ctx, float_simd, a);
-  if (dtype == PXR_F16) {
-    PXR_CASE(__half, 128) PXR_CASE(__half, 64) PXR_CASE(__half, 32) PXR_CASE(__half, 16) PXR_CASE(__half, 8)
-    PXR_CASE(__half, 256)
-  } else if (dtype == PXR_F32) {
-    PXR_CASE(float, 128) PXR_CASE(float, 64) PXR_CASE(float, 16)
-  } else if (dtype == PXR_F64) {
-    PXR_CASE(double, 128) PXR_CASE(double, 16)
-  }
-#undef PXR_CASE
-  return fail(PXR_ERR_UNSUPPORTED, "Unsupported dimensions (CHANNELS=%d, dtype=%d, N_NODES=1).", C, dtype);
-}
-
-}
diff --git a/pixel-perfect-sfm_b200/csrc/pxr_inner.cuh b/pixel-perfect-sfm_b200/csrc/pxr_inner.cuh
--- a/pixel-perfect-sfm_b200/csrc/pxr_inner.cuh
+++ b/pixel-perfect-sfm_b200/csrc/pxr_inner.cuh
@@ -1,210 +1,16 @@
 #pragma once
 #include "pxr_ba_kernels.cuh"
 #include "pxr_fm_eval.cuh"
+#include "pxr_fm_small.cuh"
 
 namespace pxr {
-
-struct InnerArgs {
-  int64_t n_points;
-  const int64_t* point_off; const int64_t* pt_begin;
-  const int32_t* obs_img; const int64_t* obs_patch;
-  const int32_t* img_cam; const int32_t* cam_model;
-  const double* cam_params; const double* qvec; const double* tvec;
-  double* xyz;
-  const int32_t* corner; const double* scale; double ups;
-  const uint8_t* patches; int ph, pw;
-  const double* refs;
-  LossParams loss;
-  int l2_normalize;
-};
-
-struct PointEval { double cost, H[6], g[3]; };
-
-template <typename T, int C, bool FS>
-__device__ __forceinline__ void inner_eval(const InnerArgs& a, int64_t p, int lane, const double X[3], PointEval& e) {
-  constexpr int CPL = C >= 32 ? C / 32 : 1;
-  constexpr int ACTIVE = C / CPL;
-  constexpr int TAP_BYTES = C * (int)sizeof(T);
-  const bool active = lane < ACTIVE;
-  const int64_t ob = a.pt_begin[p], oe = a.pt_begin[p + 1];
-  double cost = 0, H0 = 0, H1 = 0, H2 = 0, H3 = 0, H4 = 0, H5 = 0, g0 = 0, g1 = 0, g2 = 0;
-  double refv[CPL];
-  if (a.refs && active) {
-#pragma unroll
-    for (int k = 0; k < CPL; ++k) refv[k] = __ldg(a.refs + p * C + lane * CPL + k);
-  }
-  for (int64_t base = ob; base < oe; base += 32) {
-    const int cnt = (int)min((int64_t)32, oe - base);
-    double u = 0, v = 0, Jp[2][3] = {{0, 0, 0}, {0, 0, 0}};
-    const uint8_t* pbase = a.patches;
-    if (lane < cnt) {
-      const int64_t o = base + lane;
-      const int img = a.obs_img[o];
-      const int64_t pi = a.obs_patch ? a.obs_patch[o] : o;
-      const int cam = a.img_cam[img];
-      double q[4], t[3], cp[kMaxK], xy[2], Jpose[2][6], Jk[2][kMaxK];
-#pragma unroll
-      for (int i = 0; i < 4; ++i) q[i] = a.qvec[4 * (int64_t)img + i];
-#pragma unroll
-      for (int i = 0; i < 3; ++i) t[i] = a.tvec[3 * (int64_t)img + i];
-#pragma unroll
-      for (int i = 0; i < kMaxK; ++i) cp[i] = a.cam_params[(int64_t)cam * kMaxK + i];
-      world_to_pixel<true>(a.cam_model[cam], cp, q, t, X, xy, Jpose, Jp, Jk);
-      const double sx = a.scale[2 * pi] * a.ups, sy = a.scale[2 * pi + 1] * a.ups;
-      u = (xy[0] * a.scale[2 * pi] - 0.5 - (double)a.corner[2 * pi]) * a.ups;
-      v = (xy[1] * a.scale[2 * pi + 1] - 0.5 - (double)a.corner[2 * pi + 1]) * a.ups;
-#pragma unroll
-      for (int k = 0; k < 3; ++k) { Jp[0][k] *= sx; Jp[1][k] *= sy; }
-      pbase = a.patches + pi * (int64_t)a.ph * a.pw * TAP_BYTES;
-    }
-    const double fu = floor(u), fv = floor(v);
-    const int col = (int)fmin(fmax(fu, -4.0), (double)a.pw + 4.0);
-    const int row = (int)fmin(fmax(fv, -4.0), (double)a.ph + 4.0);
-    const double xc = u - fu, xr = v - fv;
-    double my_red[6] = {0, 0, 0, 0, 0, 0};
-    for (int j = 0; j < cnt; ++j) {
-      const int jc = __shfl_sync(0xffffffffu, col, j);
-      const int jr = __shfl_sync(0xffffffffu, row, j);
-      const double jxc = __shfl_sync(0xffffffffu, xc, j);
-      const double jxr = __shfl_sync(0xffffffffu, xr, j);
-      const uint8_t* src = reinterpret_cast<const uint8_t*>((uintptr_t)__shfl_sync(0xffffffffu, (unsigned long long)(uintptr_t)pbase, j));
-      GlobalWindow win;
-#pragma unroll
-      for (int i = 0; i < 4; ++i) {
-        const int rr = min(max(jr - 1 + i, 0), a.ph - 1);
-        win.rowp[i] = src + (int64_t)rr * a.pw * TAP_BYTES;
-        win.coff[i] = min(max(jc - 1 + i, 0), a.pw - 1) * TAP_BYTES;
-      }
-      double f[CPL], fr[CPL], fc[CPL], r[CPL], red[6];
-#pragma unroll
-      for (int k = 0; k < CPL; ++k) { f[k] = 0; fr[k] = 0; fc[k] = 0; r[k] = 0; }
-      if (active) bicubic_window<T, C, CPL, true, FS>(win, lane, jxc, jxr, f, fr, fc);
-      normalize_and_reduce<CPL, true, true>(active, a.l2_normalize != 0, a.refs ? refv : nullptr, f, fr, fc, r, red, lane);
-      if (lane == j) {
-#pragma unroll
-        for (int k = 0; k < 6; ++k) my_red[k] = red[k];
-      }
-    }
-    if (lane < cnt) {
-      double rho[3];
-      loss_eval(a.loss, 1.0, my_red[0], rho);
-      cost += 0.5 * rho[0];
-      const double bu = rho[1] * my_red[1], bv = rho[1] * my_red[2];
-      const double auu = rho[1] * my_red[3], auv = rho[1] * my_red[4], avv = rho[1] * my_red[5];
-      double apu[3], apv[3];
-#pragma unroll
-      for (int k = 0; k < 3; ++k) { apu[k] = auu * Jp[0][k] + auv * Jp[1][k]; apv[k] = auv * Jp[0][k] + avv * Jp[1][k]; }
-      H0 += Jp[0][0] * apu[0] + Jp[1][0] * apv[0];
-      H1 += Jp[0][0] * apu[1] + Jp[1][0] * apv[1];
-      H2 += Jp[0][0] * apu[2] + Jp[1][0] * apv[2];
-      H3 += Jp[0][1] * apu[1] + Jp[1][1] * apv[1];
-      H4 += Jp[0][1] * apu[2] + Jp[1][1] * apv[2];
-      H5 += Jp[0][2] * apu[2] + Jp[1][2] * apv[2];
-      g0 += Jp[0][0] * bu + Jp[1][0] * bv;
-      g1 += Jp[0][1] * bu + Jp[1][1] * bv;
-      g2 += Jp[0][2] * bu + Jp[1][2] * bv;
-    }
-  }
-  e.cost = warp_sum(cost);
-  e.H[0] = warp_sum(H0); e.H[1] = warp_sum(H1); e.H[2] = warp_sum(H2);
-  e.H[3] = warp_sum(H3); e.H[4] = warp_sum(H4); e.H[5] = warp_sum(H5);
-  e.g[0] = warp_sum(g0); e.g[1] = warp_sum(g1); e.g[2] = warp_sum(g2);
-}
-
-template <typename T, int C, bool FS>
-__global__ void __launch_bounds__(128) ba_inner_kernel(InnerArgs a) {
-  const int64_t p = ((int64_t)blockIdx.x * blockDim.x + threadIdx.x) >> 5;
-  const int lane = threadIdx.x & 31;
-  if (p >= a.n_points || a.point_off[p] < 0) return;
-  if (a.pt_begin[p + 1] == a.pt_begin[p]) return;
-  const int max_iter = 50, max_invalid = 5;
-  const double ftol = 1e-6, gtol = 1e-10, ptol = 1e-8, min_rel_dec = 1e-3;
-  const double max_radius = 1e16, min_radius = 1e-32, min_diag = 1e-6, max_diag = 1e32;
-  double x[3] = {a.xyz[3 * p], a.xyz[3 * p + 1], a.xyz[3 * p + 2]};
-  PointEval cur;
-  inner_eval<T, C, FS>(a, p, lane, x, cur);
-  if (!isfinite(cur.cost)) return;
-  double sc[3];
-  sc[0] = 1.0 / (1.0 + sqrt(cur.H[0])); sc[1] = 1.0 / (1.0 + sqrt(cur.H[3])); sc[2] = 1.0 / (1.0 + sqrt(cur.H[5]));
-  double radius = 1e4, decrease_factor = 2.0;
-  double x_cost = cur.cost, current_cost = cur.cost;
-  double x_norm = sqrt(x[0] * x[0] + x[1] * x[1] + x[2] * x[2]);
-  double gmax = fmax(fabs(cur.g[0]), fmax(fabs(cur.g[1]), fabs(cur.g[2])));
-  int num_invalid = 0;
-  for (int iter = 1;; ++iter) {
-    if (iter - 1 >= max_iter) break;
-    if (gmax <= gtol) break;
-    if (radius < min_radius) break;
-    const double diag[3] = {cur.H[0], cur.H[3], cur.H[5]};
-    double D2[3];
-#pragma unroll
-    for (int k = 0; k < 3; ++k) {
-      const double s2 = sc[k] * sc[k];
-      D2[k] = fmin(fmax(diag[k] * s2, min_diag), max_diag) / (radius * s2);
-    }
-    const double Hf[9] = {cur.H[0], cur.H[1], cur.H[2], cur.H[1], cur.H[3], cur.H[4], cur.H[2], cur.H[4], cur.H[5]};
-    double inv[9];
-    bool valid = inv3_sym(Hf, D2, inv);
-    double d[3] = {0, 0, 0}, mcc = 0;
-    if (valid) {
-#pragma unroll
-      for (int k = 0; k < 3; ++k) d[k] = -(inv[k * 3] * cur.g[0] + inv[k * 3 + 1] * cur.g[1] + inv[k * 3 + 2] * cur.g[2]);
-      double gd = 0, dHd = 0;
-#pragma unroll
-      for (int k = 0; k < 3; ++k) {
-        gd += cur.g[k] * d[k];
-        dHd += d[k] * (Hf[k * 3] * d[0] + Hf[k * 3 + 1] * d[1] + Hf[k * 3 + 2] * d[2]);
-      }
-      mcc = -gd - 0.5 * dHd;
-      valid = isfinite(d[0]) && isfinite(d[1]) && isfinite(d[2]) && mcc > 0.0;
-    }
-    if (!valid) {
-      if (++num_invalid >= max_invalid) break;
-      radius /= decrease_factor; decrease_factor *= 2.0;
-      continue;
-    }
-    num_invalid = 0;
-    const double xc_[3] = {x[0] + d[0], x[1] + d[1], x[2] + d[2]};
-    PointEval cand;
-    inner_eval<T, C, FS>(a, p, lane, xc_, cand);
-    const double candidate_cost = isfinite(cand.cost) ? cand.cost : 1.7976931348623157e308;
-    const double step_norm = sqrt((xc_[0] - x[0]) * (xc_[0] - x[0]) + (xc_[1] - x[1]) * (xc_[1] - x[1]) + (xc_[2] - x[2]) * (xc_[2] - x[2]));
-    if (step_norm <= ptol * (x_norm + ptol)) break;
-    const double cost_change = x_cost - candidate_cost;
-    if (fabs(cost_change) <= ftol * x_cost) break;
-    const double rel = (current_cost - candidate_cost) / mcc;
-    if (rel > min_rel_dec) {
-      x[0] = xc_[0]; x[1] = xc_[1]; x[2] = xc_[2];
-      x_norm = sqrt(x[0] * x[0] + x[1] * x[1] + x[2] * x[2]);
-      cur = cand; x_cost = cand.cost; current_cost = candidate_cost;
-      gmax = fmax(fabs(cur.g[0]), fmax(fabs(cur.g[1]), fabs(cur.g[2])));
-      radius = radius / fmax(1.0 / 3.0, 1.0 - pow(2.0 * rel - 1.0, 3.0));
-      radius = fmin(max_radius, radius);
-      decrease_factor = 2.0;
-    } else {
-      radius /= decrease_factor; decrease_factor *= 2.0;
-    }
-  }
-  if (lane == 0) { a.xyz[3 * p] = x[0]; a.xyz[3 * p + 1] = x[1]; a.xyz[3 * p + 2] = x[2]; }
-}
 
 struct InnerState {
   double x[3];
   double cand[3];
   double cost, current_cost, H[6], g[3], sc[3];
   double radius, decf, xnorm, gmax, mcc;
-  int iter, invalid, active;
-};
-
-struct InnerStepArgs {
-  int64_t n_points;
-  const int64_t* point_off; const int64_t* pt_begin;
-  const double* obs_out; const double* juv; int juv_stride; int juv_w;
-  double* xyz;
-  InnerState* st;
-  LossParams loss;
-  int64_t* list;
-  unsigned long long* counters;
+  int iter, invalid;
 };
 
 __device__ __forceinline__ bool inner_propose(InnerState& s) {
@@ -251,43 +57,32 @@
   }
 }
 
-static __global__ void __launch_bounds__(128) inner_step_kernel(InnerStepArgs a, int phase) {
-  const int64_t p = (int64_t)blockIdx.x * blockDim.x + threadIdx.x;
-  if (p >= a.n_points) return;
-  InnerState s = a.st[p];
-  if (phase == 0) {
-    s.active = (a.point_off[p] >= 0 && a.pt_begin[p + 1] > a.pt_begin[p]) ? 1 : 0;
+__device__ __forceinline__ void inner_add(const LossParams& loss, const double* oo, const double* pu, const double* pv,
+                                          double& cost, double H[6], double g[3]) {
+  double rho[3];
+  loss_eval(loss, 1.0, oo[0], rho);
+  cost += 0.5 * rho[0];
+  const double bu = rho[1] * oo[1], bv = rho[1] * oo[2];
+  const double auu = rho[1] * oo[3], auv = rho[1] * oo[4], avv = rho[1] * oo[5];
+  double apu[3], apv[3];
+#pragma unroll
+  for (int k = 0; k < 3; ++k) { apu[k] = auu * pu[k] + auv * pv[k]; apv[k] = auv * pu[k] + avv * pv[k]; }
+  H[0] += pu[0] * apu[0] + pv[0] * apv[0];
+  H[1] += pu[0] * apu[1] + pv[0] * apv[1];
+  H[2] += pu[0] * apu[2] + pv[0] * apv[2];
+  H[3] += pu[1] * apu[1] + pv[1] * apv[1];
+  H[4] += pu[1] * apu[2] + pv[1] * apv[2];
+  H[5] += pu[2] * apu[2] + pv[2] * apv[2];
+#pragma unroll
+  for (int k = 0; k < 3; ++k) g[k] += pu[k] * bu + pv[k] * bv;
+}
+
+__device__ __forceinline__ bool inner_step(InnerState& s, bool first, double cost, const double H[6], const double g[3],
+                                           bool* accepted) {
+  const double ftol = 1e-6, ptol = 1e-8, min_rel_dec = 1e-3, max_radius = 1e16;
+  *accepted = first;
+  if (first) {
     s.iter = 0; s.invalid = 0;
-    if (!s.active) { a.st[p] = s; return; }
-#pragma unroll
-    for (int k = 0; k < 3; ++k) s.x[k] = a.xyz[3 * p + k];
-  } else if (!s.active) return;
-  double cost = 0, H[6] = {0, 0, 0, 0, 0, 0}, g[3] = {0, 0, 0};
-  for (int64_t o = a.pt_begin[p]; o < a.pt_begin[p + 1]; ++o) {
-    const double* oo = a.obs_out + o * 8;
-    double rho[3];
-    loss_eval(a.loss, 1.0, oo[0], rho);
-    cost += 0.5 * rho[0];
-    const double bu = rho[1] * oo[1], bv = rho[1] * oo[2];
-    const double auu = rho[1] * oo[3], auv = rho[1] * oo[4], avv = rho[1] * oo[5];
-    const double* J = a.juv + o * (int64_t)a.juv_stride;
-    const double pu[3] = {J[6], J[7], J[8]}, pv[3] = {J[a.juv_w + 6], J[a.juv_w + 7], J[a.juv_w + 8]};
-    double apu[3], apv[3];
-#pragma unroll
-    for (int k = 0; k < 3; ++k) { apu[k] = auu * pu[k] + auv * pv[k]; apv[k] = auv * pu[k] + avv * pv[k]; }
-    H[0] += pu[0] * apu[0] + pv[0] * apv[0];
-    H[1] += pu[0] * apu[1] + pv[0] * apv[1];
-    H[2] += pu[0] * apu[2] + pv[0] * apv[2];
-    H[3] += pu[1] * apu[1] + pv[1] * apv[1];
-    H[4] += pu[1] * apu[2] + pv[1] * apv[2];
-    H[5] += pu[2] * apu[2] + pv[2] * apv[2];
-#pragma unroll
-    for (int k = 0; k < 3; ++k) g[k] += pu[k] * bu + pv[k] * bv;
-  }
-  const double ftol = 1e-6, ptol = 1e-8, min_rel_dec = 1e-3, max_radius = 1e16;
-  bool go = true;
-  if (phase == 0) {
-    if (!isfinite(cost)) go = false;
     s.cost = s.current_cost = cost;
 #pragma unroll
     for (int k = 0; k < 6; ++k) s.H[k] = H[k];
@@ -297,51 +92,236 @@
     s.radius = 1e4; s.decf = 2.0;
     s.xnorm = sqrt(s.x[0] * s.x[0] + s.x[1] * s.x[1] + s.x[2] * s.x[2]);
     s.gmax = fmax(fabs(g[0]), fmax(fabs(g[1]), fabs(g[2])));
+    if (!isfinite(cost)) return false;
   } else {
     const double candidate_cost = isfinite(cost) ? cost : 1.7976931348623157e308;
     const double dx = s.cand[0] - s.x[0], dy = s.cand[1] - s.x[1], dz = s.cand[2] - s.x[2];
     const double step_norm = sqrt(dx * dx + dy * dy + dz * dz);
-    if (step_norm <= ptol * (s.xnorm + ptol)) go = false;
-    else if (fabs(s.cost - candidate_cost) <= ftol * s.cost) go = false;
-    else {
-      const double rel = (s.current_cost - candidate_cost) / s.mcc;
-      if (rel > min_rel_dec) {
-#pragma unroll
-        for (int k = 0; k < 3; ++k) { s.x[k] = s.cand[k]; s.g[k] = g[k]; }
-#pragma unroll
-        for (int k = 0; k < 6; ++k) s.H[k] = H[k];
-        s.xnorm = sqrt(s.x[0] * s.x[0] + s.x[1] * s.x[1] + s.x[2] * s.x[2]);
-        s.cost = cost; s.current_cost = candidate_cost;
-        s.gmax = fmax(fabs(g[0]), fmax(fabs(g[1]), fabs(g[2])));
-        s.radius = s.radius / fmax(1.0 / 3.0, 1.0 - pow(2.0 * rel - 1.0, 3.0));
-        s.radius = fmin(max_radius, s.radius);
-        s.decf = 2.0;
-      } else {
-        s.radius /= s.decf; s.decf *= 2.0;
+    if (step_norm <= ptol * (s.xnorm + ptol)) return false;
+    if (fabs(s.cost - candidate_cost) <= ftol * s.cost) return false;
+    const double rel = (s.current_cost - candidate_cost) / s.mcc;
+    if (rel > min_rel_dec) {
+      *accepted = true;
+#pragma unroll
+      for (int k = 0; k < 3; ++k) { s.x[k] = s.cand[k]; s.g[k] = g[k]; }
+#pragma unroll
+      for (int k = 0; k < 6; ++k) s.H[k] = H[k];
+      s.xnorm = sqrt(s.x[0] * s.x[0] + s.x[1] * s.x[1] + s.x[2] * s.x[2]);
+      s.cost = cost; s.current_cost = candidate_cost;
+      s.gmax = fmax(fabs(g[0]), fmax(fabs(g[1]), fabs(g[2])));
+      s.radius = s.radius / fmax(1.0 / 3.0, 1.0 - pow(2.0 * rel - 1.0, 3.0));
+      s.radius = fmin(max_radius, s.radius);
+      s.decf = 2.0;
+    } else {
+      s.radius /= s.decf; s.decf *= 2.0;
+    }
+  }
+  return inner_propose(s);
+}
+
+constexpr int kInnerSlots = 4;
+constexpr int kInnerRec = 12;
+
+struct InnerArgs {
+  int64_t n_points;
+  const int64_t* point_off; const int64_t* pt_begin;
+  ProjectArgs geo;
+  FmEvalArgs fm;
+  double* xyz;
+  double* rec;
+  unsigned long long* next_point;
+};
+
+struct InnerSlot {
+  InnerState st;
+  double x[3];
+  int64_t p, ob;
+  int n;
+  int first;
+};
+
+template <typename T, int C> struct InnerCfg {
+  static constexpr bool kSmall = C < 8;
+  static constexpr int kSlot = 16 * C * (int)sizeof(T);
+  static constexpr int kWarps = (kSmall || kSlot <= 4096) ? 8 : 4;
+  static constexpr int kSmem = kSmall ? 0 : kWarps * kFmStages * kSlot + kWarps * kFmStages * 8 + kWarps * 32 * (int)sizeof(FmAux);
+};
+
+__device__ __forceinline__ void inner_claim(const InnerArgs& a, InnerSlot& sl) {
+  for (;;) {
+    const int64_t p = (int64_t)atomicAdd(a.next_point, 1ull);
+    if (p >= a.n_points) { sl.p = -1; sl.n = 0; return; }
+    const int64_t ob = a.pt_begin[p], oe = a.pt_begin[p + 1];
+    if (a.point_off[p] < 0 || oe == ob) continue;
+    sl.p = p; sl.ob = ob; sl.n = (int)(oe - ob); sl.first = 1;
+#pragma unroll
+    for (int k = 0; k < 3; ++k) sl.st.x[k] = sl.x[k] = a.xyz[3 * p + k];
+    return;
+  }
+}
+
+__device__ __forceinline__ const InnerSlot& inner_item(const InnerSlot* slots, const int pre[kInnerSlots + 1], int k, int64_t* o) {
+  int s = 0, start = 0;
+#pragma unroll
+  for (int i = 1; i < kInnerSlots; ++i)
+    if (k >= pre[i]) { s = i; start = pre[i]; }
+  *o = slots[s].ob + (k - start);
+  return slots[s];
+}
+
+__device__ __forceinline__ void inner_project(const InnerArgs& a, const InnerSlot& sl, int64_t o, double uv[2]) {
+  const double X[3] = {sl.x[0], sl.x[1], sl.x[2]};
+  double xy[2], sc[2], Jpose[2][6], Jpt[2][3], Jk[2][kMaxK];
+  observe<true>(a.geo, o, X, uv, xy, sc, Jpose, Jpt, Jk);
+  double* r = a.rec + o * kInnerRec;
+#pragma unroll
+  for (int k = 0; k < 3; ++k) { r[6 + k] = sc[0] * Jpt[0][k]; r[9 + k] = sc[1] * Jpt[1][k]; }
+}
+
+template <typename T, int C, bool FS>
+__device__ __forceinline__ void inner_eval_warps(const InnerArgs& a, const InnerSlot* slots, const int pre[kInnerSlots + 1],
+                                                 int n_items, uint8_t* smem, uint32_t& phase_bits) {
+  constexpr int W = InnerCfg<T, C>::kWarps;
+  constexpr int CPL = C >= 32 ? C / 32 : 1;
+  constexpr int ACTIVE = C / CPL;
+  constexpr int TAP_BYTES = C * (int)sizeof(T);
+  constexpr int SLOT_BYTES = 16 * TAP_BYTES;
+  static_assert(TAP_BYTES % 16 == 0, "bulk copies need 16-byte multiples");
+  const int warp = threadIdx.x >> 5, lane = threadIdx.x & 31;
+  uint8_t* wbase = smem + (size_t)warp * kFmStages * SLOT_BYTES;
+  uint64_t* bars = reinterpret_cast<uint64_t*>(smem + (size_t)W * kFmStages * SLOT_BYTES) + warp * kFmStages;
+  FmAux* aux = reinterpret_cast<FmAux*>(smem + (size_t)W * kFmStages * SLOT_BYTES + W * kFmStages * 8) + warp * 32;
+  const FmEvalArgs& f = a.fm;
+  const bool active = lane < ACTIVE;
+  const int64_t patch_bytes = (int64_t)f.ph * f.pw * TAP_BYTES;
+  for (int base = 0; base < n_items; base += 32 * W) {
+    const int nvalid = min(32, (n_items - base - warp + W - 1) / W);
+    if (nvalid <= 0) break;
+    int64_t pt = 0;
+    __syncwarp();
+    if (lane < nvalid) {
+      int64_t o;
+      const InnerSlot& sl = inner_item(slots, pre, base + lane * W + warp, &o);
+      pt = sl.p;
+      double uv[2];
+      inner_project(a, sl, o, uv);
+      const int64_t pidx = f.item_patch ? f.item_patch[o] : o;
+      const FmAux x = window_geometry(uv[0], uv[1], f.patches + pidx * patch_bytes, o, f.ph, f.pw);
+      aux[lane] = x;
+      if (f.res_rect && !window_resident(f.res_rect[pidx], x.row, x.col, f.ph, f.pw)) {
+        const unsigned long long slot = atomicAdd(f.viol_count, 1ull);
+        if ((long long)slot < f.viol_capacity) f.viol_list[slot] = o;
       }
     }
-  }
-  if (go) go = inner_propose(s);
-  if (go) {
-#pragma unroll
-    for (int k = 0; k < 3; ++k) a.xyz[3 * p + k] = s.cand[k];
-  } else {
-    s.active = 0;
-#pragma unroll
-    for (int k = 0; k < 3; ++k) a.xyz[3 * p + k] = s.x[k];
-  }
-  a.st[p] = s;
-}
-
-static __global__ void __launch_bounds__(128) inner_list_kernel(InnerStepArgs a, int all_variable) {
-  const int64_t p = (int64_t)blockIdx.x * blockDim.x + threadIdx.x;
-  if (p >= a.n_points) return;
-  const bool act = all_variable ? (a.point_off[p] >= 0 && a.pt_begin[p + 1] > a.pt_begin[p]) : (a.st[p].active != 0);
-  if (!act) return;
-  const int64_t ob = a.pt_begin[p], n = a.pt_begin[p + 1] - ob;
-  const unsigned long long base = atomicAdd(&a.counters[0], (unsigned long long)n);
-  atomicAdd(&a.counters[1], 1ull);
-  for (int64_t i = 0; i < n; ++i) a.list[base + i] = ob + i;
+    __syncwarp();
+#pragma unroll
+    for (int s = 0; s < kFmStages; ++s)
+      if (s < nvalid) issue_window<TAP_BYTES>(aux[s], wbase + (size_t)s * SLOT_BYTES, &bars[s], f.ph, f.pw, lane);
+    for (int j = 0; j < nvalid; ++j) {
+      const int slot = j % kFmStages;
+      double refv[CPL];
+      if (f.refs) {
+        const int64_t jp = __shfl_sync(0xffffffffu, (long long)pt, j);
+        const double* rp = f.refs + jp * C + (active ? lane * CPL : 0);
+#pragma unroll
+        for (int k = 0; k < CPL; ++k) refv[k] = __ldg(rp + k);
+      }
+      mbar_wait(&bars[slot], (phase_bits >> slot) & 1u);
+      phase_bits ^= (1u << slot);
+      double fv[CPL], fr[CPL], fc[CPL], r[CPL], red[6];
+#pragma unroll
+      for (int k = 0; k < CPL; ++k) { fv[k] = 0; fr[k] = 0; fc[k] = 0; r[k] = 0; }
+      if (active) {
+        const SmemWindow<TAP_BYTES> win{wbase + (size_t)slot * SLOT_BYTES};
+        bicubic_window<T, C, CPL, true, FS>(win, lane, aux[j].xc, aux[j].xr, fv, fr, fc);
+      }
+      __syncwarp();
+      if (j + kFmStages < nvalid)
+        issue_window<TAP_BYTES>(aux[j + kFmStages], wbase + (size_t)slot * SLOT_BYTES, &bars[slot], f.ph, f.pw, lane);
+      const double tot = normalize_and_reduce<CPL, true, false>(active, f.l2_normalize != 0, f.refs ? refv : nullptr, fv, fr, fc, r, red, lane);
+      const int idx = ((lane >> 4) & 1) * 4 + ((lane >> 3) & 1) * 2 + ((lane >> 2) & 1);
+      if ((lane & 3) == 0 && idx < 6) a.rec[aux[j].item * kInnerRec + idx] = tot;
+    }
+  }
+}
+
+template <typename T, int C>
+__device__ __forceinline__ void inner_eval_threads(const InnerArgs& a, const InnerSlot* slots, const int pre[kInnerSlots + 1], int n_items) {
+  for (int k = threadIdx.x; k < n_items; k += blockDim.x) {
+    int64_t o;
+    const InnerSlot& sl = inner_item(slots, pre, k, &o);
+    double uv[2], red[6];
+    inner_project(a, sl, o, uv);
+    fm_small_item<T, C, true>(a.fm, o, uv[0], uv[1], red);
+    double* r = a.rec + o * kInnerRec;
+#pragma unroll
+    for (int i = 0; i < 6; ++i) r[i] = red[i];
+  }
+}
+
+__device__ __forceinline__ void inner_slot_step(const InnerArgs& a, InnerSlot& sl, int lane) {
+  double cost = 0, H[6] = {0, 0, 0, 0, 0, 0}, g[3] = {0, 0, 0};
+  for (int base = 0; base < sl.n; base += 32) {
+    const int m = min(32, sl.n - base);
+    double v[kInnerRec];
+#pragma unroll
+    for (int i = 0; i < kInnerRec; ++i) v[i] = lane < m ? a.rec[(sl.ob + base + lane) * kInnerRec + i] : 0.0;
+    for (int j = 0; j < m; ++j) {
+      double w[kInnerRec];
+#pragma unroll
+      for (int i = 0; i < kInnerRec; ++i) w[i] = __shfl_sync(0xffffffffu, v[i], j);
+      inner_add(a.fm.loss, w, w + 6, w + 9, cost, H, g);
+    }
+  }
+  bool accepted = false, go = false;
+  if (lane == 0) {
+    InnerState s = sl.st;
+    go = inner_step(s, sl.first != 0, cost, H, g, &accepted);
+#pragma unroll
+    for (int k = 0; k < 3; ++k) sl.x[k] = go ? s.cand[k] : s.x[k];
+    if (!go) {
+#pragma unroll
+      for (int k = 0; k < 3; ++k) a.xyz[3 * sl.p + k] = s.x[k];
+    }
+    sl.st = s; sl.first = 0;
+  }
+  accepted = __shfl_sync(0xffffffffu, accepted, 0);
+  go = __shfl_sync(0xffffffffu, go, 0);
+  if (accepted)
+    for (int i = lane; i < sl.n; i += 32) a.fm.out[(sl.ob + i) * 8] = a.rec[(sl.ob + i) * kInnerRec];
+  __syncwarp();
+  if (!go && lane == 0) inner_claim(a, sl);
+}
+
+template <typename T, int C, bool FS>
+__global__ void __launch_bounds__(InnerCfg<T, C>::kWarps * 32, 2) inner_fused_kernel(InnerArgs a) {
+  typedef InnerCfg<T, C> Cfg;
+  static_assert(kInnerSlots <= Cfg::kWarps, "one warp per slot runs its step");
+  __shared__ InnerSlot slots[kInnerSlots];
+  extern __shared__ __align__(128) uint8_t smem[];
+  const int warp = threadIdx.x >> 5, lane = threadIdx.x & 31;
+  if (threadIdx.x < kInnerSlots) inner_claim(a, slots[threadIdx.x]);
+  if (!Cfg::kSmall && lane == 0) {
+    uint64_t* bars = reinterpret_cast<uint64_t*>(smem + (size_t)Cfg::kWarps * kFmStages * Cfg::kSlot) + warp * kFmStages;
+#pragma unroll
+    for (int s = 0; s < kFmStages; ++s) mbar_init(&bars[s], 1);
+    mbar_fence_init();
+  }
+  __syncthreads();
+  uint32_t phase_bits = 0;
+  for (;;) {
+    int pre[kInnerSlots + 1];
+    pre[0] = 0;
+#pragma unroll
+    for (int s = 0; s < kInnerSlots; ++s) pre[s + 1] = pre[s] + slots[s].n;
+    const int n_items = pre[kInnerSlots];
+    if (n_items == 0) break;
+    if constexpr (Cfg::kSmall) inner_eval_threads<T, C>(a, slots, pre, n_items);
+    else inner_eval_warps<T, C, FS>(a, slots, pre, n_items, smem, phase_bits);
+    __syncthreads();
+    if (warp < kInnerSlots && slots[warp].n > 0) inner_slot_step(a, slots[warp], lane);
+    __syncthreads();
+  }
 }
 
 static __global__ void __launch_bounds__(256) diff_norm_kernel(const double* a, const double* b, int64_t n, double* acc, double* part = nullptr) {
```
